# tum-vision/mono_dataset_code

Hardware: AMD Instinct MI355X
Metric: Mpix/s photometric+FOV undistort, 1280x1024 gray (higher is better)
Workload: dtype f32

## Files before the change

### include/mdc_hip.h

```cpp
#ifndef MDC_HIP_H
#define MDC_HIP_H

#include <stddef.h>
#include <stdint.h>

#ifndef MDC_API
#if defined(__GNUC__) || defined(__clang__)
#define MDC_API __attribute__((visibility("default")))
#else
#define MDC_API
#endif
#endif

#ifdef __cplusplus
extern "C" {
#endif

typedef struct mdc_ctx mdc_ctx;

typedef enum mdc_status {
  MDC_OK = 0,
  MDC_ERR_ARG = -1,
  MDC_ERR_STATE = -2,
  MDC_ERR_SIZE = -3,
  MDC_ERR_HIP = -4,
  MDC_ERR_NO_DEVICE = -5,
  MDC_ERR_NOMEM = -6
} mdc_status;

enum {
  MDC_GAMMA = 1u,
  MDC_VIGNETTE = 2u,
  MDC_KILL_OVEREXPOSED = 4u,
  MDC_RECTIFY = 8u
};

enum {
  MDC_KERNEL_AUTO = 0,
  MDC_KERNEL_GATHER = 1,
  MDC_KERNEL_TILED = 2
};
enum { MDC_OPT_KERNEL = 1, MDC_OPT_FRAMES_PER_BLOCK = 2 ,
       MDC_OPT_TILE_ROWS = 5 ,
       MDC_OPT_TILE_ORDER = 6 ,
       MDC_OPT_WINDOW_BUFFERS = 7 ,
       MDC_OPT_FRAME_INTERLEAVE = 8 ,
       MDC_OPT_TILE_COLS = 9 ,
       MDC_OPT_PIN_CALLER_BUFFERS = 10 ,
       MDC_OPT_TWO_STAGE = 11 ,
       MDC_OPT_PREFETCH_CHUNK = 12 ,
       MDC_OPT_PREFETCH_STREAMS = 13 ,
       MDC_OPT_ZERO_COPY = 14 ,
       MDC_OPT_DEVICE_PIPELINE_CHUNK = 16 ,
       MDC_OPT_DEVICE_PIPELINE_CHUNK_HINT = 17 ,
       MDC_OPT_TAIL_TAPER = 15 ,
       MDC_OPT_XCD_ROTATE = 18  };
enum { MDC_ORDER_BANDS = 0 , MDC_ORDER_ROWS = 1 ,
       MDC_ORDER_IDENTITY = 2 ,
       MDC_ORDER_BLOCKS2D = 3  };

typedef struct mdc_info {
  int device;
  int in_w, in_h;
  int out_w, out_h;
  int valid_gamma;
  int valid_vignette;
  int valid_remap;
  int tiled;
  int tile_w, tile_h;
  int n_tiles;
  int lds_bytes;
  int window_buffers;
  int f32_tiled;
  int f32_tile_w, f32_tile_h;
  int src_bbox[4];
  int64_t src_bbox_bytes;
  int64_t src_staged_bytes;
  int64_t n_black;
  int two_stage;
  int prefetch_chunk;
  int prefetch_streams;
} mdc_info;


MDC_API int mdc_create(int device, mdc_ctx** out);
MDC_API int mdc_device_count(void);
MDC_API int mdc_device_pci_bus_id(mdc_ctx* ctx, char* buf, size_t cap);
MDC_API void mdc_destroy(mdc_ctx* ctx);
MDC_API const char* mdc_last_error(const mdc_ctx* ctx);
MDC_API int mdc_get_info(mdc_ctx* ctx, mdc_info* info);
MDC_API int mdc_set_option(mdc_ctx* ctx, int option, int value);
MDC_API const char* mdc_build_flags(void);
MDC_API const char* mdc_code_id(void);


MDC_API int mdc_set_photometric(mdc_ctx* ctx, const float* ginv, const float* vignette_inv, int w, int h);

MDC_API int mdc_set_remap(mdc_ctx* ctx, const float* remap_x, const float* remap_y, int in_w, int in_h, int out_w, int out_h);


MDC_API int mdc_unmap_host(mdc_ctx* ctx, const uint8_t* image_in, float* image_out, int n, unsigned flags);

MDC_API int mdc_undistort_host_f32(mdc_ctx* ctx, const float* input, float* output, int n_in, int n_out);
MDC_API int mdc_undistort_host_u8(mdc_ctx* ctx, const uint8_t* input, float* output, int n_in, int n_out);

MDC_API int mdc_process_host(mdc_ctx* ctx, const uint8_t* raw, float* out, unsigned flags);


MDC_API void* mdc_host_alloc(size_t bytes);
MDC_API void mdc_host_free(void* p);

MDC_API int mdc_process_frames_host(mdc_ctx* ctx, const uint8_t* const* raw, float* const* out, int64_t nframes,
                            unsigned flags);

MDC_API int mdc_process_jpeg_frames_host(mdc_ctx* ctx, const void* const* records, int64_t record_bytes, int blocks_w, int blocks_rows,
                                 float* const* out, int64_t nframes, unsigned flags);
MDC_API int mdc_jpeg_idct_batch_device(mdc_ctx* ctx, const void* d_records, int64_t record_bytes, uint8_t* d_frames, int w, int h, int blocks_w,
                               int blocks_rows, int64_t nframes, void* stream);

#define MDC_JPEG_STREAM_MAGIC 0x33534a4du
#define MDC_JPEG_HUFF_SUBTABLES 32
typedef struct mdc_jpeg_huff {
  uint32_t t1[2048];
  uint32_t t2[MDC_JPEG_HUFF_SUBTABLES][32];
} mdc_jpeg_huff;
typedef struct mdc_jpeg_stream_header {
  uint32_t magic, w, h, ecs_bytes;
  uint32_t restart_interval;
  uint32_t n_intervals;
  uint32_t comp_info;
  uint32_t ecs_offset;
  uint16_t quant[64];
  mdc_jpeg_huff dc, ac;
} mdc_jpeg_stream_header;
MDC_API int mdc_process_jpeg_streams_host(mdc_ctx* ctx, const void* const* streams, const int64_t* stream_bytes, float* const* out, int64_t nframes,
                                  unsigned flags, int* status);
MDC_API int mdc_jpeg_huffman_batch_device(mdc_ctx* ctx, const void* d_streams, int64_t stream_stride, void* d_records, int64_t record_bytes, int w,
                                  int h, int blocks_w, int blocks_rows, int64_t nframes, int* d_status, void* stream);

typedef struct mdc_device_outputs {
  float* base;
  int levels;
  float* level[3];
  float* dI[4];
  float* abs_squared_grad[4];
} mdc_device_outputs;
MDC_API int mdc_process_frames_host_to_device(mdc_ctx* ctx, const uint8_t* const* raw, int64_t nframes, unsigned flags,
                                              const mdc_device_outputs* out, const int64_t* frame_index);
MDC_API int mdc_process_jpeg_frames_host_to_device(mdc_ctx* ctx, const void* const* records, int64_t record_bytes, int blocks_w, int blocks_rows,
                                                   int64_t nframes, unsigned flags, const mdc_device_outputs* out, const int64_t* frame_index);
MDC_API int mdc_process_jpeg_streams_host_to_device(mdc_ctx* ctx, const void* const* streams, const int64_t* stream_bytes, int64_t nframes,
                                                    unsigned flags, const mdc_device_outputs* out, const int64_t* frame_index, int* status);
MDC_API int mdc_device_alloc(mdc_ctx* ctx, size_t bytes, void** d_ptr);
MDC_API int mdc_tune_placement_device(mdc_ctx* ctx, const uint8_t* const* d_in, int n_in, float* const* d_out, int n_out, int64_t nframes,
                                      unsigned flags, void* stream, int* best_in, int* best_out, float* ms);
enum { MDC_PLACE_AUTO = 0, MDC_PLACE_FIRST = 1, MDC_PLACE_MALLOC = 2, MDC_PLACE_VMM = 3 };
typedef struct mdc_placed_buffers {
  uint8_t* d_in;
  float* d_out;
  size_t in_bytes, out_bytes;
  int64_t nframes, probe_frames;
  int strategy;
  int candidates_in, candidates_out, picked_in, picked_out;
  float pair_ms[64];
  int pieces, piece_mib;
  int class_count[3];
  float ms_first, ms_chosen;
  char note[384];
  void* handle;
} mdc_placed_buffers;
MDC_API int mdc_alloc_placed_device(mdc_ctx* ctx, size_t in_bytes, size_t out_bytes, int64_t nframes, unsigned flags, int strategy, void* stream,
                                    mdc_placed_buffers* out);
MDC_API int mdc_free_placed_device(mdc_ctx* ctx, mdc_placed_buffers* buffers);
#define MDC_STRIPED_SET_MAX 16
typedef struct mdc_striped_set {
  int n;
  void* d_ptr[MDC_STRIPED_SET_MAX];
  size_t bytes[MDC_STRIPED_SET_MAX];
  int strategy;
  int pieces, piece_mib;
  int class_count[3];
  char note[384];
  void* handle;
} mdc_striped_set;
MDC_API int mdc_alloc_striped_set_device(mdc_ctx* ctx, int n, const size_t* bytes, void* stream, mdc_striped_set* out);
MDC_API int mdc_free_striped_set_device(mdc_ctx* ctx, mdc_striped_set* set);
MDC_API void mdc_device_free(mdc_ctx* ctx, void* d_ptr);
MDC_API int mdc_copy_to_host(mdc_ctx* ctx, void* dst, const void* d_src, size_t bytes);


MDC_API int mdc_unmap_batch_device(mdc_ctx* ctx, const uint8_t* d_in, float* d_out, int64_t nframes, unsigned flags,
                           void* stream);

MDC_API int mdc_process_batch_device(mdc_ctx* ctx, const uint8_t* d_in, float* d_out, int64_t nframes, unsigned flags,
                             void* stream);

MDC_API int mdc_undistort_batch_device_f32(mdc_ctx* ctx, const float* d_in, float* d_out, int64_t nframes, void* stream);

MDC_API int mdc_pyramid_batch_device(mdc_ctx* ctx, const float* d_base, int w, int h, int levels, float* const* d_levels,
                             int64_t nframes, void* stream);

MDC_API int mdc_process_pyramid_batch_device(mdc_ctx* ctx, const uint8_t* d_in, float* d_base, int levels,
                                     float* const* d_levels, int64_t nframes, unsigned flags, void* stream);

MDC_API int mdc_gradients_batch_device(mdc_ctx* ctx, const float* d_level, int w, int h, float* d_dI, float* d_abs_squared_grad,
                               int64_t nframes, void* stream);

MDC_API int mdc_process_pyramid_gradients_batch_device(mdc_ctx* ctx, const uint8_t* d_in, float* d_base, int levels, float* const* d_levels,
                                               float* const* d_dI, float* const* d_abs_squared_grad, int64_t nframes, unsigned flags,
                                               int chunk_frames, void* stream);


typedef struct mdc_fov_model {
  float in_calib[5];
  int in_w, in_h;
  float out_calib[5];
  int out_w, out_h;
} mdc_fov_model;

MDC_API int mdc_distort_points_device(mdc_ctx* ctx, const mdc_fov_model* model, float* d_x, float* d_y, int64_t n, void* stream);
MDC_API int mdc_distort_points_host(mdc_ctx* ctx, const mdc_fov_model* model, float* x, float* y, int64_t n);



MDC_API int mdc_vcal_plane_step_device(mdc_ctx* ctx, const float* d_images, const float* d_p2x, const float* d_p2y, int n_images, int w, int h,
                               int n_plane, float* d_plane_color, const float* d_vignette_factor, int oth2, float* d_ff,
                               float* d_fc, double* d_er, void* stream);
MDC_API int mdc_vcal_vignette_step_device(mdc_ctx* ctx, const float* d_images, const float* d_p2x, const float* d_p2y, int n_images, int w,
                                  int h, int n_plane, const float* d_plane_color, float* d_vignette_factor, int oth2, float* d_tt,
                                  float* d_ct, double* d_er, void* stream);

typedef struct mdc_vcal_index mdc_vcal_index;
MDC_API int mdc_vcal_index_create(mdc_ctx* ctx, const float* d_images, const float* d_p2x, const float* d_p2y, int n_images, int w, int h,
                          int n_plane, void* stream, mdc_vcal_index** out);
MDC_API void mdc_vcal_index_destroy(mdc_vcal_index* index);
MDC_API int64_t mdc_vcal_index_bytes(const mdc_vcal_index* index);
MDC_API int64_t mdc_vcal_index_entries(const mdc_vcal_index* index);
MDC_API int mdc_vcal_vignette_step_indexed_device(mdc_ctx* ctx, const mdc_vcal_index* index, const float* d_plane_color,
                                          float* d_vignette_factor, int oth2, float* d_tt, float* d_ct, double* d_er, void* stream);

MDC_API int mdc_vcal_solve_device(mdc_ctx* ctx, const float* d_images, const float* d_p2x, const float* d_p2y, int n_images, int w, int h,
                          int n_plane, float* d_plane_color, float* d_vignette_factor, int max_iterations, int outlier_th,
                          double* er_out, void* stream);

MDC_API int mdc_vcal_scale_images_device(mdc_ctx* ctx, float* d_images, int n_images, int64_t npix, float mean_exposure,
                                 const float* d_exposure_times, void* stream);

MDC_API int mdc_vcal_gradient_mask_device(mdc_ctx* ctx, float* d_images, int n_images, int w, int h, int max_abs_grad, void* stream);

MDC_API int mdc_vcal_mask_coords_device(mdc_ctx* ctx, float* d_x, float* d_y, int64_t n, int w, int h, void* stream);

MDC_API int mdc_vcal_plane_coords_device(mdc_ctx* ctx, const mdc_fov_model* model, const float* d_corners, float* d_hk, int n, int gw,
                                 int gh, float facw, float fach, float* d_p2x, float* d_p2y, void* stream);

MDC_API int mdc_vcal_smooth_device(mdc_ctx* ctx, const float* d_vignette_factor, int w, int h, float* d_smoothed, float* d_scratch,
                           void* stream);

MDC_API int mdc_vcal_plot_plane_device(mdc_ctx* ctx, const float* d_plane, int gw, int gh, uint8_t* d_rgb, float* range_host, void* stream);
MDC_API int mdc_vcal_vignette_u16_device(mdc_ctx* ctx, const float* d_vignette, int64_t n, uint16_t* d_out, void* stream);



MDC_API int mdc_rcal_leak_pad_device(mdc_ctx* ctx, uint8_t* d_images, int n_images, int w, int h, int leak_padding, void* stream);
MDC_API int mdc_rcal_init_e_device(mdc_ctx* ctx, const uint8_t* d_images, int n_images, int w, int h, double* d_E, void* stream);
MDC_API int mdc_rcal_rmse_device(mdc_ctx* ctx, const uint8_t* d_images, const double* d_exposure, int n_images, int w, int h,
                         const double* d_G, const double* d_E, double* d_out, void* stream);
MDC_API int mdc_rcal_g_step_device(mdc_ctx* ctx, const uint8_t* d_images, const double* d_exposure, int n_images, int w, int h,
                           const double* d_E, double* d_G, void* stream);
typedef struct mdc_rcal_index mdc_rcal_index;
MDC_API int mdc_rcal_index_create(mdc_ctx* ctx, const uint8_t* d_images, int n_images, int w, int h, void* stream, mdc_rcal_index** out);
MDC_API void mdc_rcal_index_destroy(mdc_rcal_index* index);
MDC_API int64_t mdc_rcal_index_bytes(const mdc_rcal_index* index);
MDC_API int64_t mdc_rcal_index_entries(const mdc_rcal_index* index);
MDC_API int64_t mdc_rcal_index_longest_chain(const mdc_rcal_index* index);
MDC_API int mdc_rcal_g_step_indexed_device(mdc_ctx* ctx, const mdc_rcal_index* index, const double* d_exposure, const double* d_E,
                                   double* d_G, void* stream);
MDC_API int mdc_rcal_e_step_device(mdc_ctx* ctx, const uint8_t* d_images, const double* d_exposure, int n_images, int w, int h,
                           const double* d_G, double* d_E, double* d_rmse_g, void* stream);
MDC_API int mdc_rcal_rescale_device(mdc_ctx* ctx, const uint8_t* d_images, const double* d_exposure, int n_images, int w, int h,
                            double* d_G, double* d_E, double* d_rmse_e, double* d_rmse_resc, void* stream);

#define MDC_RCAL_EXACT_ORDER 0u
#define MDC_RCAL_DIRECT 1u
typedef struct mdc_rcal_iter {
  double rmse_G, num_G;
  double rmse_E, num_E;
  double rmse_resc, num_resc;
  double rescale;
} mdc_rcal_iter;
typedef struct mdc_rcal_log {
  double init_rmse, init_num;
  mdc_rcal_iter* iters;
} mdc_rcal_log;
MDC_API int mdc_rcal_solve_device(mdc_ctx* ctx, const uint8_t* d_images, const double* d_exposure, int n_images, int w, int h,
                          int iterations, unsigned mode, double* d_G, double* d_E, mdc_rcal_log* log, void* stream);
MDC_API int mdc_rcal_plot_e_device(mdc_ctx* ctx, const double* d_E, int w, int h, uint8_t* d_rgb, uint16_t* d_e16, double* range_host,
                           void* stream);
MDC_API int mdc_rcal_plot_g_device(mdc_ctx* ctx, const double* d_G, float* d_img, double* range_host, void* stream);
MDC_API int mdc_copy_to_device(mdc_ctx* ctx, void* d_dst, const void* src, size_t bytes);

typedef struct mdc_tune_result {
  int tile_w, tile_h, frames_per_block;
  float ms;
  int candidates;
} mdc_tune_result;
MDC_API int mdc_tune_device(mdc_ctx* ctx, const uint8_t* d_in, float* d_out, int64_t nframes, unsigned flags, void* stream,
                    mdc_tune_result* result);

MDC_API int mdc_describe_launch(mdc_ctx* ctx, unsigned flags, int pyramid_levels, char* buf, size_t cap);


MDC_API int mdc_export_tables(mdc_ctx* ctx, void* blob, size_t cap, size_t* size);
MDC_API int mdc_import_tables(mdc_ctx* ctx, const void* blob, size_t size);

MDC_API int mdc_synchronize(mdc_ctx* ctx);

#ifdef __cplusplus
}
#endif
#endif
```

### mono_dataset_code_amd/build.py

```python
import os
import shutil
import subprocess
import time
import sys

PKG = os.path.dirname(os.path.abspath(__file__))
ROOT = os.path.dirname(PKG)
CSRC = os.path.join(PKG, "csrc")
HOST = os.path.join(CSRC, "host")
INC = os.path.join(ROOT, "include")
EIGEN_STUB = os.path.join(INC, "mono_dataset_code", "compat")

LIB_HIP = os.path.join(PKG, "libmdc_hip.so")
LIB_HOST = os.path.join(PKG, "libmdc_host.so")

HIP_SOURCES = [os.path.join(CSRC, f) for f in ("mdc_kernels.hip", "mdc_vcal.hip", "mdc_jpeg.hip", "mdc_capi.hip", "mdc_plan.hip", "mdc_host_calls.hip",
                                                "mdc_pipeline.hip", "mdc_placement.hip", "mdc_rcal.hip")]
HIP_DEPS = HIP_SOURCES + [os.path.join(CSRC, "mdc_exports.map"), os.path.join(CSRC, "mdc_internal.h"), os.path.join(CSRC, "mdc_ctx.h"), os.path.join(CSRC, "mdc_build_config.h"), os.path.join(CSRC, "fov_point_model.h"), os.path.join(CSRC, "minmax_first.h"), os.path.join(CSRC, "placement_classes.h"), os.path.join(CSRC, "xcd_placement.h"), os.path.join(INC, "mdc_hip.h")]
HOST_SOURCES = [os.path.join(HOST, f) for f in (
    "fov_undistorter.cpp", "photometric_undistorter.cpp", "gray_png.cpp", "host_device.cpp", "mdc_host_capi.cpp",
    "image_codecs.cpp", "image_codecs_png.cpp", "image_codecs_jpeg.cpp", "image_codecs_jpeg_stream.cpp", "zip_reader.cpp", "image_pool.cpp", "frame_source.cpp", "decode_pool.cpp",
    "prefetch_cache.cpp", "device_lanes.cpp", "batch_run.cpp", "dataset_reader.cpp")]
HOST_DEPS = HOST_SOURCES + [os.path.join(HOST, "mdc_host_exports.map"), os.path.join(HOST, "gray_png.h"), os.path.join(HOST, "host_device.h"),
                            os.path.join(HOST, "image_codecs.h"), os.path.join(HOST, "image_codecs_internal.h"), os.path.join(HOST, "image_codecs_jpeg.h"), os.path.join(HOST, "zip_reader.h"),
                            os.path.join(HOST, "frame_source.h"), os.path.join(HOST, "decode_pool.h"), os.path.join(HOST, "prefetch_cache.h"),
                            os.path.join(HOST, "device_lanes.h"), os.path.join(HOST, "batch_run.h"), os.path.join(CSRC, "png_inflate_core.h"),
                            os.path.join(INC, "mono_dataset_code", "BenchmarkDatasetReader.h"),
                            os.path.join(INC, "mdc_hip.h"), os.path.join(INC, "mdc_host.h"),
                            os.path.join(INC, "mono_dataset_code", "FOVUndistorter.h"),
                            os.path.join(INC, "mono_dataset_code", "PhotometricUndistorter.h"),
                            os.path.join(INC, "mono_dataset_code", "ExposureImage.h"),
                            os.path.join(INC, "mono_dataset_code", "MdcBind.h")]

HIP_FLAGS = ["--offload-arch=gfx950", "-O3", "-std=c++17", "-ffp-contract=off", "-fPIC", "-shared",
             "-fno-fast-math", "-fvisibility=hidden", "-fvisibility-inlines-hidden", "-Wall", "-Wno-unused-function"]
HOST_FLAGS = ["-O2", "-std=c++11", "-ffp-contract=off", "-fPIC", "-shared", "-fvisibility=hidden", "-fvisibility-inlines-hidden", "-Wall"]
HOST_EXPORT_MAP = os.path.join(HOST, "mdc_host_exports.map")
EXPORT_MAP = os.path.join(CSRC, "mdc_exports.map")
RECIPE = os.path.abspath(__file__)


def _stale(target, deps):
    if not os.path.exists(target):
        return True
    t = os.path.getmtime(target)
    return any(os.path.getmtime(d) > t for d in deps)


def _run(cmd):
    r = subprocess.run(cmd, stdout=subprocess.PIPE, stderr=subprocess.STDOUT, text=True)
    if r.returncode != 0:
        sys.stderr.write(r.stdout)
        raise RuntimeError("build failed: " + " ".join(cmd))
    return r.stdout


def hipcc():
    for c in (os.environ.get("HIPCC"), shutil.which("hipcc"), "/opt/rocm/bin/hipcc"):
        if c and os.path.exists(c):
            return c
    raise RuntimeError("hipcc not found")


def eigen_include():
    for d in ("/usr/include/eigen3", "/usr/local/include/eigen3"):
        if os.path.exists(os.path.join(d, "Eigen", "Core")):
            return d
    return EIGEN_STUB


def code_text(src):
    out, i, n = [], 0, len(src)
    while i < n:
        c = src[i]
        if c == "/" and i + 1 < n and src[i + 1] == "/":
            while i < n and src[i] != "\n":
                if src[i] == "\\" and i + 1 < n and src[i + 1] == "\n":
                    i += 1
                i += 1
        elif c == "/" and i + 1 < n and src[i + 1] == "*":
            j = src.find("*/", i + 2)
            i = n if j < 0 else j + 2
            out.append(" ")
        elif c in "\"'":
            j = i + 1
            while j < n and src[j] != c:
                j += 2 if src[j] == "\\" else 1
            out.append(src[i:j + 1])
            i = j + 1
        elif c in " \t\r\f\v":
            if not out or out[-1] != " ":
                out.append(" ")
            i += 1
        else:
            out.append(c)
            i += 1
    lines = [l.strip() for l in "".join(out).split("\n")]
    return "\n".join(l for l in lines if l)


def code_id(defines=()):
    import hashlib

    h = hashlib.sha256()
    for path in sorted(HIP_DEPS):
        h.update(os.path.basename(path).encode() + b"\0")
        with open(path, "r", encoding="utf-8", errors="surrogateescape") as f:
            h.update(code_text(f.read()).encode("utf-8", "surrogateescape"))
    h.update(" ".join(HIP_FLAGS + sorted(defines)).encode())
    try:
        h.update(subprocess.run([hipcc(), "--version"], stdout=subprocess.PIPE).stdout)
    except OSError:
        pass
    return h.hexdigest()[:16]


def _linked_from(lib, defines=()):
    try:
        with open(lib, "rb") as f:
            return code_id(defines).encode() in f.read()
    except OSError:
        return False


def _compile_link_hip(out, defines=(), objdir_tag="product"):
    from concurrent.futures import ThreadPoolExecutor

    started = time.time()
    identity = code_id(defines)
    objdir = os.path.join(PKG, "build", objdir_tag)
    os.makedirs(objdir, exist_ok=True)
    flags = [f for f in HIP_FLAGS if f != "-shared"] + ["-I" + INC] + ["-D" + d for d in defines]
    stamp = os.path.join(objdir, "flags.txt")
    flags_changed = not os.path.exists(stamp) or open(stamp).read() != " ".join(flags)
    headers = [d for d in HIP_DEPS if d not in HIP_SOURCES]
    jobs = []
    for src in HIP_SOURCES:
        obj = os.path.join(objdir, os.path.basename(src) + ".o")
        if flags_changed or _stale(obj, [src] + headers) or not os.path.exists(out) or not _linked_from(out, defines):
            jobs.append([hipcc()] + flags + ["-c", src, "-o", obj])
    with ThreadPoolExecutor(max_workers=max(1, len(jobs))) as ex:
        list(ex.map(_run, jobs))
    with open(stamp, "w") as f:
        f.write(" ".join(flags))
    objs = [os.path.join(objdir, os.path.basename(src) + ".o") for src in HIP_SOURCES]
    idsrc = os.path.join(objdir, "mdc_code_id.cpp")
    with open(idsrc, "w") as f:
        f.write('#include "mdc_hip.h"\nextern "C" const char* mdc_code_id(void) { return "%s"; }\n' % identity)
    idobj = idsrc + ".o"
    _run(["g++", "-O1", "-fPIC", "-fvisibility=hidden", "-I" + INC, "-c", idsrc, "-o", idobj])
    _run([hipcc(), "--offload-arch=gfx950", "-shared", "-fPIC", "-Wl,--version-script=" + EXPORT_MAP] + objs + [idobj, "-o", out])
    if any(os.path.getmtime(d) > started for d in HIP_DEPS):
        sys.stderr.write("mono_dataset_code_amd.build: a source changed while %s was being built; it is stamped %s and the next build redoes it\n"
                         % (os.path.basename(out), identity))


def build_hip(force=False):
    if force or _stale(LIB_HIP, HIP_DEPS + [RECIPE]) or not _linked_from(LIB_HIP):
        if force:
            shutil.rmtree(os.path.join(PKG, "build", "product"), ignore_errors=True)
        _compile_link_hip(LIB_HIP)
    return LIB_HIP


def build_host(force=False):
    build_hip(force)
    if force or _stale(LIB_HOST, HOST_DEPS + [LIB_HIP]):
        _run(["g++"] + HOST_FLAGS + ["-I" + INC, "-I" + os.path.join(INC, "mono_dataset_code"), "-I" + HOST,
                                     "-I" + eigen_include()] + HOST_SOURCES +
             ["-L" + PKG, "-lmdc_hip", "-Wl,-rpath,$ORIGIN", "-Wl,--version-script=" + HOST_EXPORT_MAP, "-lz", "-lpthread", "-ldl", "-o", LIB_HOST])
    return LIB_HOST
# ... 211 lines not shown
```

### mono_dataset_code_amd/capi.py

```python
import ctypes as C
import os
import types

import numpy as np

_PKG = os.path.dirname(os.path.abspath(__file__))
LIB_HIP_PATH = os.environ.get("MDC_LIB_HIP") or os.path.join(_PKG, "libmdc_hip.so")
LIB_HOST_PATH = os.path.join(_PKG, "libmdc_host.so")

GAMMA, VIGNETTE, KILL_OVEREXPOSED, RECTIFY = 1, 2, 4, 8
KERNEL_AUTO, KERNEL_GATHER, KERNEL_TILED = 0, 1, 2
OPT_KERNEL, OPT_FRAMES_PER_BLOCK, OPT_TILE_ROWS, OPT_TILE_ORDER, OPT_WINDOW_BUFFERS, OPT_FRAME_INTERLEAVE, OPT_TILE_COLS, OPT_PIN_CALLER_BUFFERS = 1, 2, 5, 6, 7, 8, 9, 10
OPT_TWO_STAGE = 11
OPT_PREFETCH_CHUNK = 12
OPT_PREFETCH_STREAMS = 13
OPT_ZERO_COPY = 14
OPT_TAIL_TAPER = 15
OPT_XCD_ROTATE = 18
OPT_DEVICE_PIPELINE_CHUNK, OPT_DEVICE_PIPELINE_CHUNK_HINT = 16, 17
ORDER_BANDS, ORDER_ROWS, ORDER_IDENTITY, ORDER_BLOCKS2D = 0, 1, 2, 3
OK, ERR_ARG, ERR_STATE, ERR_SIZE, ERR_HIP, ERR_NO_DEVICE, ERR_NOMEM = 0, -1, -2, -3, -4, -5, -6

PLACE_AUTO, PLACE_FIRST, PLACE_MALLOC, PLACE_VMM = 0, 1, 2, 3
PLACE_NAMES = {PLACE_AUTO: "auto", PLACE_FIRST: "first", PLACE_MALLOC: "malloc", PLACE_VMM: "vmm"}


RCAL_EXACT_ORDER, RCAL_DIRECT = 0, 1


class RcalIter(C.Structure):
    _fields_ = [(n, C.c_double) for n in ("rmse_G", "num_G", "rmse_E", "num_E", "rmse_resc", "num_resc", "rescale")]


class RcalLog(C.Structure):
    _fields_ = [("init_rmse", C.c_double), ("init_num", C.c_double), ("iters", C.POINTER(RcalIter))]


class PlacedBuffers(C.Structure):
    _fields_ = [("d_in", C.c_void_p), ("d_out", C.c_void_p), ("in_bytes", C.c_size_t), ("out_bytes", C.c_size_t), ("nframes", C.c_int64),
                ("probe_frames", C.c_int64), ("strategy", C.c_int), ("candidates_in", C.c_int), ("candidates_out", C.c_int), ("picked_in", C.c_int),
                ("picked_out", C.c_int), ("pair_ms", C.c_float * 64), ("pieces", C.c_int), ("piece_mib", C.c_int), ("class_count", C.c_int * 3),
                ("ms_first", C.c_float), ("ms_chosen", C.c_float), ("note", C.c_char * 384), ("handle", C.c_void_p)]

    def describe(self):
        d = {"strategy": PLACE_NAMES.get(self.strategy, str(self.strategy)), "how": self.note.decode(errors="replace"),
             "probe_frames": int(self.probe_frames), "ms_on_first_allocations": round(float(self.ms_first), 4) or None,
             "ms_on_chosen_pair": round(float(self.ms_chosen), 4) or None}
        if self.strategy == PLACE_MALLOC and self.candidates_in > 1:
            ki, ko = self.candidates_in, self.candidates_out
            d["ms_frames_i_results_j"] = [[round(float(self.pair_ms[i * ko + j]), 4) for j in range(ko)] for i in range(ki)]
            d["picked_frames"], d["picked_results"] = int(self.picked_in), int(self.picked_out)
        if self.strategy == PLACE_VMM:
            d["pieces"], d["piece_mib"], d["class_count"] = int(self.pieces), int(self.piece_mib), [int(x) for x in self.class_count]
        return d


class StripedSet(C.Structure):
    _fields_ = [("n", C.c_int), ("d_ptr", C.c_void_p * 16), ("bytes", C.c_size_t * 16), ("strategy", C.c_int), ("pieces", C.c_int), ("piece_mib", C.c_int),
                ("class_count", C.c_int * 3), ("note", C.c_char * 384), ("handle", C.c_void_p)]


class FovModel(C.Structure):
    _fields_ = [("in_calib", C.c_float * 5), ("in_w", C.c_int), ("in_h", C.c_int), ("out_calib", C.c_float * 5),
                ("out_w", C.c_int), ("out_h", C.c_int)]


class MdcInfo(C.Structure):
    _fields_ = [("device", C.c_int), ("in_w", C.c_int), ("in_h", C.c_int), ("out_w", C.c_int), ("out_h", C.c_int),
                ("valid_gamma", C.c_int), ("valid_vignette", C.c_int), ("valid_remap", C.c_int), ("tiled", C.c_int),
                ("tile_w", C.c_int), ("tile_h", C.c_int), ("n_tiles", C.c_int), ("lds_bytes", C.c_int),
                ("window_buffers", C.c_int), ("f32_tiled", C.c_int), ("f32_tile_w", C.c_int), ("f32_tile_h", C.c_int),
                ("src_bbox", C.c_int * 4), ("src_bbox_bytes", C.c_int64), ("src_staged_bytes", C.c_int64),
                ("n_black", C.c_int64), ("two_stage", C.c_int), ("prefetch_chunk", C.c_int), ("prefetch_streams", C.c_int)]


class DeviceOutputs(C.Structure):
    _fields_ = [("base", C.c_void_p), ("levels", C.c_int), ("level", C.c_void_p * 3), ("dI", C.c_void_p * 4), ("abs_squared_grad", C.c_void_p * 4)]

    @classmethod
    def make(cls, base, levels=1, level=(), dI=(), abs2=()):
        o = cls()
        o.base, o.levels = base, levels
        for i, p in enumerate(level):
            o.level[i] = p
        for i, p in enumerate(dI):
            o.dI[i] = p
        for i, p in enumerate(abs2):
            o.abs_squared_grad[i] = p
        return o


class TuneResult(C.Structure):
    _fields_ = [("tile_w", C.c_int), ("tile_h", C.c_int), ("frames_per_block", C.c_int), ("ms", C.c_float), ("candidates", C.c_int)]


class MdcError(RuntimeError):
    def __init__(self, code, msg):
        super().__init__("mdc error %d: %s" % (code, msg))
        self.code = code


_vp, _i, _i64, _u32, _sz = C.c_void_p, C.c_int, C.c_int64, C.c_uint32, C.c_size_t
_u, _f, _cp, _P = C.c_uint, C.c_float, C.c_char_p, C.POINTER

HIP_API = {
    "mdc_create": (_i, [_i, _P(_vp)]),
    "mdc_device_count": (_i, []),
    "mdc_device_pci_bus_id": (_i, [_vp, _cp, _sz]),
    "mdc_destroy": (None, [_vp]),
    "mdc_last_error": (_cp, [_vp]),
    "mdc_get_info": (_i, [_vp, _P(MdcInfo)]),
    "mdc_set_option": (_i, [_vp, _i, _i]),
    "mdc_build_flags": (_cp, []),
    "mdc_code_id": (_cp, []),
    "mdc_set_photometric": (_i, [_vp, _vp, _vp, _i, _i]),
    "mdc_set_remap": (_i, [_vp, _vp, _vp, _i, _i, _i, _i]),
    "mdc_unmap_host": (_i, [_vp, _vp, _vp, _i, _u]),
    "mdc_undistort_host_f32": (_i, [_vp, _vp, _vp, _i, _i]),
    "mdc_undistort_host_u8": (_i, [_vp, _vp, _vp, _i, _i]),
    "mdc_process_host": (_i, [_vp, _vp, _vp, _u]),
    "mdc_host_alloc": (_vp, [_sz]),
    "mdc_host_free": (None, [_vp]),
    "mdc_process_frames_host": (_i, [_vp, _P(_vp), _P(_vp), _i64, _u]),
    "mdc_process_jpeg_frames_host": (_i, [_vp, _P(_vp), _i64, _i, _i, _P(_vp), _i64, _u]),
    "mdc_jpeg_idct_batch_device": (_i, [_vp, _vp, _i64, _vp, _i, _i, _i, _i, _i64, _vp]),
    "mdc_process_jpeg_streams_host": (_i, [_vp, _P(_vp), _P(_i64), _P(_vp), _i64, _u, _P(_i)]),
    "mdc_jpeg_huffman_batch_device": (_i, [_vp, _vp, _i64, _vp, _i64, _i, _i, _i, _i, _i64, _vp, _vp]),
    "mdc_process_frames_host_to_device": (_i, [_vp, _P(_vp), _i64, _u, _P(DeviceOutputs), _P(_i64)]),
    "mdc_process_jpeg_frames_host_to_device": (_i, [_vp, _P(_vp), _i64, _i, _i, _i64, _u, _P(DeviceOutputs), _P(_i64)]),
    "mdc_process_jpeg_streams_host_to_device": (_i, [_vp, _P(_vp), _P(_i64), _i64, _u, _P(DeviceOutputs), _P(_i64), _P(_i)]),
    "mdc_device_alloc": (_i, [_vp, _sz, _P(_vp)]),
    "mdc_tune_placement_device": (_i, [_vp, _P(_vp), _i, _P(_vp), _i, _i64, _u, _vp, _P(_i), _P(_i), _P(_f)]),
    "mdc_alloc_placed_device": (_i, [_vp, _sz, _sz, _i64, _u, _i, _vp, _P(PlacedBuffers)]),
    "mdc_free_placed_device": (_i, [_vp, _P(PlacedBuffers)]),
    "mdc_alloc_striped_set_device": (_i, [_vp, _i, _P(_sz), _vp, _P(StripedSet)]),
    "mdc_free_striped_set_device": (_i, [_vp, _P(StripedSet)]),
    "mdc_device_free": (None, [_vp, _vp]),
    "mdc_copy_to_host": (_i, [_vp, _vp, _vp, _sz]),
    "mdc_unmap_batch_device": (_i, [_vp, _vp, _vp, _i64, _u, _vp]),
    "mdc_process_batch_device": (_i, [_vp, _vp, _vp, _i64, _u, _vp]),
    "mdc_undistort_batch_device_f32": (_i, [_vp, _vp, _vp, _i64, _vp]),
    "mdc_pyramid_batch_device": (_i, [_vp, _vp, _i, _i, _i, _P(_vp), _i64, _vp]),
    "mdc_process_pyramid_batch_device": (_i, [_vp, _vp, _vp, _i, _P(_vp), _i64, _u, _vp]),
    "mdc_gradients_batch_device": (_i, [_vp, _vp, _i, _i, _vp, _vp, _i64, _vp]),
    "mdc_process_pyramid_gradients_batch_device": (_i, [_vp, _vp, _vp, _i, _P(_vp), _P(_vp), _P(_vp), _i64, _u, _i, _vp]),
    "mdc_distort_points_device": (_i, [_vp, _P(FovModel), _vp, _vp, _i64, _vp]),
    "mdc_distort_points_host": (_i, [_vp, _P(FovModel), _vp, _vp, _i64]),
    "mdc_vcal_plane_step_device": (_i, [_vp, _vp, _vp, _vp, _i, _i, _i, _i, _vp, _vp, _i, _vp, _vp, _vp, _vp]),
    "mdc_vcal_vignette_step_device": (_i, [_vp, _vp, _vp, _vp, _i, _i, _i, _i, _vp, _vp, _i, _vp, _vp, _vp, _vp]),
    "mdc_vcal_index_create": (_i, [_vp, _vp, _vp, _vp, _i, _i, _i, _i, _vp, _P(_vp)]),
    "mdc_vcal_index_destroy": (None, [_vp]),
    "mdc_vcal_index_bytes": (_i64, [_vp]),
    "mdc_vcal_index_entries": (_i64, [_vp]),
    "mdc_vcal_vignette_step_indexed_device": (_i, [_vp, _vp, _vp, _vp, _i, _vp, _vp, _vp, _vp]),
    "mdc_vcal_solve_device": (_i, [_vp, _vp, _vp, _vp, _i, _i, _i, _i, _vp, _vp, _i, _i, _vp, _vp]),
    "mdc_vcal_scale_images_device": (_i, [_vp, _vp, _i, _i64, _f, _vp, _vp]),
    "mdc_vcal_gradient_mask_device": (_i, [_vp, _vp, _i, _i, _i, _i, _vp]),
    "mdc_vcal_mask_coords_device": (_i, [_vp, _vp, _vp, _i64, _i, _i, _vp]),
    "mdc_vcal_plane_coords_device": (_i, [_vp, _P(FovModel), _vp, _vp, _i, _i, _i, _f, _f, _vp, _vp, _vp]),
    "mdc_vcal_smooth_device": (_i, [_vp, _vp, _i, _i, _vp, _vp, _vp]),
    "mdc_vcal_plot_plane_device": (_i, [_vp, _vp, _i, _i, _vp, _vp, _vp]),
    "mdc_vcal_vignette_u16_device": (_i, [_vp, _vp, _i64, _vp, _vp]),
    "mdc_rcal_leak_pad_device": (_i, [_vp, _vp, _i, _i, _i, _i, _vp]),
    "mdc_rcal_init_e_device": (_i, [_vp, _vp, _i, _i, _i, _vp, _vp]),
    "mdc_rcal_rmse_device": (_i, [_vp, _vp, _vp, _i, _i, _i, _vp, _vp, _vp, _vp]),
    "mdc_rcal_g_step_device": (_i, [_vp, _vp, _vp, _i, _i, _i, _vp, _vp, _vp]),
    "mdc_rcal_index_create": (_i, [_vp, _vp, _i, _i, _i, _vp, _P(_vp)]),
    "mdc_rcal_index_destroy": (None, [_vp]),
    "mdc_rcal_index_bytes": (_i64, [_vp]),
    "mdc_rcal_index_entries": (_i64, [_vp]),
    "mdc_rcal_index_longest_chain": (_i64, [_vp]),
    "mdc_rcal_g_step_indexed_device": (_i, [_vp, _vp, _vp, _vp, _vp, _vp]),
    "mdc_rcal_e_step_device": (_i, [_vp, _vp, _vp, _i, _i, _i, _vp, _vp, _vp, _vp]),
    "mdc_rcal_rescale_device": (_i, [_vp, _vp, _vp, _i, _i, _i, _vp, _vp, _vp, _vp, _vp]),
    "mdc_rcal_solve_device": (_i, [_vp, _vp, _vp, _i, _i, _i, _i, _u, _vp, _vp, _P(RcalLog), _vp]),
    "mdc_rcal_plot_e_device": (_i, [_vp, _vp, _i, _i, _vp, _vp, _vp, _vp]),
    "mdc_rcal_plot_g_device": (_i, [_vp, _vp, _vp, _vp, _vp]),
    "mdc_copy_to_device": (_i, [_vp, _vp, _vp, _sz]),
    "mdc_tune_device": (_i, [_vp, _vp, _vp, _i64, _u, _vp, _P(TuneResult)]),
    "mdc_describe_launch": (_i, [_vp, _u, _i, _cp, _sz]),
    "mdc_export_tables": (_i, [_vp, _vp, _sz, _P(_sz)]),
    "mdc_import_tables": (_i, [_vp, _vp, _sz]),
    "mdc_synchronize": (_i, [_vp]),
}
HOST_API = {
    "mdch_fov_create": (_vp, [_cp]),
    "mdch_fov_destroy": (None, [_vp]),
    "mdch_fov_valid": (_i, [_vp]),
    "mdch_fov_has_gpu": (_i, [_vp]),
    "mdch_fov_dims": (None, [_vp, _vp]),
    "mdch_fov_intrinsics": (None, [_vp, _vp]),
    "mdch_fov_remap": (_i, [_vp, _vp, _vp]),
    "mdch_fov_distort": (None, [_vp, _vp, _vp, _i]),
    "mdch_fov_undistort_f32": (None, [_vp, _vp, _vp, _i, _i]),
    "mdch_fov_undistort_u8": (None, [_vp, _vp, _vp, _i, _i]),
    "mdch_fov_model": (None, [_vp, _P(FovModel)]),
    "mdch_photo_create": (_vp, [_cp, _cp, _i, _i]),
    "mdch_photo_destroy": (None, [_vp]),
    "mdch_photo_valid": (_i, [_vp]),
    "mdch_photo_has_gpu": (_i, [_vp]),
    "mdch_photo_ginv": (_i, [_vp, _vp]),
    "mdch_photo_g": (_i, [_vp, _vp]),
    "mdch_photo_vignette": (_i, [_vp, _vp, _vp]),
    "mdch_photo_unmap": (None, [_vp, _vp, _vp, _i, _i, _i, _i]),
    "mdch_bind": (_i, [_vp, _vp, _vp]),
    "mdch_pack_tables": (_i, [_vp, _vp, _vp, _sz, _P(_sz)]),
    "mdch_reader_create": (_vp, [_cp]),
    "mdch_reader_destroy": (None, [_vp]),
    "mdch_reader_num_images": (_i, [_vp]),
    "mdch_reader_timestamp": (C.c_double, [_vp, _i]),
    "mdch_reader_exposure": (_f, [_vp, _i]),
    "mdch_reader_dims": (None, [_vp, _vp]),
    "mdch_reader_get_image": (_i, [_vp, _i, _i, _i, _i, _i, _vp, C.c_long, _vp, _P(C.c_double), _P(_f)]),
    "mdch_reader_get_images": (_i, [_vp, _i, _i, _i, _i, _i, _i, _vp, C.c_long, _vp]),
    "mdch_reader_get_images_device": (_i, [_vp, _i, _i, _i, _i, _i, _i, _P(DeviceOutputs), _vp]),
    "mdch_reader_context": (_vp, [_vp]),
    "mdch_reader_device": (_i, [_vp]),
    "mdch_reader_get_raw": (_i, [_vp, _i, _vp, C.c_long, _vp]),
    "mdch_reader_get_images_raw_device": (_i, [_vp, _i, _i, _i, _vp, _vp]),
    "mdch_reader_raw_dims": (None, [_vp, _vp]),
    "mdch_reader_set_threads": (None, [_vp, _i]),
    "mdch_reader_set_prefetch": (None, [_vp, _i]),
    "mdch_reader_set_lookahead": (None, [_vp, _i]),
    "mdch_reader_set_gpu_jpeg": (None, [_vp, _i]),
    "mdch_reader_set_gpu_png": (None, [_vp, _i]),
    "mdch_reader_png_device_frames": (C.c_long, [_vp]),
    "mdch_reader_last_error": (_cp, [_vp]),
    "mdch_reader_prefetch_stats": (None, [_vp, _vp]),
    "mdch_reader_device_stats": (_i, [_vp, _i, _vp, _vp]),
    "mdch_decode_gray8": (_i, [_vp, _sz, _vp, _sz, _vp, _cp, _sz]),
    "mdch_jpeg_record_bytes": (_sz, [_i, _i, _vp]),
    "mdch_decode_jpeg_record": (_i, [_vp, _sz, _vp, _sz, _i, _vp, _cp, _sz]),
    "mdch_jpeg_stream": (C.c_longlong, [_vp, _sz, _vp, _sz, _vp, _cp, _sz]),
    "mdch_png_stream": (_i, [_vp, _sz, _P(_i), _P(_i), _vp, _sz, _P(_sz)]),
    "mdch_image_alloc": (_vp, [C.c_ulong]),
    "mdch_image_free": (None, [_vp]),
    "mdch_image_pool_trim": (None, []),
    "mdch_image_pool_idle_bytes": (C.c_ulong, []),
}
BENCH_API = {
    "mdcb_synth_frames_device": (_i, [_i, _vp, _i64, _i64, _i, _u32, _vp]),
    "mdcb_ceiling_mix_device": (_i, [_i, _vp, _i64, _vp, _i64, _i, _i, _vp]),
    "mdcb_marker_device": (_i, [_i, _i, _vp]),
    "mdcb_alias_alloc": (_i, [_i, _i64, _i, _P(_vp), _P(_i64)]),
    "mdcb_alias_free": (_i, [_i, _vp, _i64, _i]),
    "mdcb_chunked_alloc": (_i, [_i, _i64, _i, _i, _P(_vp)]),
# ... 1225 lines not shown
```

### mono_dataset_code_amd/csrc/mdc_capi.hip

```cpp
#include "mdc_ctx.h"

using namespace mdc;


namespace mdc {

static thread_local std::string g_create_err;
static thread_local std::string t_err, t_err_other;
static thread_local const mdc_ctx* t_err_ctx = nullptr;

int fail(mdc_ctx* c, int code, const char* fmt, ...) {
  char buf[512];
  va_list ap;
  va_start(ap, fmt);
  vsnprintf(buf, sizeof buf, fmt, ap);
  va_end(ap);
  if (c) {
    {
      std::lock_guard<std::mutex> lk(c->err_mu);
      c->err = buf;
    }
    t_err = buf;
    t_err_ctx = c;
  } else {
    g_create_err = buf;
  }
  return code;
}



void normalise(const mdc_ctx* c, unsigned flags, bool& g, bool& v, bool& o) {
  g = (flags & MDC_GAMMA) != 0;
  v = (flags & MDC_VIGNETTE) != 0;
  o = (flags & MDC_KILL_OVEREXPOSED) != 0;
  if (!c->valid_gamma && g) g = false;
  if (!c->valid_vignette && v) v = false;
  if (!g && v) {
    v = false;
    g = false;
  }
}

const float* lut_for(const mdc_ctx* c, bool g, bool o) { return c->d_luts + 256 * ((g ? 1 : 0) | (o ? 2 : 0)); }

int upload_luts(mdc_ctx* c) {
  std::vector<float> l(4 * 256);
  for (int var = 0; var < 4; var++)
    for (int b = 0; b < 256; b++) {
      float x = (var & 1) ? (c->valid_gamma ? c->h_ginv[b] : (float)b) : (float)b;
      if ((var & 2) && b == 255) x = std::numeric_limits<float>::quiet_NaN();
      l[var * 256 + b] = x;
    }
  if (!c->d_luts) MDC_HIP(c, hipMalloc(&c->d_luts, l.size() * sizeof(float)));
  MDC_HIP(c, hipMemcpy(c->d_luts, l.data(), l.size() * sizeof(float), hipMemcpyHostToDevice));
  return MDC_OK;
}

int frames_per_block(const mdc_ctx* c, int64_t nframes, int blocks_per_group, int target_wgs) {
  if (c->opt_fpb > 0) return (int)std::min<int64_t>(c->opt_fpb, std::max<int64_t>(nframes, 1));
  int64_t groups = std::max<int64_t>(1, (target_wgs + blocks_per_group - 1) / std::max(1, blocks_per_group));
  groups = std::min<int64_t>(groups, std::max<int64_t>(1, nframes / 8));
  int64_t fpb = (nframes + groups - 1) / groups;
  if (fpb < 32 && (int64_t)blocks_per_group * ((nframes + 31) / 32) >= 2048) fpb = 32;
  if (target_wgs == 4800 && fpb > 64) fpb = 64;
  return (int)fpb;
}













TilePlan tile_plan(const mdc_ctx* c, int which) {
  const mdc_ctx::SrcPlan& pl = c->plan[which];
  return TilePlan{pl.d_chunks, pl.d_nch, pl.d_taps, pl.d_order, pl.n_blocks, pl.n_tiles, pl.tiles_x, pl.tile_w, pl.tile_h,
                  pl.chunk_cap, pl.win_bytes, pl.nbuf, c->n_black > 0, c->opt_interleave != 0, c->opt_taper != 2, c->opt_xcd_rotate != 0};
}

RemapArgs remap_args(const mdc_ctx* c, const float* lut, const float* vinv) {
  RemapArgs a;
  a.lut = lut;
  a.vinv = vinv;
  a.rx = c->d_rx;
  a.ry = c->d_ry;
  a.in_w = c->rm_in_w;
  a.in_h = c->rm_in_h;
  a.out_w = c->out_w;
  a.out_h = c->out_h;
  return a;
}

int64_t prefetch_box_bytes(const mdc_ctx* c) {
  const int x0 = c->bbox[0], x1 = c->bbox[2], y0 = c->bbox[1], y1 = c->bbox[3];
  return y1 >= y0 ? (int64_t)(y1 - y0 + 1) * std::min(c->rm_in_w, ((x1 + 128) & ~127) - (x0 & ~127)) : 0;
}
int prefetch_streams(const mdc_ctx* c) { return c->opt_prefetch_streams == 1 ? 1 : 2; }
int64_t strip_resident(bool pyr) { return 256 * (pyr ? 4 : 5); }
int64_t chunk_groups(const mdc_ctx* c, bool pyr) {
  const int64_t nb = std::max(1, c->strip.n_blocks);
  return std::max<int64_t>(1, (strip_resident(pyr) * 5 / 8 + nb / 2) / nb);
}
int64_t prefetch_chunk_frames(const mdc_ctx* c, bool pyr = true) {
  if (c->opt_prefetch_chunk > 0) return c->opt_prefetch_chunk;
  const int64_t box = std::max<int64_t>(1, prefetch_box_bytes(c));
  if (prefetch_streams(c) == 1) return std::max<int64_t>(16, (31ll << 20) / box);
  const int64_t g = chunk_groups(c, pyr);
  const int64_t per_group = std::max<int64_t>(8, ((26ll << 20) / box + g / 2) / g);
  return g * per_group;
}

int enqueue_undistort_f32(mdc_ctx* c, const float* d_in, float* d_out, int64_t nframes, hipStream_t s) {
  RemapArgs a = remap_args(c, nullptr, nullptr);
  const bool aligned = (reinterpret_cast<uintptr_t>(d_in) & 15) == 0;
  if (c->plan[1].tiled && aligned && c->opt_kernel != MDC_KERNEL_GATHER) {
    const int fpb = frames_per_block(c, nframes, c->plan[1].n_blocks);
    MDC_HIP(c, launch_remap_tiled_f32(d_in, d_out, a, tile_plan(c, 1), nframes, fpb, s));
  } else {
    const int fpb = frames_per_block(c, nframes, (c->out_w * c->out_h + 255) / 256);
    MDC_HIP(c, launch_remap_gather_f32(d_in, d_out, a, nframes, fpb, s));
  }
  return MDC_OK;
}

int enqueue_process(mdc_ctx* c, const uint8_t* d_in, float* d_out, int64_t nframes, unsigned flags, hipStream_t s,
                    float* const* pyr, bool* pyr_done) {
  if (pyr_done) *pyr_done = false;
  bool g, v, o;
  normalise(c, flags, g, v, o);
  const float* lut = lut_for(c, g, o);
  const float* vinv = v ? c->d_vinv : nullptr;
  if (!(flags & MDC_RECTIFY)) {
    const int fw = c->in_w > 0 ? c->in_w : c->rm_in_w, fh = c->in_h > 0 ? c->in_h : c->rm_in_h;
    if (fw <= 0 || fh <= 0) return fail(c, MDC_ERR_STATE, "frame size unknown: set the photometric tables or a remap first");
    const int64_t npix = (int64_t)fw * fh;
    int fpb = frames_per_block(c, nframes, (int)((npix + 4095) / 4096), 20000);
    if (!c->opt_fpb) fpb = std::min(fpb, 8);
    MDC_HIP(c, launch_unmap(d_in, d_out, lut, vinv, npix, nframes, fpb, s));
    return MDC_OK;
  }
  if (!c->valid_remap) return fail(c, MDC_ERR_STATE, "no remap set (UndistorterFOV invalid)");
  if (vinv && (c->in_w != c->rm_in_w || c->in_h != c->rm_in_h))
    return fail(c, MDC_ERR_SIZE, "vignette is %dx%d but the remap expects %dx%d input", c->in_w, c->in_h, c->rm_in_w,
                c->rm_in_h);
  RemapArgs a = remap_args(c, lut, vinv);
  const bool aligned = (reinterpret_cast<uintptr_t>(d_in) & 15) == 0;
  if (c->strip.planned && aligned && c->opt_kernel != MDC_KERNEL_GATHER) {
    const mdc_ctx::Strip& st = c->strip;
    const StripPlan sp{st.d_chunks, st.d_nch, st.d_taps, st.d_order, st.n_blocks, st.n_tiles, st.tiles_x, st.win_bytes, st.passes, st.nbuf,
                       c->opt_interleave != 0, c->opt_xcd_rotate == 2};
    const bool fuse_pyr = pyr && c->out_w % kStripTileW == 0;
    const int iw = c->rm_in_w;
    const int x0 = c->bbox[0], x1 = c->bbox[2], y0 = c->bbox[1], y1 = c->bbox[3];
    const int64_t frame_in = (int64_t)iw * c->rm_in_h;
    const int64_t box_bytes = prefetch_box_bytes(c);
    int64_t chunk = prefetch_chunk_frames(c, fuse_pyr);
    const bool prefetch = c->opt_prefetch_chunk >= 0 && (fuse_pyr || c->opt_prefetch_chunk > 0 || prefetch_streams(c) == 2) && box_bytes >= 4096 &&
                          nframes >= 2 * chunk;
    if (!prefetch) chunk = nframes;
    const size_t no = (size_t)c->out_w * c->out_h;
    const int64_t resident = strip_resident(fuse_pyr);
    auto strip = [&](int64_t f0, int64_t n, int fpb, hipStream_t t) {
      return launch_remap_strip_u8(d_in + (size_t)f0 * frame_in, d_out + (size_t)f0 * no, a, sp, n, fpb, t,
                                   fuse_pyr ? pyr[0] + (size_t)f0 * (no / 4) : nullptr, fuse_pyr ? pyr[1] + (size_t)f0 * (no / 16) : nullptr,
                                   fuse_pyr ? pyr[2] + (size_t)f0 * (no / 64) : nullptr);
    };
    hipStreamCaptureStatus capturing = hipStreamCaptureStatusNone;
    if (hipStreamIsCapturing(s, &capturing) != hipSuccess) {
      (void)hipGetLastError();
      capturing = hipStreamCaptureStatusNone;
    }
    if (prefetch && prefetch_streams(c) == 2 && capturing == hipStreamCaptureStatusNone) {
      SlotLease side(c, false);
      side.drained();
      mdc_ctx::HostSlot* h = side.s;
      if (h && !h->ev_fork) {
        if (hipEventCreateWithFlags(&h->ev_fork, hipEventDisableTiming) != hipSuccess) h->ev_fork = nullptr;
        if (h->ev_fork && hipEventCreateWithFlags(&h->ev_join, hipEventDisableTiming) != hipSuccess) {
          (void)hipEventDestroy(h->ev_fork);
          h->ev_fork = nullptr;
        }
      }
      if (h && h->ev_fork) {
        const int64_t groups = chunk_groups(c, fuse_pyr);
        MDC_HIP(c, hipEventRecord(h->ev_fork, s));
        MDC_HIP(c, hipStreamWaitEvent(h->stream, h->ev_fork, 0));
        hipError_t e = hipSuccess;
        int k = 0;
        for (int64_t f0 = 0; f0 < nframes && e == hipSuccess; f0 += chunk, k++) {
          const int64_t n = std::min<int64_t>(chunk, nframes - f0);
          hipStream_t t = (k & 1) ? h->stream : s;
          e = launch_prefetch_rows(d_in + (size_t)f0 * frame_in, frame_in, iw, x0, x1, y0, y1, n, c->d_vcal_max, t);
          const int fpb = c->opt_fpb > 0 ? (int)std::min<int64_t>(c->opt_fpb, n) : (int)((n + groups - 1) / groups);
          if (e == hipSuccess) e = strip(f0, n, fpb, t);
        }
        const hipError_t ej = hipEventRecord(h->ev_join, h->stream);
        const hipError_t ew = ej == hipSuccess ? hipStreamWaitEvent(s, h->ev_join, 0) : ej;
        MDC_HIP(c, e);
        MDC_HIP(c, ew);
        if (pyr_done) *pyr_done = fuse_pyr;
        return MDC_OK;
      }
    }
    if (prefetch) MDC_HIP(c, launch_prefetch_rows(d_in, frame_in, iw, x0, x1, y0, y1, std::min<int64_t>(chunk, nframes), c->d_vcal_max, s));
    for (int64_t f0 = 0; f0 < nframes; f0 += chunk) {
      const int64_t n = std::min<int64_t>(chunk, nframes - f0);
      if (prefetch && f0 + chunk < nframes)
        MDC_HIP(c, launch_prefetch_rows(d_in + (size_t)(f0 + chunk) * frame_in, frame_in, iw, x0, x1, y0, y1, std::min<int64_t>(chunk, nframes - f0 - chunk),
                                        c->d_vcal_max, s));
      int fpb = frames_per_block(c, n, st.n_blocks);
      if (prefetch && !c->opt_fpb) fpb = (int)std::max<int64_t>(8, (n * st.n_blocks + resident - 1) / resident);
      MDC_HIP(c, strip(f0, n, fpb, s));
    }
    if (pyr_done) *pyr_done = fuse_pyr;
    return MDC_OK;
  }
  bool use_tiled = c->plan[0].tiled && aligned;
  if (c->opt_kernel == MDC_KERNEL_GATHER) use_tiled = false;
  if (c->opt_kernel == MDC_KERNEL_TILED && !use_tiled)
    return fail(c, MDC_ERR_STATE, "tiled kernel requested but not plannable for this remap / alignment");
  if (use_tiled) {
    const TilePlan p = tile_plan(c, 0);
    int fpb = frames_per_block(c, nframes, p.n_blocks);
    if (!c->opt_fpb && c->tuned_fpb > 0 && nframes >= c->tuned_min_frames) fpb = (int)std::min<int64_t>(c->tuned_fpb, nframes);
    const bool fuse_pyr = pyr && p.tile_w * p.tile_h <= 2048 && p.tile_h % 8 == 0 && c->out_w % p.tile_w == 0 && c->out_h % p.tile_h == 0 &&
                          tiled_lds_bytes(p.win_bytes, p.nbuf, true) + tiled_pyramid_lds_bytes(p.tile_w, p.tile_h) <= kLdsPerCU;
    MDC_HIP(c, launch_remap_tiled_u8(d_in, d_out, a, p, nframes, fpb, s, fuse_pyr ? pyr[0] : nullptr,
                                     fuse_pyr ? pyr[1] : nullptr, fuse_pyr ? pyr[2] : nullptr));
    if (pyr_done) *pyr_done = fuse_pyr;
  } else {
    const int fpb = frames_per_block(c, nframes, (c->out_w * c->out_h + 255) / 256);
    MDC_HIP(c, launch_remap_gather_u8(d_in, d_out, a, nframes, fpb, s));
  }
  return MDC_OK;
}

int enqueue_pyramid_gradients(mdc_ctx* c, const uint8_t* d_in, float* d_base, int levels, float* const* d_levels, float* const* d_dI,
                              float* const* d_abs_squared_grad, int64_t nframes, unsigned flags, int chunk_frames, hipStream_t s) {
  const bool with_gradients = d_dI != nullptr && d_abs_squared_grad != nullptr;
  const bool rect = (flags & MDC_RECTIFY) != 0;
  if (rect && !c->valid_remap) return fail(c, MDC_ERR_STATE, "no remap set (UndistorterFOV invalid)");
  const int w0 = rect ? c->out_w : (c->in_w > 0 ? c->in_w : c->rm_in_w), h0 = rect ? c->out_h : (c->in_h > 0 ? c->in_h : c->rm_in_h);
  const int iw = (rect || c->in_w <= 0) ? c->rm_in_w : c->in_w, ih = (rect || c->in_h <= 0) ? c->rm_in_h : c->in_h;
  if (w0 <= 0 || h0 <= 0 || iw <= 0 || ih <= 0) return fail(c, MDC_ERR_STATE, "frame size unknown");
  int lw[8], lh[8];
  size_t level_bytes = 0;
  for (int l = 0; l < levels; l++) {
    lw[l] = w0 >> l;
    lh[l] = h0 >> l;
    if (lw[l] < 1 || lh[l] < 1) return fail(c, MDC_ERR_ARG, "level %d of a %dx%d image is empty", l, w0, h0);
    level_bytes += (size_t)lw[l] * lh[l] * sizeof(float);
  }
  int64_t chunk = chunk_frames;
  if (chunk <= 0) {
    chunk = (int64_t)((672ull << 20) / level_bytes);
    chunk = chunk >= 32 ? chunk / 32 * 32 : std::max<int64_t>(1, chunk);
  }
  {
    int64_t wgs = 0;
    for (int l = 0; l < std::min(levels, 4); l++) wgs += (int64_t)((lw[l] + 127) / 128) * ((lh[l] + 7) / 8);
    chunk = std::max<int64_t>(1, std::min<int64_t>(chunk, ((1ll << 31) - 1) / std::max<int64_t>(1, wgs)));
  }
  const size_t npi = (size_t)iw * ih;
  for (int64_t f0 = 0; f0 < nframes; f0 += chunk) {
    const int64_t n = std::min<int64_t>(chunk, nframes - f0);
    float* lv[8];
    for (int l = 1; l < levels; l++) lv[l - 1] = d_levels[l - 1] + (size_t)f0 * lw[l] * lh[l];
    float* base = d_base + (size_t)f0 * w0 * h0;
    float* pyr[3] = {levels > 1 ? lv[0] : nullptr, levels > 2 ? lv[1] : nullptr, levels > 3 ? lv[2] : nullptr};
    bool fused = false;
#if MDC_EXP_STRIP_FAKE_GRAD
    g_fake_grad_dI = with_gradients ? d_dI[0] + (size_t)f0 * w0 * h0 * 3 : nullptr;
    g_fake_grad_abs = with_gradients ? d_abs_squared_grad[0] + (size_t)f0 * w0 * h0 : nullptr;
#endif
    int rc = enqueue_process(c, d_in + (size_t)f0 * npi, base, n, flags, s, levels > 1 ? pyr : nullptr, &fused);
#if MDC_EXP_STRIP_FAKE_GRAD
    g_fake_grad_dI = g_fake_grad_abs = nullptr;
#endif
    if (rc != MDC_OK) return rc;
    const int first = fused ? std::min(levels, 4) : 1;
    const float* src = first == 1 ? base : lv[first - 2];
    for (int l = first; l < levels; l++) {
      MDC_HIP(c, launch_pyramid_level(src, lv[l - 1], lw[l - 1], lh[l - 1], n, s));
      src = lv[l - 1];
    }
#if MDC_EXP_STRIP_FAKE_GRAD
    constexpr int kGradFirst = 1;
#else
    constexpr int kGradFirst = 0;
#endif
    for (int l0 = kGradFirst; l0 < levels && with_gradients; l0 += 4) {
      const int nl = std::min(4, levels - l0);
      const float* gs[4];
      float *gd[4], *ga[4];
      for (int k = 0; k < nl; k++) {
        const int l = l0 + k;
        gs[k] = l == 0 ? base : lv[l - 1];
        gd[k] = d_dI[l] + (size_t)f0 * lw[l] * lh[l] * 3;
        ga[k] = d_abs_squared_grad[l] + (size_t)f0 * lw[l] * lh[l];
      }
      MDC_HIP(c, launch_gradients_levels(nl, gs, gd, ga, lw + l0, lh + l0, n, s));
    }
  }
  return MDC_OK;
}

struct BlobHeader {
  uint32_t magic, version;
  int32_t in_w, in_h, rm_in_w, rm_in_h, out_w, out_h;
  int32_t valid_gamma, valid_vignette, valid_remap, pad;
};
constexpr uint32_t kMagic = 0x4d444331u;

DistortModel distort_model(const mdc_fov_model* f) {
  return make_distort_model(f->in_calib, f->in_w, f->in_h, f->out_calib, f->out_w, f->out_h);
}

}

static int set_photometric_locked(mdc_ctx* c, const float* ginv, const float* vignette_inv, int w, int h);
static int set_remap_locked(mdc_ctx* c, const float* rx, const float* ry, int in_w, int in_h, int out_w, int out_h);


extern "C" {

int mdc_create(int device, mdc_ctx** out) try {
  if (!out) return fail(nullptr, MDC_ERR_ARG, "mdc_create: out is NULL");
  *out = nullptr;
  int n = 0;
  hipError_t e = hipGetDeviceCount(&n);
  if (e != hipSuccess || n <= 0)
    return fail(nullptr, MDC_ERR_NO_DEVICE, "no HIP device visible (%s); this library has no CPU fallback",
                e == hipSuccess ? "device count 0" : hipGetErrorString(e));
  if (device == -1 && hipGetDevice(&device) != hipSuccess) device = 0;
  if (device < 0 || device >= n) return fail(nullptr, MDC_ERR_ARG, "device %d out of range [0,%d)", device, n);
  mdc_ctx* c = new mdc_ctx();
  c->device = device;
  DeviceGuard dg(device);
  c->h_ginv.assign(256, 0.f);
  if (const char* e = getenv("MDC_PIN_CALLER_BUFFERS")) c->opt_pin_caller = atoi(e) != 0;
  if (const char* e = getenv("MDC_ZERO_COPY")) c->opt_zero_copy = std::max(0, std::min(2, atoi(e)));
  int rc = upload_luts(c);
  if (rc == MDC_OK && hipMalloc(&c->d_vcal_max, mdc_ctx::kVcalMaxWords * sizeof(unsigned)) != hipSuccess)
    rc = fail(c, MDC_ERR_HIP, "hipMalloc of the context's scratch words failed");
  if (rc != MDC_OK) {
    g_create_err = t_err;
    if (c->d_luts) (void)hipFree(c->d_luts);
    t_err_ctx = nullptr;
    delete c;
    return rc;
  }
  *out = c;
  return MDC_OK;
} MDC_CATCH(nullptr)

void mdc_destroy(mdc_ctx* c) {
  if (!c) return;
  {
    DeviceGuard dg(c->device);
    for (mdc_ctx::HostSlot* h : c->slots) {
      if (h->stream) (void)hipStreamSynchronize(h->stream);
      if (h->d_in) (void)hipFree(h->d_in);
      if (h->d_out) (void)hipFree(h->d_out);
      if (h->ev_fork) (void)hipEventDestroy(h->ev_fork);
      if (h->ev_join) (void)hipEventDestroy(h->ev_join);
      if (h->stream) (void)hipStreamDestroy(h->stream);
      delete h;
    }
    c->slots.clear();
    for (int k = 0; k < 2; k++)
      if (c->pipe_stream[k]) (void)hipStreamSynchronize(c->pipe_stream[k]);
    if (c->pipe_up_stream) (void)hipStreamSynchronize(c->pipe_up_stream);
    unpin_all(c);
    free_plan(c);
    {
      std::vector<void*> arenas;
      {
        std::lock_guard<std::mutex> lk(c->striped_mu);
        for (auto& kv : c->striped) arenas.push_back(kv.second);
        c->striped.clear();
      }
      for (void* a : arenas) {
        mdc_striped_set set;
        memset(&set, 0, sizeof set);
        set.handle = a;
        (void)mdc_free_striped_set_device(c, &set);
      }
    }
    void* ptrs[] = {c->d_luts, c->d_vinv, c->d_rx, c->d_ry, c->d_vcal_max, c->d_pipe_in[0], c->d_pipe_in[1], c->d_pipe_out[0], c->d_pipe_out[1],
                    c->d_pipe_rec[0], c->d_pipe_rec[1], c->d_pipe_strm[0], c->d_pipe_strm[1], c->d_pipe_status[0], c->d_pipe_status[1], c->d_pipe_seg[0], c->d_pipe_seg[1]};
    for (void* p : ptrs)
      if (p) (void)hipFree(p);
    if (c->h_pipe_status) (void)hipHostFree(c->h_pipe_status);
    for (int k = 0; k < 2; k++) {
      if (c->pipe_done[k]) (void)hipEventDestroy(c->pipe_done[k]);
      if (c->pipe_dec[k]) (void)hipEventDestroy(c->pipe_dec[k]);
      if (c->pipe_up[k]) (void)hipEventDestroy(c->pipe_up[k]);
      if (c->pipe_huff[k]) (void)hipEventDestroy(c->pipe_huff[k]);
      if (c->pipe_stream[k]) (void)hipStreamDestroy(c->pipe_stream[k]);
    }
    if (c->pipe_up_stream) (void)hipStreamDestroy(c->pipe_up_stream);
  }
  if (t_err_ctx == c) t_err_ctx = nullptr;
  delete c;
}

const char* mdc_build_flags(void) { return mdc::build_flags_string(); }

int mdc_device_count(void) {
  int n = 0;
  if (hipGetDeviceCount(&n) != hipSuccess) {
    (void)hipGetLastError();
    return 0;
  }
  return n;
}

const char* mdc_last_error(const mdc_ctx* c) {
  if (!c) return g_create_err.c_str();
  if (t_err_ctx == c) return t_err.c_str();
  std::lock_guard<std::mutex> lk(c->err_mu);
  t_err_other = c->err;
  return t_err_other.c_str();
}

int mdc_device_pci_bus_id(mdc_ctx* c, char* buf, size_t cap) try {
  if (!c) return MDC_ERR_ARG;
  if (!buf || cap < 13) return fail(c, MDC_ERR_ARG, "mdc_device_pci_bus_id: buffer of >= 13 bytes expected");
  char tmp[64] = {0};
  MDC_HIP(c, hipDeviceGetPCIBusId(tmp, (int)sizeof tmp, c->device));
  for (char* q = tmp; *q; q++) *q = (char)tolower((unsigned char)*q);
  snprintf(buf, cap, "%s", tmp);
  return MDC_OK;
} MDC_CATCH(c)

int mdc_set_option(mdc_ctx* c, int option, int value) try {
  if (!c) return MDC_ERR_ARG;
  WriteLock lk(c->mu);
  switch (option) {
    case MDC_OPT_KERNEL:
      if (value < MDC_KERNEL_AUTO || value > MDC_KERNEL_TILED) return fail(c, MDC_ERR_ARG, "bad kernel selector %d", value);
      c->opt_kernel = value;
      return MDC_OK;
    case MDC_OPT_FRAMES_PER_BLOCK:
      if (value < 0) return fail(c, MDC_ERR_ARG, "bad frames-per-block %d", value);
      c->opt_fpb = value;
      return MDC_OK;
    case MDC_OPT_TILE_ROWS: {
      if (value != 0 && value != 16 && value != 32 && value != 60 && value != 64)
        return fail(c, MDC_ERR_ARG, "tile rows must be 0 (automatic), 16, 32, 60 or 64");
      if (value == c->opt_tile_h) return MDC_OK;
      c->opt_tile_h = value;
      c->tuned_fpb = 0;
      if (!c->valid_remap) return MDC_OK;
      DeviceGuard dg(c->device);
      MDC_HIP(c, hipDeviceSynchronize());
      return plan_tiles(c);
    }
    case MDC_OPT_TILE_COLS: {
      if (value != 0 && value != 64 && value != 128) return fail(c, MDC_ERR_ARG, "tile columns must be 0 (automatic), 64 or 128");
      if (value == c->opt_tile_w) return MDC_OK;
      c->opt_tile_w = value;
      c->tuned_fpb = 0;
      if (!c->valid_remap) return MDC_OK;
      DeviceGuard dg(c->device);
      MDC_HIP(c, hipDeviceSynchronize());
      return plan_tiles(c);
    }
    case MDC_OPT_FRAME_INTERLEAVE:
      c->opt_interleave = value != 0;
      return MDC_OK;
    case MDC_OPT_PIN_CALLER_BUFFERS: {
      c->opt_pin_caller = value != 0;
      if (!c->opt_pin_caller) {
        DeviceGuard dg(c->device);
        MDC_HIP(c, hipDeviceSynchronize());
        unpin_all(c);
      }
      return MDC_OK;
    }
    case MDC_OPT_WINDOW_BUFFERS: {
      if (value < 0 || value > 4) return fail(c, MDC_ERR_ARG, "window buffers must be 0 (auto) or 1..4 (1: strip kernel only)");
      if (value == c->opt_nbuf) return MDC_OK;
      c->opt_nbuf = value;
      if (!c->valid_remap) return MDC_OK;
      DeviceGuard dg(c->device);
      MDC_HIP(c, hipDeviceSynchronize());
      return plan_tiles(c);
    }
    case MDC_OPT_DEVICE_PIPELINE_CHUNK:
      if (value != 0 && (value < 16 || value > 256)) return fail(c, MDC_ERR_ARG, "device pipeline chunk must be 0 (automatic) or 16..256 frames");
      c->opt_dev_chunk = value;
      return MDC_OK;
    case MDC_OPT_DEVICE_PIPELINE_CHUNK_HINT:
      if (value != 0 && (value < 16 || value > 256)) return fail(c, MDC_ERR_ARG, "device pipeline chunk hint must be 0 (none) or 16..256 frames");
      c->opt_dev_chunk_hint = value;
      return MDC_OK;
    case MDC_OPT_TAIL_TAPER:
      if (value < 0 || value > 2) return fail(c, MDC_ERR_ARG, "tail taper selector must be 0 (automatic), 1 (on) or 2 (off)");
      c->opt_taper = value;
      return MDC_OK;
    case MDC_OPT_ZERO_COPY:
      if (value < 0 || value > 2) return fail(c, MDC_ERR_ARG, "zero-copy selector must be 0 (automatic), 1 (on) or 2 (off)");
      c->opt_zero_copy = value;
      return MDC_OK;
    case MDC_OPT_PREFETCH_STREAMS:
      if (value < 0 || value > 2) return fail(c, MDC_ERR_ARG, "prefetch streams must be 0 (automatic), 1 or 2");
      c->opt_prefetch_streams = value;
      return MDC_OK;
    case MDC_OPT_PREFETCH_CHUNK:
      if (value < -1) return fail(c, MDC_ERR_ARG, "prefetch chunk must be -1 (off), 0 (automatic) or a frame count");
      c->opt_prefetch_chunk = value;
      return MDC_OK;
    case MDC_OPT_TWO_STAGE: {
      if (value < 0 || value > 2) return fail(c, MDC_ERR_ARG, "two-stage selector must be 0 (automatic), 1 (on) or 2 (off)");
      if (value == c->opt_two_stage) return MDC_OK;
      c->opt_two_stage = value;
      c->tuned_fpb = 0;
      if (!c->valid_remap) return MDC_OK;
      DeviceGuard dg(c->device);
      MDC_HIP(c, hipDeviceSynchronize());
      return plan_tiles(c);
    }
    case MDC_OPT_TILE_ORDER: {
      if (value < MDC_ORDER_BANDS || value > MDC_ORDER_BLOCKS2D) return fail(c, MDC_ERR_ARG, "bad tile order %d", value);
      if (value == c->opt_order) return MDC_OK;
      c->opt_order = value;
      if (!c->valid_remap) return MDC_OK;
      DeviceGuard dg(c->device);
      MDC_HIP(c, hipDeviceSynchronize());
      return plan_tiles(c);
    }
    case MDC_OPT_XCD_ROTATE: {
      if (value < 0 || value > 2) return fail(c, MDC_ERR_ARG, "XCD rotation must be 0 (off), 1 (on) or 2 (on, strip kernel included)");
      if (value == c->opt_xcd_rotate) return MDC_OK;
      c->opt_xcd_rotate = value;
      c->tuned_fpb = 0;
      if (!c->valid_remap) return MDC_OK;
      DeviceGuard dg(c->device);
      MDC_HIP(c, hipDeviceSynchronize());
      return plan_tiles(c);
    }
  }
  return fail(c, MDC_ERR_ARG, "unknown option %d", option);
} MDC_CATCH(c)

int mdc_get_info(mdc_ctx* c, mdc_info* i) try {
  if (!c || !i) return MDC_ERR_ARG;
  ReadLock lk(c->mu);
  memset(i, 0, sizeof *i);
  i->device = c->device;
  i->in_w = c->in_w ? c->in_w : c->rm_in_w;
  i->in_h = c->in_h ? c->in_h : c->rm_in_h;
  i->out_w = c->valid_remap ? c->out_w : 0;
  i->out_h = c->valid_remap ? c->out_h : 0;
  i->valid_gamma = c->valid_gamma;
  i->valid_vignette = c->valid_vignette;
  i->valid_remap = c->valid_remap;
  const mdc_ctx::SrcPlan& p0 = c->plan[0];
  i->tiled = c->valid_remap && p0.tiled;
  i->tile_w = p0.tiled ? p0.tile_w : c->opt_tile_w;
  i->tile_h = p0.tiled ? p0.tile_h : c->opt_tile_h;
  i->n_tiles = p0.n_tiles;
  i->lds_bytes = p0.tiled ? (int)tiled_lds_bytes(p0.win_bytes, p0.nbuf, true) : 0;
  i->two_stage = c->strip.planned ? 1 : 0;
  i->prefetch_chunk = (c->strip.planned && c->opt_prefetch_chunk >= 0 && prefetch_box_bytes(c) >= 4096) ? (int)prefetch_chunk_frames(c) : 0;
  i->prefetch_streams = i->prefetch_chunk ? prefetch_streams(c) : 0;
  if (c->strip.planned) {
    i->tiled = c->valid_remap;
    i->tile_w = kStripTileW;
    i->tile_h = kStripTileH;
    i->n_tiles = c->strip.n_tiles;
    i->lds_bytes = (int)strip_lds_bytes(c->strip.win_bytes, c->strip.nbuf, kStripWaves);
    i->window_buffers = c->strip.nbuf;
  }
  i->window_buffers = p0.tiled ? p0.nbuf : 0;
  i->f32_tiled = c->valid_remap && c->plan[1].tiled;
  i->f32_tile_w = c->plan[1].tiled ? c->plan[1].tile_w : 0;
  i->f32_tile_h = c->plan[1].tiled ? c->plan[1].tile_h : 0;
  for (int k = 0; k < 4; k++) i->src_bbox[k] = c->bbox[k];
  i->src_bbox_bytes = c->bbox[2] >= 0 ? (int64_t)(c->bbox[2] - c->bbox[0] + 1) * (c->bbox[3] - c->bbox[1] + 1) : 0;
  i->src_staged_bytes = c->strip.planned ? c->strip.staged_bytes : p0.staged_bytes;
  i->n_black = c->n_black;
  return MDC_OK;
} MDC_CATCH(c)

int mdc_set_photometric(mdc_ctx* c, const float* ginv, const float* vignette_inv, int w, int h) try {
  if (!c) return MDC_ERR_ARG;
  if (w <= 0 || h <= 0) return fail(c, MDC_ERR_ARG, "bad frame size %dx%d", w, h);
  WriteLock lk(c->mu);
  return set_photometric_locked(c, ginv, vignette_inv, w, h);
} MDC_CATCH(c)

static int set_photometric_locked(mdc_ctx* c, const float* ginv, const float* vignette_inv, int w, int h) {
  DeviceGuard dg(c->device);
  MDC_HIP(c, hipDeviceSynchronize());
  c->in_w = w;
  c->in_h = h;
  c->valid_gamma = ginv != nullptr;
  if (ginv) c->h_ginv.assign(ginv, ginv + 256);
  int rc = upload_luts(c);
  if (rc != MDC_OK) return rc;
  c->valid_vignette = vignette_inv != nullptr;
  if (c->d_vinv) {
    (void)hipFree(c->d_vinv);
    c->d_vinv = nullptr;
  }
  c->h_vinv.clear();
  if (vignette_inv) {
    const size_t n = (size_t)w * h;
    c->h_vinv.assign(vignette_inv, vignette_inv + n);
    MDC_HIP(c, hipMalloc(&c->d_vinv, n * sizeof(float)));
    MDC_HIP(c, hipMemcpy(c->d_vinv, vignette_inv, n * sizeof(float), hipMemcpyHostToDevice));
  }
  return MDC_OK;
}

int mdc_set_remap(mdc_ctx* c, const float* rx, const float* ry, int in_w, int in_h, int out_w, int out_h) try {
  if (!c) return MDC_ERR_ARG;
  WriteLock lk(c->mu);
  return set_remap_locked(c, rx, ry, in_w, in_h, out_w, out_h);
} MDC_CATCH(c)

static int set_remap_locked(mdc_ctx* c, const float* rx, const float* ry, int in_w, int in_h, int out_w, int out_h) {
  DeviceGuard dg(c->device);
  MDC_HIP(c, hipDeviceSynchronize());
  c->valid_remap = false;
  c->tuned_fpb = 0;
  free_plan(c);
  for (float** p : {&c->d_rx, &c->d_ry})
    if (*p) {
      (void)hipFree(*p);
      *p = nullptr;
    }
  c->h_rx.clear();
  c->h_ry.clear();
  if (!rx || !ry) return MDC_OK;
  if (in_w <= 1 || in_h <= 1 || out_w <= 0 || out_h <= 0)
    return fail(c, MDC_ERR_ARG, "bad remap geometry %dx%d -> %dx%d", in_w, in_h, out_w, out_h);
  const size_t n = (size_t)out_w * out_h;
  for (size_t i = 0; i < n; i++) {
    if (rx[i] < 0) continue;
    if (!(rx[i] > 0 && ry[i] > 0 && rx[i] < in_w - 1 && ry[i] < in_h - 1))
      return fail(c, MDC_ERR_ARG, "remap entry %zu = (%g,%g) is outside (0,%d)x(0,%d)", i, rx[i], ry[i], in_w - 1,
                  in_h - 1);
  }
  c->h_rx.assign(rx, rx + n);
  c->h_ry.assign(ry, ry + n);
  c->rm_in_w = in_w;
  c->rm_in_h = in_h;
  c->out_w = out_w;
  c->out_h = out_h;
  MDC_HIP(c, hipMalloc(&c->d_rx, n * sizeof(float)));
  MDC_HIP(c, hipMalloc(&c->d_ry, n * sizeof(float)));
  MDC_HIP(c, hipMemcpy(c->d_rx, rx, n * sizeof(float), hipMemcpyHostToDevice));
  MDC_HIP(c, hipMemcpy(c->d_ry, ry, n * sizeof(float), hipMemcpyHostToDevice));
  int rc = plan_tiles(c);
  if (rc != MDC_OK) return rc;
  c->valid_remap = true;
  return MDC_OK;
}

int mdc_unmap_batch_device(mdc_ctx* c, const uint8_t* d_in, float* d_out, int64_t nframes, unsigned flags, void* stream) try {
  if (!c) return MDC_ERR_ARG;
  if (!d_in || !d_out || nframes < 0) return fail(c, MDC_ERR_ARG, "mdc_unmap_batch_device: bad argument");
  ReadLock lk(c->mu);
  DeviceGuard dg(c->device);
  return enqueue_process(c, d_in, d_out, nframes, flags & ~MDC_RECTIFY, (hipStream_t)stream);
} MDC_CATCH(c)

int mdc_process_batch_device(mdc_ctx* c, const uint8_t* d_in, float* d_out, int64_t nframes, unsigned flags, void* stream) try {
  if (!c) return MDC_ERR_ARG;
  if (!d_in || !d_out || nframes < 0) return fail(c, MDC_ERR_ARG, "mdc_process_batch_device: bad argument");
  ReadLock lk(c->mu);
  DeviceGuard dg(c->device);
  return enqueue_process(c, d_in, d_out, nframes, flags, (hipStream_t)stream);
} MDC_CATCH(c)

int mdc_undistort_batch_device_f32(mdc_ctx* c, const float* d_in, float* d_out, int64_t nframes, void* stream) try {
  if (!c) return MDC_ERR_ARG;
  if (!d_in || !d_out || nframes < 0) return fail(c, MDC_ERR_ARG, "mdc_undistort_batch_device_f32: bad argument");
  ReadLock lk(c->mu);
  DeviceGuard dg(c->device);
  if (!c->valid_remap) return fail(c, MDC_ERR_STATE, "no remap set (UndistorterFOV invalid)");
  return enqueue_undistort_f32(c, d_in, d_out, nframes, (hipStream_t)stream);
} MDC_CATCH(c)

int mdc_pyramid_batch_device(mdc_ctx* c, const float* d_base, int w, int h, int levels, float* const* d_levels,
                             int64_t nframes, void* stream) try {
  if (!c) return MDC_ERR_ARG;
  if (!d_base || w <= 0 || h <= 0 || levels < 1 || nframes < 0 || (levels > 1 && !d_levels))
    return fail(c, MDC_ERR_ARG, "mdc_pyramid_batch_device: bad argument");
  ReadLock lk(c->mu);
  DeviceGuard dg(c->device);
  hipStream_t s = (hipStream_t)stream;
  const float* src = d_base;
  for (int l = 1; l < levels; l++) {
    if (!d_levels[l - 1]) return fail(c, MDC_ERR_ARG, "level %d buffer is NULL", l);
    MDC_HIP(c, launch_pyramid_level(src, d_levels[l - 1], w >> (l - 1), h >> (l - 1), nframes, s));
    src = d_levels[l - 1];
  }
  return MDC_OK;
} MDC_CATCH(c)

int mdc_process_pyramid_batch_device(mdc_ctx* c, const uint8_t* d_in, float* d_base, int levels, float* const* d_levels,
                                     int64_t nframes, unsigned flags, void* stream) try {
  if (!c) return MDC_ERR_ARG;
  if (!d_in || !d_base || nframes < 0 || levels < 1 || (levels > 1 && !d_levels))
    return fail(c, MDC_ERR_ARG, "mdc_process_pyramid_batch_device: bad argument");
  for (int l = 1; l < levels; l++)
    if (!d_levels[l - 1]) return fail(c, MDC_ERR_ARG, "level %d buffer is NULL", l);
  ReadLock lk(c->mu);
  DeviceGuard dg(c->device);
  hipStream_t s = (hipStream_t)stream;
  const bool rect = (flags & MDC_RECTIFY) != 0;
  const int w = rect ? c->out_w : (c->in_w > 0 ? c->in_w : c->rm_in_w), h = rect ? c->out_h : (c->in_h > 0 ? c->in_h : c->rm_in_h);
  float* pyr[3] = {levels > 1 ? d_levels[0] : nullptr, levels > 2 ? d_levels[1] : nullptr, levels > 3 ? d_levels[2] : nullptr};
  bool fused = false;
  int rc = enqueue_process(c, d_in, d_base, nframes, flags, s, levels > 1 ? pyr : nullptr, &fused);
  if (rc != MDC_OK) return rc;
  const int first = fused ? std::min(levels, 4) : 1;
  const float* src = first == 1 ? d_base : d_levels[first - 2];
  for (int l = first; l < levels; l++) {
    MDC_HIP(c, launch_pyramid_level(src, d_levels[l - 1], w >> (l - 1), h >> (l - 1), nframes, s));
    src = d_levels[l - 1];
  }
  return MDC_OK;
} MDC_CATCH(c)


int mdc_distort_points_device(mdc_ctx* c, const mdc_fov_model* model, float* d_x, float* d_y, int64_t n, void* stream) try {
  if (!c) return MDC_ERR_ARG;
  if (!model || n < 0 || (n > 0 && (!d_x || !d_y))) return fail(c, MDC_ERR_ARG, "mdc_distort_points_device: bad argument");
  ReadLock lk(c->mu);
  DeviceGuard dg(c->device);
  MDC_HIP(c, launch_distort_points(d_x, d_y, n, distort_model(model), (hipStream_t)stream));
  return MDC_OK;
} MDC_CATCH(c)


int mdc_gradients_batch_device(mdc_ctx* c, const float* d_level, int w, int h, float* d_dI, float* d_abs_squared_grad,
                               int64_t nframes, void* stream) try {
  if (!c) return MDC_ERR_ARG;
  if (!d_level || !d_dI || !d_abs_squared_grad || w < 1 || h < 1 || nframes < 0 || (int64_t)w * h >= (1ll << 31))
    return fail(c, MDC_ERR_ARG, "mdc_gradients_batch_device: bad argument");
  ReadLock lk(c->mu);
  DeviceGuard dg(c->device);
  MDC_HIP(c, launch_gradients(d_level, d_dI, d_abs_squared_grad, w, h, nframes, (hipStream_t)stream));
  return MDC_OK;
} MDC_CATCH(c)

int mdc_process_pyramid_gradients_batch_device(mdc_ctx* c, const uint8_t* d_in, float* d_base, int levels, float* const* d_levels,
                                               float* const* d_dI, float* const* d_abs_squared_grad, int64_t nframes, unsigned flags,
                                               int chunk_frames, void* stream) try {
  if (!c) return MDC_ERR_ARG;
  if (!d_in || !d_base || nframes < 0 || levels < 1 || levels > 8 || (levels > 1 && !d_levels) || !d_dI || !d_abs_squared_grad || chunk_frames < 0)
    return fail(c, MDC_ERR_ARG, "mdc_process_pyramid_gradients_batch_device: bad argument");
  for (int l = 0; l < levels; l++)
    if ((l && !d_levels[l - 1]) || !d_dI[l] || !d_abs_squared_grad[l]) return fail(c, MDC_ERR_ARG, "level %d has a NULL buffer", l);
  ReadLock lk(c->mu);
  DeviceGuard dg(c->device);
  return enqueue_pyramid_gradients(c, d_in, d_base, levels, d_levels, d_dI, d_abs_squared_grad, nframes, flags, chunk_frames, (hipStream_t)stream);
} MDC_CATCH(c)

int mdc_vcal_plane_step_device(mdc_ctx* c, const float* d_images, const float* d_p2x, const float* d_p2y, int n_images, int w, int h,
                               int n_plane, float* d_plane_color, const float* d_vignette_factor, int oth2, float* d_ff,
                               float* d_fc, double* d_er, void* stream) try {
  if (!c) return MDC_ERR_ARG;
  if (!d_images || !d_p2x || !d_p2y || !d_plane_color || !d_vignette_factor || !d_ff || !d_fc || !d_er || n_images < 0 || w < 2 ||
      h < 2 || n_plane < 0 || (long long)w * h >= (1ll << 31))
    return fail(c, MDC_ERR_ARG, "mdc_vcal_plane_step_device: bad argument");
  ReadLock lk(c->mu);
  DeviceGuard dg(c->device);
  MDC_HIP(c, launch_vcal_plane_step(d_images, d_p2x, d_p2y, n_images, w, h, n_plane, d_plane_color, d_vignette_factor, oth2, d_ff,
                                    d_fc, d_er, (hipStream_t)stream));
  return MDC_OK;
} MDC_CATCH(c)

int mdc_vcal_vignette_step_device(mdc_ctx* c, const float* d_images, const float* d_p2x, const float* d_p2y, int n_images, int w,
                                  int h, int n_plane, const float* d_plane_color, float* d_vignette_factor, int oth2, float* d_tt,
                                  float* d_ct, double* d_er, void* stream) try {
// ... 38 lines not shown

int64_t mdc_vcal_index_bytes(const mdc_vcal_index* index) { return index ? mdc::vcal_index_bytes(index->ix) : 0; }
int64_t mdc_vcal_index_entries(const mdc_vcal_index* index) { return index ? mdc::vcal_index_entries(index->ix) : 0; }

int mdc_vcal_vignette_step_indexed_device(mdc_ctx* c, const mdc_vcal_index* index, const float* d_plane_color,
                                          float* d_vignette_factor, int oth2, float* d_tt, float* d_ct, double* d_er, void* stream) try {
  if (!c) return MDC_ERR_ARG;
  if (!index || !d_plane_color || !d_vignette_factor || !d_tt || !d_ct || !d_er)
    return fail(c, MDC_ERR_ARG, "mdc_vcal_vignette_step_indexed_device: bad argument");
  if (index->device != c->device) return fail(c, MDC_ERR_ARG, "mdc_vcal_vignette_step_indexed_device: index built on another device");
  ReadLock lk(c->mu);
  DeviceGuard dg(c->device);
  MDC_HIP(c, mdc::launch_vcal_vignette_step_indexed(index->ix, d_plane_color, d_vignette_factor, oth2, d_tt, d_ct, d_er,
                                                    c->d_vcal_max + (c->vcal_max_next++ % mdc_ctx::kVcalMaxWords), (hipStream_t)stream));
  return MDC_OK;
} MDC_CATCH(c)

int mdc_vcal_scale_images_device(mdc_ctx* c, float* d_images, int n_images, int64_t npix, float mean_exposure,
                                 const float* d_exposure_times, void* stream) try {
  if (!c) return MDC_ERR_ARG;
  if (n_images < 0 || n_images > 65535 || npix < 0 || (n_images > 0 && npix > 0 && (!d_images || !d_exposure_times)))
    return fail(c, MDC_ERR_ARG, "mdc_vcal_scale_images_device: bad argument");
  ReadLock lk(c->mu);
  DeviceGuard dg(c->device);
  MDC_HIP(c, launch_vcal_scale_images(d_images, n_images, npix, mean_exposure, d_exposure_times, (hipStream_t)stream));
  return MDC_OK;
} MDC_CATCH(c)

int mdc_vcal_gradient_mask_device(mdc_ctx* c, float* d_images, int n_images, int w, int h, int max_abs_grad, void* stream) try {
  if (!c) return MDC_ERR_ARG;
  if (n_images < 0 || (n_images > 0 && !d_images) || w < 1 || h < 1 || (long long)w * h >= (1ll << 31) || max_abs_grad < 0)
    return fail(c, MDC_ERR_ARG, "mdc_vcal_gradient_mask_device: bad argument");
  ReadLock lk(c->mu);
  DeviceGuard dg(c->device);
  MDC_HIP(c, launch_vcal_gradient_mask(d_images, n_images, w, h, max_abs_grad, (hipStream_t)stream));
  return MDC_OK;
} MDC_CATCH(c)

int mdc_vcal_mask_coords_device(mdc_ctx* c, float* d_x, float* d_y, int64_t n, int w, int h, void* stream) try {
  if (!c) return MDC_ERR_ARG;
  if (n < 0 || (n > 0 && (!d_x || !d_y)) || w < 1 || h < 1) return fail(c, MDC_ERR_ARG, "mdc_vcal_mask_coords_device: bad argument");
  ReadLock lk(c->mu);
  DeviceGuard dg(c->device);
  MDC_HIP(c, launch_vcal_mask_coords(d_x, d_y, n, w, h, (hipStream_t)stream));
  return MDC_OK;
} MDC_CATCH(c)

int mdc_vcal_plane_coords_device(mdc_ctx* c, const mdc_fov_model* model, const float* d_corners, float* d_hk, int n, int gw, int gh,
                                 float facw, float fach, float* d_p2x, float* d_p2y, void* stream) try {
  if (!c) return MDC_ERR_ARG;
  if (n < 0 || n > 65535 || gw < 1 || gh < 1 || (long long)gw * gh >= (1ll << 31) ||
      (n > 0 && (!d_hk || !d_p2x || !d_p2y)) || (model && (model->in_w < 1 || model->in_h < 1)))
    return fail(c, MDC_ERR_ARG, "mdc_vcal_plane_coords_device: bad argument");
  ReadLock lk(c->mu);
  DeviceGuard dg(c->device);
  DistortModel m;
  if (model) m = distort_model(model);
  MDC_HIP(c, launch_vcal_plane_coords(d_corners, d_hk, n, gw, gh, facw, fach, model ? &m : nullptr, model ? model->in_w : 0,
                                      model ? model->in_h : 0, d_p2x, d_p2y, (hipStream_t)stream));
  return MDC_OK;
} MDC_CATCH(c)

int mdc_vcal_smooth_device(mdc_ctx* c, const float* d_vignette_factor, int w, int h, float* d_smoothed, float* d_scratch,
                           void* stream) try {
  if (!c) return MDC_ERR_ARG;
  if (!d_vignette_factor || !d_smoothed || !d_scratch || w < 1 || h < 1 || (long long)w * h >= (1ll << 31) ||
      d_smoothed == d_scratch || d_vignette_factor == d_scratch)
    return fail(c, MDC_ERR_ARG, "mdc_vcal_smooth_device: bad argument");
  ReadLock lk(c->mu);
  DeviceGuard dg(c->device);
  MDC_HIP(c, launch_vcal_smooth(d_vignette_factor, w, h, d_smoothed, d_scratch, (hipStream_t)stream));
  return MDC_OK;
} MDC_CATCH(c)

int mdc_vcal_plot_plane_device(mdc_ctx* c, const float* d_plane, int gw, int gh, uint8_t* d_rgb, float* range_host, void* stream) try {
  if (!c) return mdc_device_count() > 0 ? MDC_ERR_ARG : MDC_ERR_NO_DEVICE;
  if (!d_plane || !d_rgb || !range_host || gw < 1 || gh < 1 || (long long)gw * gh >= (1ll << 31))
    return fail(c, MDC_ERR_ARG, "mdc_vcal_plot_plane_device: bad argument");
  ReadLock lk(c->mu);
  DeviceGuard dg(c->device);
  MDC_HIP(c, launch_vcal_plot_plane(d_plane, (long long)gw * gh, d_rgb, range_host, (hipStream_t)stream));
  return MDC_OK;
} MDC_CATCH(c)

int mdc_vcal_vignette_u16_device(mdc_ctx* c, const float* d_vignette, int64_t n, uint16_t* d_out, void* stream) try {
  if (!c) return mdc_device_count() > 0 ? MDC_ERR_ARG : MDC_ERR_NO_DEVICE;
  if (n < 0 || (n > 0 && (!d_vignette || !d_out)) || ((uintptr_t)d_out & 1) || ((uintptr_t)d_vignette & 3))
    return fail(c, MDC_ERR_ARG, "mdc_vcal_vignette_u16_device: bad argument");
  ReadLock lk(c->mu);
  DeviceGuard dg(c->device);
  MDC_HIP(c, launch_vcal_vignette_u16(d_vignette, n, d_out, (hipStream_t)stream));
  return MDC_OK;
} MDC_CATCH(c)

int mdc_vcal_solve_device(mdc_ctx* c, const float* d_images, const float* d_p2x, const float* d_p2y, int n_images, int w, int h,
                          int n_plane, float* d_plane_color, float* d_vignette_factor, int max_iterations, int outlier_th,
                          double* er_out, void* stream) try {
  if (!c) return MDC_ERR_ARG;
  if (!d_plane_color || !d_vignette_factor || max_iterations < 0 || outlier_th < 0 || outlier_th > 46340)
    return fail(c, MDC_ERR_ARG, "mdc_vcal_solve_device: bad argument");
  if (max_iterations == 0) return MDC_OK;
  mdc_vcal_index* index = nullptr;
  int rc = mdc_vcal_index_create(c, d_images, d_p2x, d_p2y, n_images, w, h, n_plane, stream, &index);
  if (rc != MDC_OK) return rc;
  ReadLock lk(c->mu);
  DeviceGuard dg(c->device);
  hipStream_t s = (hipStream_t)stream;
  float *d_ff = nullptr, *d_fc = nullptr, *d_tt = nullptr, *d_ct = nullptr;
  double* d_er = nullptr;
  const size_t plane_bytes = (size_t)std::max(n_plane, 1) * sizeof(float), img_bytes = (size_t)w * h * sizeof(float);
  const size_t er_bytes = (size_t)max_iterations * 4 * sizeof(double);
  auto done = [&](int code) {
    (void)hipStreamSynchronize(s);
    for (void* p : {(void*)d_ff, (void*)d_fc, (void*)d_tt, (void*)d_ct, (void*)d_er}) (void)hipFree(p);
    mdc_vcal_index_destroy(index);
    return code;
  };
#define MDC_SOLVE(call_)                                                  \
  do {                                                                    \
    hipError_t e_ = (call_);                                              \
    if (e_ != hipSuccess) return done(fail(c, MDC_ERR_HIP, "%s: %s", #call_, hipGetErrorString(e_))); \
  } while (0)
  MDC_SOLVE(hipMalloc(&d_ff, plane_bytes));
  MDC_SOLVE(hipMalloc(&d_fc, plane_bytes));
  MDC_SOLVE(hipMalloc(&d_tt, img_bytes));
  MDC_SOLVE(hipMalloc(&d_ct, img_bytes));
  MDC_SOLVE(hipMalloc(&d_er, er_bytes));
  for (int it = 0; it < max_iterations; it++) {
    const int oth2 = it < max_iterations / 2 ? 10000 * 10000 : outlier_th * outlier_th;
    MDC_SOLVE(launch_vcal_plane_step(d_images, d_p2x, d_p2y, n_images, w, h, n_plane, d_plane_color, d_vignette_factor, oth2, d_ff,
                                     d_fc, d_er + 4 * it, s));
    MDC_SOLVE(mdc::launch_vcal_vignette_step_indexed(index->ix, d_plane_color, d_vignette_factor, oth2, d_tt, d_ct, d_er + 4 * it + 2,
                                                     c->d_vcal_max + (c->vcal_max_next++ % mdc_ctx::kVcalMaxWords), s));
  }
  if (er_out) MDC_SOLVE(hipMemcpyAsync(er_out, d_er, er_bytes, hipMemcpyDeviceToHost, s));
#undef MDC_SOLVE
  return done(MDC_OK);
} MDC_CATCH(c)

int mdc_tune_device(mdc_ctx* c, const uint8_t* d_in, float* d_out, int64_t nframes, unsigned flags, void* stream,
                    mdc_tune_result* result) try {
  if (!c) return MDC_ERR_ARG;
  if (!d_in || !d_out || nframes <= 0) return fail(c, MDC_ERR_ARG, "mdc_tune_device: bad argument");
  WriteLock lk(c->mu);
  DeviceGuard dg(c->device);
  if (!(flags & MDC_RECTIFY) || !c->valid_remap) return fail(c, MDC_ERR_STATE, "mdc_tune_device: needs a remap and MDC_RECTIFY");
  hipStream_t s = (hipStream_t)stream;
  static const TileShape shapes[] = {{128, 16}, {64, 32}, {128, 32}};
  static const int fpbs[] = {32, 64, 96, 128};
  hipEvent_t e0, e1;
  MDC_HIP(c, hipEventCreate(&e0));
  MDC_HIP(c, hipEventCreate(&e1));
  float best = 1e30f;
  int bw = 0, bh = 0, bf = 0, tried = 0;
  int rc = MDC_OK;
  const int caller_fpb = c->opt_fpb;
  for (const TileShape& sh : shapes) {
    c->opt_tile_w = sh.w;
    c->opt_tile_h = sh.h;
    if (hipDeviceSynchronize() != hipSuccess) {
      rc = fail(c, MDC_ERR_HIP, "mdc_tune_device: hipDeviceSynchronize failed");
      break;
    }
    if ((rc = plan_tiles(c)) != MDC_OK) break;
    if (!c->plan[0].tiled) continue;
    for (int fpb : fpbs) {
      c->opt_fpb = fpb;
      float ms[5];
      bool ok = true;
      for (int k = 0; k < 7 && ok; k++) {
        if (k >= 2) ok = hipEventRecord(e0, s) == hipSuccess;
        ok = ok && enqueue_process(c, d_in, d_out, nframes, flags, s) == MDC_OK;
        if (k >= 2) ok = ok && hipEventRecord(e1, s) == hipSuccess && hipEventSynchronize(e1) == hipSuccess &&
                         hipEventElapsedTime(&ms[k - 2], e0, e1) == hipSuccess;
      }
      if (!ok) continue;
      std::sort(ms, ms + 5);
      tried++;
      if (ms[2] < best) {
        best = ms[2];
        bw = sh.w;
        bh = sh.h;
        bf = fpb;
      }
    }
  }
  (void)hipEventDestroy(e0);
  (void)hipEventDestroy(e1);
  (void)hipDeviceSynchronize();
  c->opt_tile_w = bw;
  c->opt_tile_h = bh;
  c->opt_fpb = caller_fpb;
  c->tuned_fpb = bf;
  c->tuned_min_frames = bf ? std::max<int64_t>(nframes / 4, (int64_t)bf * 8) : 0;
  const int rc2 = plan_tiles(c);
  if (rc == MDC_OK) rc = rc2;
  if (result) {
    result->tile_w = bw;
    result->tile_h = bh;
    result->frames_per_block = bf;
    result->ms = tried ? best : 0.f;
    result->candidates = tried;
  }
  return rc;
} MDC_CATCH(c)

int mdc_tune_placement_device(mdc_ctx* c, const uint8_t* const* d_in, int n_in, float* const* d_out, int n_out, int64_t nframes, unsigned flags,
                              void* stream, int* best_in, int* best_out, float* ms_out) try {
  if (!c) return MDC_ERR_ARG;
  if (!d_in || !d_out || n_in < 1 || n_out < 1 || (int64_t)n_in * n_out > 256 || nframes <= 0 || !best_in || !best_out)
    return fail(c, MDC_ERR_ARG, "mdc_tune_placement_device: bad argument");
  for (int k = 0; k < n_in; k++)
    if (!d_in[k]) return fail(c, MDC_ERR_ARG, "mdc_tune_placement_device: input candidate %d is NULL", k);
  for (int k = 0; k < n_out; k++)
    if (!d_out[k]) return fail(c, MDC_ERR_ARG, "mdc_tune_placement_device: output candidate %d is NULL", k);
  ReadLock lk(c->mu);
  DeviceGuard dg(c->device);
  hipStream_t s = (hipStream_t)stream;
  hipEvent_t e0, e1;
  MDC_HIP(c, hipEventCreate(&e0));
  if (hipEventCreate(&e1) != hipSuccess) {
    (void)hipEventDestroy(e0);
    return fail(c, MDC_ERR_HIP, "hipEventCreate failed");
  }
  int rc = MDC_OK, bi = 0, bo = 0;
  float best = 1e30f;
  for (int i = 0; i < n_in && rc == MDC_OK; i++)
    for (int j = 0; j < n_out && rc == MDC_OK; j++) {
      float ms[5] = {0, 0, 0, 0, 0};
      for (int k = 0; k < 7 && rc == MDC_OK; k++) {
        bool ok = k < 2 || hipEventRecord(e0, s) == hipSuccess;
        if (ok) rc = enqueue_process(c, d_in[i], d_out[j], nframes, flags, s);
        if (rc != MDC_OK) break;
        if (k >= 2) ok = ok && hipEventRecord(e1, s) == hipSuccess && hipEventSynchronize(e1) == hipSuccess && hipEventElapsedTime(&ms[k - 2], e0, e1) == hipSuccess;
        if (!ok) rc = fail(c, MDC_ERR_HIP, "mdc_tune_placement_device: timing a launch failed");
      }
      if (rc != MDC_OK) break;
      std::sort(ms, ms + 5);
      if (ms_out) ms_out[(size_t)i * n_out + j] = ms[2];
      if (ms[2] < best) {
        best = ms[2];
        bi = i;
        bo = j;
      }
    }
  (void)hipStreamSynchronize(s);
  (void)hipEventDestroy(e0);
  (void)hipEventDestroy(e1);
  *best_in = bi;
  *best_out = bo;
  return rc;
} MDC_CATCH(c)

int mdc_describe_launch(mdc_ctx* c, unsigned flags, int pyramid_levels, char* buf, size_t cap) try {
  if (!c || !buf || cap == 0) return MDC_ERR_ARG;
  ReadLock lk(c->mu);
  bool g, v, o;
  normalise(c, flags, g, v, o);
  char tmp[160];
  if (pyramid_levels == -1) {
    if (!c->valid_remap) return fail(c, MDC_ERR_STATE, "no remap set (UndistorterFOV invalid)");
    const mdc_ctx::SrcPlan& p = c->plan[1];
    if (p.tiled && c->opt_kernel != MDC_KERNEL_GATHER)
      snprintf(tmp, sizeof tmp, "remap_tiled_kernel<false, %s, false, true, %d, %d, %d>", c->n_black > 0 ? "true" : "false", p.tile_w,
               tile_threads(p.tile_w, p.tile_h), p.nbuf);
    else snprintf(tmp, sizeof tmp, "remap_gather_f32_kernel");
  } else if (!(flags & MDC_RECTIFY)) {
    const int fw = c->in_w > 0 ? c->in_w : c->rm_in_w, fh = c->in_h > 0 ? c->in_h : c->rm_in_h;
    snprintf(tmp, sizeof tmp, "%s<%s>", ((int64_t)fw * fh) % 4 == 0 ? "unmap_xpose_kernel" : "unmap_scalar_kernel", v ? "true" : "false");
  } else if (!c->valid_remap) {
    return fail(c, MDC_ERR_STATE, "no remap set (UndistorterFOV invalid)");
  } else if (c->strip.planned && c->opt_kernel != MDC_KERNEL_GATHER) {
    const bool pyr = pyramid_levels > 1 && c->out_w % kStripTileW == 0;
    snprintf(tmp, sizeof tmp, "remap_strip_kernel<%s, %s, %d, %d, %d>", v ? "true" : "false", pyr ? "true" : "false", c->strip.nbuf,
             c->strip.passes, kStripWaves);
  } else if (c->plan[0].tiled && c->opt_kernel != MDC_KERNEL_GATHER) {
    const mdc_ctx::SrcPlan& p = c->plan[0];
    const bool pyr = pyramid_levels > 1 && p.tile_w * p.tile_h <= 2048 && p.tile_h % 8 == 0 && c->out_w % p.tile_w == 0 && c->out_h % p.tile_h == 0 &&
                     tiled_lds_bytes(p.win_bytes, p.nbuf, true) + tiled_pyramid_lds_bytes(p.tile_w, p.tile_h) <= kLdsPerCU;
    snprintf(tmp, sizeof tmp, "remap_tiled_kernel<%s, %s, %s, false, %d, %d, %d>", v ? "true" : "false",
             c->n_black > 0 ? "true" : "false", pyr ? "true" : "false", p.tile_w, tile_threads(p.tile_w, p.tile_h), p.nbuf);
  } else {
    snprintf(tmp, sizeof tmp, "remap_gather_u8_kernel<%s>", v ? "true" : "false");
  }
  if (strlen(tmp) + 1 > cap) return fail(c, MDC_ERR_ARG, "mdc_describe_launch: buffer too small");
  memcpy(buf, tmp, strlen(tmp) + 1);
  return MDC_OK;
} MDC_CATCH(c)

int mdc_synchronize(mdc_ctx* c) try {
  if (!c) return MDC_ERR_ARG;
  ReadLock lk(c->mu);
  DeviceGuard dg(c->device);
  std::vector<hipStream_t> streams;
  {
    std::lock_guard<std::mutex> sl(c->slot_mu);
    for (mdc_ctx::HostSlot* h : c->slots) streams.push_back(h->stream);
  }
  for (int k = 0; k < 2; k++)
    if (c->pipe_stream[k]) streams.push_back(c->pipe_stream[k]);
  if (c->pipe_up_stream) streams.push_back(c->pipe_up_stream);
  for (hipStream_t st : streams) MDC_HIP(c, hipStreamSynchronize(st));
  return MDC_OK;
} MDC_CATCH(c)












int mdc_jpeg_huffman_batch_device(mdc_ctx* c, const void* d_streams, int64_t stream_stride, void* d_records, int64_t record_bytes, int w, int h,
                                  int blocks_w, int blocks_rows, int64_t nframes, int* d_status, void* stream) try {
  if (!c) return MDC_ERR_ARG;
  if (!d_streams || !d_records || !d_status || nframes < 0 || w <= 0 || h <= 0) return fail(c, MDC_ERR_ARG, "mdc_jpeg_huffman_batch_device: bad argument");
  ReadLock lk(c->mu);
  DeviceGuard dg(c->device);
  void* scratch = nullptr;
  hipStream_t s = (hipStream_t)stream;
  if (jpeg_huffman_segments(nframes) > 1 && hipMallocAsync(&scratch, jpeg_huffman_scratch_bytes(nframes), s) != hipSuccess) {
    (void)hipGetLastError();
    scratch = nullptr;
  }
  const hipError_t e = launch_jpeg_huffman(d_streams, stream_stride, d_records, record_bytes, w, h, blocks_w, blocks_rows, nframes, d_status, s, 7u, scratch);
  if (scratch) (void)hipFreeAsync(scratch, s);
  MDC_HIP(c, e);
  return MDC_OK;
} MDC_CATCH(c)

int mdc_jpeg_idct_batch_device(mdc_ctx* c, const void* d_records, int64_t record_bytes, uint8_t* d_frames, int w, int h, int blocks_w,
                               int blocks_rows, int64_t nframes, void* stream) try {
  if (!c) return MDC_ERR_ARG;
  if (!d_records || !d_frames || nframes < 0 || w <= 0 || h <= 0) return fail(c, MDC_ERR_ARG, "mdc_jpeg_idct_batch_device: bad argument");
  ReadLock lk(c->mu);
  DeviceGuard dg(c->device);
  MDC_HIP(c, launch_jpeg_idct(d_records, record_bytes, d_frames, w, h, blocks_w, blocks_rows, nframes, (hipStream_t)stream));
  return MDC_OK;
} MDC_CATCH(c)


int mdc_export_tables(mdc_ctx* c, void* blob, size_t cap, size_t* size) try {
  if (!c || !size) return MDC_ERR_ARG;
  ReadLock lk(c->mu);
  const size_t nv = c->valid_vignette ? c->h_vinv.size() : 0;
  const size_t nr = c->valid_remap ? c->h_rx.size() : 0;
  const size_t need = sizeof(BlobHeader) + 256 * 4 + nv * 4 + 2 * nr * 4;
  *size = need;
  if (!blob) return MDC_OK;
  if (cap < need) return fail(c, MDC_ERR_ARG, "export buffer too small (%zu < %zu)", cap, need);
  BlobHeader h{kMagic, 1, c->in_w, c->in_h, c->rm_in_w, c->rm_in_h, c->out_w, c->out_h,
// ... 57 lines not shown
```

### mono_dataset_code_amd/csrc/mdc_ctx.h

```cpp
#pragma once
#include "../../include/mdc_hip.h"
#include "mdc_internal.h"

#include <algorithm>
#include <atomic>
#include <chrono>
#include <cmath>
#include <condition_variable>
#include <cstdarg>
#include <cstdio>
#include <cstdlib>
#include <cstring>
#include <limits>
#include <map>
#include <mutex>
#include <new>
#include <shared_mutex>
#include <string>
#include <vector>

struct mdc_ctx {
  int device = 0;
  std::shared_timed_mutex mu;
  mutable std::mutex err_mu;
  std::string err;
  std::mutex pin_mu, pipe_mu;

  struct HostSlot {
    hipStream_t stream = nullptr;
    void* d_in = nullptr;
    size_t in_cap = 0;
    float* d_out = nullptr;
    size_t out_cap = 0;
    hipEvent_t ev_fork = nullptr, ev_join = nullptr;
    bool busy = false;
  };
  static constexpr int kMaxSlots = 8;
  std::mutex slot_mu;
  std::condition_variable slot_cv;
  std::vector<HostSlot*> slots;

  int in_w = 0, in_h = 0;
  bool valid_gamma = false, valid_vignette = false;
  std::vector<float> h_ginv;
  std::vector<float> h_vinv;
  float* d_luts = nullptr;
  float* d_vinv = nullptr;

  bool valid_remap = false;
  int rm_in_w = 0, rm_in_h = 0, out_w = 0, out_h = 0;
  std::vector<float> h_rx, h_ry;
  float *d_rx = nullptr, *d_ry = nullptr;

  struct SrcPlan {
    uint32_t* d_chunks = nullptr;
    int* d_nch = nullptr;
    uint32_t* d_taps = nullptr;
    int* d_order = nullptr;
    int chunk_cap = 0, win_bytes = 0, nbuf = 2;
    int tile_w = 0, tile_h = 0, n_tiles = 0, tiles_x = 0, n_blocks = 0;
    bool tiled = false;
    int64_t staged_bytes = 0;
  } plan[2];
  struct Strip {
    uint32_t* d_chunks = nullptr;
    int* d_nch = nullptr;
    uint32_t* d_taps = nullptr;
    int* d_order = nullptr;
    int n_blocks = 0, n_tiles = 0, tiles_x = 0, win_bytes = 0, passes = 0, nbuf = 2;
    bool planned = false;
    int64_t staged_bytes = 0;
  } strip;
  int bbox[4] = {0, 0, -1, -1};
  int64_t n_black = 0;

  int opt_kernel = MDC_KERNEL_AUTO;
  int opt_fpb = 0;
  int tuned_fpb = 0;
  int64_t tuned_min_frames = 0;
  int opt_tile_h = 0;
  int opt_tile_w = 0;
  int opt_order = MDC_ORDER_BANDS;
  int opt_xcd_rotate = 1;
  int opt_nbuf = 0;
  int opt_interleave = 0;
  int opt_pin_caller = 0;
  int opt_taper = 0;
  int opt_zero_copy = 0;
  int opt_prefetch_streams = 0;
  int opt_prefetch_chunk = 0;
  int opt_dev_chunk = 0;
  int opt_dev_chunk_hint = 0;
  int opt_two_stage = 0;

  struct Pinned {
    const void* p = nullptr;
    size_t bytes = 0;
    bool ok = false;
    uint64_t used = 0;
  };
  std::vector<Pinned> pinned;
  const void* pin_candidate[2] = {nullptr, nullptr};
  size_t pin_candidate_bytes[2] = {0, 0};
  uint64_t pin_clock = 0;

  hipStream_t pipe_stream[2] = {nullptr, nullptr};
  hipEvent_t pipe_done[2] = {nullptr, nullptr};
  hipEvent_t pipe_dec[2] = {nullptr, nullptr};
  hipStream_t pipe_up_stream = nullptr;
  hipEvent_t pipe_up[2] = {nullptr, nullptr};
  hipEvent_t pipe_huff[2] = {nullptr, nullptr};
  uint8_t* d_pipe_in[2] = {nullptr, nullptr};
  float* d_pipe_out[2] = {nullptr, nullptr};
  void* d_pipe_rec[2] = {nullptr, nullptr};
  void* d_pipe_strm[2] = {nullptr, nullptr};
  int* d_pipe_status[2] = {nullptr, nullptr};
  void* d_pipe_seg[2] = {nullptr, nullptr};
  int* h_pipe_status = nullptr;
  size_t pipe_status_cap = 0;
  int pipe_chunk_cap = 0;
  size_t pipe_in_cap = 0, pipe_out_cap = 0, pipe_rec_cap = 0, pipe_strm_cap = 0;

  std::mutex striped_mu;
  std::map<void*, void*> striped;

  static constexpr int kVcalMaxWords = 256;
  unsigned* d_vcal_max = nullptr;
  std::atomic<unsigned> vcal_max_next{0};

};
using ReadLock = std::shared_lock<std::shared_timed_mutex>;
using WriteLock = std::unique_lock<std::shared_timed_mutex>;

namespace mdc {

int fail(mdc_ctx* c, int code, const char* fmt, ...);

#define MDC_HIP(c, call)                                                                      \
  do {                                                                                        \
    hipError_t e_ = (call);                                                                   \
    if (e_ != hipSuccess) return fail((c), MDC_ERR_HIP, "%s: %s", #call, hipGetErrorString(e_)); \
  } while (0)

struct DeviceGuard {
  int prev = -1;
  explicit DeviceGuard(int dev) {
    if (hipGetDevice(&prev) != hipSuccess) prev = -1;
    if (prev != dev) (void)hipSetDevice(dev);
    else prev = -1;
  }
  ~DeviceGuard() {
    if (prev >= 0) (void)hipSetDevice(prev);
  }
};

#define MDC_CATCH(c_)                                                                    \
  catch (const std::bad_alloc&) {                                                        \
    return fail((c_), MDC_ERR_NOMEM, "out of host memory");                              \
  }                                                                                      \
  catch (const std::exception& e_) {                                                     \
    return fail((c_), MDC_ERR_HIP, "unexpected exception: %s", e_.what());               \
  }                                                                                      \
  catch (...) {                                                                          \
    return fail((c_), MDC_ERR_HIP, "unexpected exception");                              \
  }

void normalise(const mdc_ctx* c, unsigned flags, bool& g, bool& v, bool& o);
const float* lut_for(const mdc_ctx* c, bool g, bool o);
int frames_per_block(const mdc_ctx* c, int64_t nframes, int blocks_per_group, int target_wgs = 4800);
TilePlan tile_plan(const mdc_ctx* c, int which);
RemapArgs remap_args(const mdc_ctx* c, const float* lut, const float* vinv);
int enqueue_process(mdc_ctx* c, const uint8_t* d_in, float* d_out, int64_t nframes, unsigned flags, hipStream_t s, float* const* pyr = nullptr,
                    bool* pyr_done = nullptr);
int enqueue_pyramid_gradients(mdc_ctx* c, const uint8_t* d_in, float* d_base, int levels, float* const* d_levels, float* const* d_dI,
                              float* const* d_abs_squared_grad, int64_t nframes, unsigned flags, int chunk_frames, hipStream_t s);
int enqueue_undistort_f32(mdc_ctx* c, const float* d_in, float* d_out, int64_t nframes, hipStream_t s);
DistortModel distort_model(const mdc_fov_model* f);

int plan_tiles(mdc_ctx* c);
void free_plan(mdc_ctx* c);

void maybe_pin(mdc_ctx* c, int role, const void* p, size_t bytes);
void unpin_all(mdc_ctx* c);
const void* device_view_raw(const mdc_ctx* c, const void* p, size_t bytes);
template <class T>
T* device_view(const mdc_ctx* c, T* p, size_t bytes) {
  return (T*)device_view_raw(c, (const void*)p, bytes);
}
bool one_host_allocation(const void* p, size_t bytes);
int ensure_stage(mdc_ctx* c, mdc_ctx::HostSlot* h, size_t in_bytes, size_t out_bytes);

struct SlotLease {
  mdc_ctx* c;
  mdc_ctx::HostSlot* s = nullptr;
  explicit SlotLease(mdc_ctx* ctx, bool wait = true);
  bool in_flight = true;
  void drained() { in_flight = false; }
  ~SlotLease();
  SlotLease(const SlotLease&) = delete;
  SlotLease& operator=(const SlotLease&) = delete;
};

}
```

### mono_dataset_code_amd/csrc/mdc_internal.h

```cpp
#pragma once
#include <hip/hip_runtime.h>
#include <stdint.h>

#include "fov_point_model.h"
#include "mdc_build_config.h"
#include "xcd_placement.h"

namespace mdc {

struct TileShape {
  int w, h;
};
constexpr TileShape kTileShapes[] = {{64, 16}, {64, 32}, {64, 60}, {64, 64}, {128, 16}, {128, 32}};
constexpr bool tile_shape_ok(int w, int h) {
  for (const TileShape& t : kTileShapes)
    if (t.w == w && t.h == h) return true;
  return false;
}
constexpr int tile_rpt(int w, int h) { return w >= 320 ? 8 : 4; }
constexpr int tile_threads(int w, int h) { return w * h / tile_rpt(w, h); }
constexpr int kTileMaxChunks = 3;
constexpr int kTileMaxChunksF32 = 4;
constexpr int kLutRep = MDC_EXP_LUT_REP;
constexpr uint32_t kOutside = 0xfffffff0u;

struct RemapArgs {
  const float* lut;
  const float* vinv;
  const float* rx;
  const float* ry;
  int in_w, in_h, out_w, out_h;
};

struct TilePlan {
  const uint32_t* d_chunks;
  const int* d_nch;
  const uint32_t* d_taps;
  const int* d_order;
  int n_blocks;
  int n_tiles, tiles_x;
  int tile_w;
  int tile_h;
  int chunk_cap;
  int win_bytes;
  int nbuf;
  bool has_black;
  bool interleave;
  bool taper = true;
  bool rotate = false;
};

constexpr int kStripTileW = 128, kStripTileH = 8;
constexpr int kStripChunkCap = 128;
constexpr int kStripWaves = MDC_EXP_STRIP_WAVES;
struct StripPlan {
  const uint32_t* d_chunks;
  const int* d_nch;
  const uint32_t* d_taps;
  const int* d_order;
  int n_blocks, n_tiles, tiles_x;
  int win_bytes;
  int passes;
  int nbuf;
  bool interleave;
  bool rotate = false;
};
#if MDC_EXP_STRIP_FAKE_GRAD
extern float* g_fake_grad_dI;
extern float* g_fake_grad_abs;
#endif
hipError_t launch_remap_strip_u8(const uint8_t* d_in, float* d_out, const RemapArgs& a, const StripPlan& p, int64_t nframes, int fpb,
                                 hipStream_t s, float* d_l1 = nullptr, float* d_l2 = nullptr, float* d_l3 = nullptr);
size_t strip_lds_bytes(int win_bytes, int nbuf, int waves);

hipError_t launch_unmap(const uint8_t* d_in, float* d_out, const float* d_lut, const float* d_vinv, int64_t npix,
                        int64_t nframes, int fpb, hipStream_t s);

hipError_t launch_remap_gather_u8(const uint8_t* d_in, float* d_out, const RemapArgs& a, int64_t nframes, int fpb,
                                  hipStream_t s);
hipError_t launch_remap_gather_f32(const float* d_in, float* d_out, const RemapArgs& a, int64_t nframes, int fpb,
                                   hipStream_t s);
hipError_t launch_remap_tiled_u8(const uint8_t* d_in, float* d_out, const RemapArgs& a, const TilePlan& p,
                                 int64_t nframes, int fpb, hipStream_t s, float* d_l1 = nullptr, float* d_l2 = nullptr,
                                 float* d_l3 = nullptr);
hipError_t launch_remap_tiled_f32(const float* d_in, float* d_out, const RemapArgs& a, const TilePlan& p,
                                  int64_t nframes, int fpb, hipStream_t s);
size_t tiled_lds_bytes(int win_bytes, int nbuf, bool lut = true);
size_t tiled_pyramid_lds_bytes(int tile_w, int tile_h);
constexpr size_t kLdsPerCU = 160 * 1024;

hipError_t launch_prefetch_rows(const uint8_t* d_frames, int64_t frame_bytes, int row_pitch, int x0, int x1, int y0, int y1, int64_t nframes,
                                uint32_t* d_sink, hipStream_t s);

hipError_t launch_pyramid_level(const float* d_src, float* d_dst, int w, int h, int64_t nframes, hipStream_t s);

hipError_t launch_distort_points(float* d_x, float* d_y, int64_t n, const DistortModel& m, hipStream_t s);

hipError_t launch_vcal_plane_step(const float* d_images, const float* d_p2x, const float* d_p2y, int n, int wI, int hI, int np,
                                  float* d_plane_color, const float* d_vig, int oth2, float* d_ff, float* d_fc, double* d_er,
                                  hipStream_t s);
hipError_t launch_vcal_vignette_step(const float* d_images, const float* d_p2x, const float* d_p2y, int n, int wI, int hI, int np,
                                     const float* d_plane_color, float* d_vig, int oth2, float* d_tt, float* d_ct, double* d_er,
                                     unsigned* d_max_bits, hipStream_t s);

struct VcalIndex;
hipError_t vcal_index_build(const float* d_images, const float* d_p2x, const float* d_p2y, int n, int wI, int hI, int np,
                            hipStream_t s, VcalIndex** out);
void vcal_index_free(VcalIndex* ix);
long long vcal_index_bytes(const VcalIndex* ix);
long long vcal_index_entries(const VcalIndex* ix);
hipError_t launch_vcal_vignette_step_indexed(const VcalIndex* ix, const float* d_plane_color, float* d_vig, int oth2, float* d_tt,
                                             float* d_ct, double* d_er, unsigned* d_max_bits, hipStream_t s);

hipError_t launch_vcal_scale_images(float* d_images, int n, int64_t npix, float mean_exposure, const float* d_exposure, hipStream_t s);
hipError_t launch_vcal_gradient_mask(float* d_images, int n, int wI, int hI, int max_abs_grad, hipStream_t s);
hipError_t launch_vcal_mask_coords(float* d_x, float* d_y, int64_t n, int wI, int hI, hipStream_t s);
hipError_t launch_vcal_plane_coords(const float* d_corners, float* d_hk, int n, int gw, int gh, float facw, float fach,
                                    const DistortModel* m, int wI, int hI, float* d_p2x, float* d_p2y, hipStream_t s);
hipError_t launch_vcal_smooth(const float* d_vig, int wI, int hI, float* d_tt, float* d_ct, hipStream_t s);
hipError_t launch_vcal_plot_plane(const float* d_plane, long long n, uint8_t* d_rgb, float* range_host, hipStream_t s);
hipError_t launch_vcal_vignette_u16(const float* d_vignette, int64_t n, uint16_t* d_out, hipStream_t s);

hipError_t launch_jpeg_huffman(const void* d_streams, int64_t stream_stride, void* d_records, int64_t record_bytes, int w, int h, int blocks_w,
                               int blocks_rows, int64_t nframes, int* d_status, hipStream_t s, unsigned kinds = 7u, void* d_scratch = nullptr);
size_t jpeg_huffman_scratch_bytes(int64_t nframes);
int jpeg_huffman_segments(int64_t nframes);
hipError_t launch_jpeg_idct(const void* d_records, int64_t record_bytes, uint8_t* d_frames, int w, int h, int blocks_w, int blocks_rows,
                            int64_t nframes, hipStream_t s);

hipError_t launch_gradients(const float* d_level, float* d_dI, float* d_abs2, int w, int h, int64_t nframes, hipStream_t s);
hipError_t launch_gradients_levels(int n_levels, const float* const* d_src, float* const* d_dI, float* const* d_abs2, const int* w,
                                   const int* h, int64_t nframes, hipStream_t s);

}
```

### mono_dataset_code_amd/csrc/mdc_kernels.hip

```cpp
#include "mdc_internal.h"

namespace mdc {

namespace {

constexpr int kLutBytes = 256 * kLutRep * 4;
#if MDC_DEBUG_BOUNDS
#define MDC_CHECK(cond)               \
  do {                                \
    if (!(cond)) __builtin_trap();    \
  } while (0)
#else
#define MDC_CHECK(cond) \
  do {                  \
  } while (0)
#endif

typedef float f32x4 __attribute__((ext_vector_type(4)));

template <int NT>
__device__ __forceinline__ void fill_lut(float* s_lut, const float* __restrict__ lut, int tid) {
  constexpr int N = 256 * (kLutRep / 4);
  constexpr int IT = (N + NT - 1) / NT;
  float v[IT];
// ... 350 lines not shown
    }
  __builtin_amdgcn_sched_barrier(0);
#endif
}

template <int N>
__device__ __forceinline__ void wait_vm_barrier() {
  static_assert(N >= 0 && N < 64, "vmcnt is 6 bits");
  asm volatile("s_waitcnt vmcnt(%0) lgkmcnt(0)\n\ts_barrier" ::"n"(N) : "memory");
}
#if MDC_EXP_TIMING
__device__ __forceinline__ unsigned long long exp_now() {
  unsigned long long t;
  asm volatile("s_memtime %0\n\ts_waitcnt lgkmcnt(0)" : "=s"(t)::"memory");
  return t;
}
#endif
#if MDC_EXP_TIMING
template <int N>
__device__ __forceinline__ void wait_vm_only() {
  asm volatile("s_waitcnt vmcnt(%0) lgkmcnt(0)" ::"n"(N) : "memory");
}
template <int D, int R, int S = 4>
__device__ __forceinline__ void frame_wait_only(int rw) {
  if (R >= 4 && rw >= 4) wait_vm_only<(D - 1) * (4 + S) + S>();
  else if (R >= 3 && rw == 3) wait_vm_only<(D - 1) * (3 + S) + S>();
  else if (R >= 2 && rw == 2) wait_vm_only<(D - 1) * (2 + S) + S>();
  else if (rw == 1) wait_vm_only<(D - 1) * (1 + S) + S>();
  else wait_vm_only<S>();
}
#endif
template <int D, int R, int S = 4>
__device__ __forceinline__ void frame_barrier(int rw) {
  if constexpr (D == 1) {
    (void)rw;
    wait_vm_barrier<S>();
    return;
  }
  if (R >= 4 && rw >= 4) wait_vm_barrier<(D - 1) * (4 + S) + S>();
  else if (R >= 3 && rw == 3) wait_vm_barrier<(D - 1) * (3 + S) + S>();
  else if (R >= 2 && rw == 2) wait_vm_barrier<(D - 1) * (2 + S) + S>();
  else if (rw == 1) wait_vm_barrier<(D - 1) * (1 + S) + S>();
  else wait_vm_barrier<S>();
}

template <bool VIG, bool BLACK, bool PYR, bool F32, int R, int TW, int NT, int NBUF, int RPT>
__device__ __forceinline__ void tile_frames(const TileThread<RPT>& t, const uint8_t* __restrict__ src,
                                            float* __restrict__ dst, uint32_t in_bytes, uint32_t out_bytes,
                                            int nframes, int nch, const uint32_t (&goff_all)[F32 ? kTileMaxChunksF32 : kTileMaxChunks],
                                            lds_u8_ptr s_win, int win_bytes, lds_f32_ptr my_lut, int tid,
                                            const PyramidOut& py, long long f_first, int fstep, uint32_t p3byte,
                                            uint32_t row_bytes) {
  constexpr int D = NBUF - 1;
  const long long in_step = (long long)fstep * in_bytes;
  const long long out_step = (long long)fstep * (out_bytes / 4);
  uint32_t goff[R];
#pragma unroll
  for (int k = 0; k < R; k++) goff[k] = goff_all[k];
  const int wave = __builtin_amdgcn_readfirstlane(tid >> 6);
  int rw = 0;
#pragma unroll
  for (int k = 0; k < R; k++) rw += (wave * 64 + k * NT < nch) ? 1 : 0;
  lds_u8_ptr w[NBUF];
#pragma unroll
  for (int i = 0; i < NBUF; i++) w[i] = s_win + i * win_bytes;
  const int last = nframes - 1;
#pragma unroll
  for (int d = 0; d < D; d++) {
#if MDC_EXP_SKIP_LOAD
    stage_window<R, NT>(src, in_bytes, w[d], goff, wave, rw);
#else
    stage_window<R, NT>(src + min(d, last) * in_step, in_bytes, w[d], goff, wave, rw);
#endif
  }
  if (R >= 4 && rw >= 4) wait_vm_barrier<(D - 1) * 4>();
  else if (R >= 3 && rw == 3) wait_vm_barrier<(D - 1) * 3>();
  else if (R >= 2 && rw == 2) wait_vm_barrier<(D - 1) * 2>();
  else if (rw == 1) wait_vm_barrier<(D - 1) * 1>();
  else wait_vm_barrier<0>();
  constexpr int G = NT / TW;
  constexpr bool LEAN = (NT >= 960 && (NBUF != 2 || BLACK || PYR || F32)) || RPT > 4;
  static_assert(!PYR || RPT == 4, "the fused pyramid pairs the 4 rows of a thread");
  constexpr int L2W = TW / 4;
  float* s_pyr = (float*)(s_win + NBUF * win_bytes);
  const int pyr_slot = (wave / (TW / 64)) * L2W + (wave % (TW / 64)) * 16;
  const uint32_t l1_bytes = out_bytes / 4, l2_bytes = out_bytes / 16, l3_bytes = out_bytes / 64;
  const bool pyr_all_levels = PYR && py.l1 && py.l2;
#if MDC_EXP_TIMING
  unsigned long long tp[4] = {0, 0, 0, 0};
  const unsigned long long t_begin = exp_now();
#endif
  const uint8_t* stg = src + (long long)min(D, last) * in_step;
  for (int f = 0; f <= last; f++) {
#if MDC_EXP_TIMING
    const unsigned long long t0 = exp_now();
#endif
    if (PYR && f > 0)
      pyramid_level3<G, TW>(py, f_first + (long long)(f - 1) * fstep, l3_bytes, s_pyr + ((f - 1) & 1) * G * L2W, p3byte, tid - (NT - 64));
#if MDC_EXP_SKIP_LOAD
    stage_window<R, NT>(src, in_bytes, w[D], goff, wave, rw);
#else
    stage_window<R, NT>(stg, in_bytes, w[D], goff, wave, rw);
    if (f + D < last) stg += in_step;
#endif
#if MDC_EXP_TIMING
    const unsigned long long t1 = exp_now();
#endif
    float res[RPT];
#if MDC_EXP_PAD_VALU
    {
      int pad_v = tid;
#pragma unroll
      for (int q = 0; q < MDC_EXP_PAD_VALU; q++) asm volatile("v_add_u32 %0, %0, %0" : "+v"(pad_v));
    }
#endif
    tile_compute<VIG, BLACK, F32, LEAN, ((LEAN || PYR) ? 2 : 4), RPT>(t, w[0], my_lut, dst, out_bytes, row_bytes, res, win_bytes);
    if constexpr (PYR)
      pyramid_levels12(t, res, py, f_first + (long long)f * fstep, l1_bytes, l2_bytes, s_pyr + (f & 1) * G * L2W + pyr_slot,
                       tid & 63);
    dst += out_step;
#if MDC_EXP_TIMING
    const unsigned long long t2 = exp_now();
    if (PYR && pyr_all_levels) frame_wait_only<D, R, 6>(rw);
    else frame_wait_only<D, R, RPT>(rw);
    const unsigned long long t3 = exp_now();
    asm volatile("s_barrier" ::: "memory");
    const unsigned long long t4 = exp_now();
    tp[0] += t1 - t0;
    tp[1] += t2 - t1;
    tp[2] += t3 - t2;
    tp[3] += t4 - t3;
#else
    if (D > 1 && f < D - 1) wait_vm_barrier<RPT>();
    else if (PYR && pyr_all_levels) frame_barrier<D, R, 6>(rw);
    else frame_barrier<D, R, RPT>(rw);
#endif
    lds_u8_ptr x = w[0];
#pragma unroll
    for (int i = 0; i < D; i++) w[i] = w[i + 1];
    w[D] = x;
  }
  if (PYR) pyramid_level3<G, TW>(py, f_first + (long long)last * fstep, l3_bytes, s_pyr + (last & 1) * G * L2W, p3byte, tid - (NT - 64));
#if MDC_EXP_TIMING
  if ((tid & 63) == 0 && (wave == 0 || wave == 5) && blockIdx.x % 41 == 3 && blockIdx.y % 7 == 2)
    printf("TIMING block %d,%d wave %d frames %d cycles/frame: issue %.0f compute+stores %.0f vmwait %.0f barrier %.0f total %.0f\n",
           (int)blockIdx.x, (int)blockIdx.y, wave, nframes, (double)tp[0] / nframes, (double)tp[1] / nframes, (double)tp[2] / nframes,
           (double)tp[3] / nframes, (double)(exp_now() - t_begin) / nframes);
#endif
}

template <bool VIG, bool BLACK, bool PYR, bool F32, int TW, int NT, int NBUF>
__global__ __launch_bounds__(NT, (NT >= 960 ? 8 : NT == 640 ? 5 : NT == 512 ? (kLutRep < 32 ? 8 : 6) : 4)) void remap_tiled_kernel(
    const uint8_t* __restrict__ in, float* __restrict__ out, RemapArgs a, TilePlan p, PyramidOut py, int nframes, int fpb,
    int interleave, int taper_full, int taper_r) {
  constexpr int RPT = tile_rpt(TW, 0);
  extern __shared__ __attribute__((aligned(1024))) unsigned char smem[];
  float* s_lut = reinterpret_cast<float*>(smem);
  lds_u8_ptr s_win = (lds_u8_ptr)smem + (F32 ? 0 : kLutBytes);

  const int tile = p.d_order[xcd_table_entry((int)blockIdx.x, (int)blockIdx.y, p.rotate)];
  if (tile < 0) return;
  const int fstep = interleave ? (int)gridDim.y : 1;
  int f0 = interleave ? (int)blockIdx.y : (int)blockIdx.y * fpb;
  int nf = interleave ? (nframes - f0 + fstep - 1) / fstep : min(nframes, f0 + fpb) - f0;
  if (!interleave && taper_r > 0 && (int)blockIdx.y >= taper_full) {
    const int k = (int)blockIdx.y - taper_full;
    const int lvl = min(k / taper_r, 2);
    const int size = fpb >> (lvl + 1);
    f0 = taper_full * fpb + taper_r * (fpb - (fpb >> lvl)) + (k - lvl * taper_r) * size;
    nf = min(nframes, f0 + size) - f0;
  }
  if (nf <= 0) return;

  const int tid = threadIdx.x;
  const int lane_x = tid % TW;
  const int row0 = (tid / TW) * RPT;
  const int ox = (tile % p.tiles_x) * TW + lane_x;
  constexpr int kTileRows = NT * RPT / TW;
  constexpr bool LEAN = (NT >= 960 && (NBUF != 2 || BLACK || PYR || F32)) || RPT > 4;
  const int oy0 = (tile / p.tiles_x) * kTileRows + row0;

  const int nch = p.d_nch[tile];
  constexpr int RMAX = F32 ? kTileMaxChunksF32 : kTileMaxChunks;
  const uint32_t* chunks = p.d_chunks + (size_t)tile * (RMAX * NT);
  uint32_t goff[RMAX];
#pragma unroll
  for (int k = 0; k < RMAX; k++) goff[k] = chunks[tid + k * NT];

  float xx[RPT], yy[RPT];
  uint32_t tp[RPT];
#pragma unroll
  for (int j = 0; j < RPT; j++) {
    const bool inside = (ox < a.out_w) && (oy0 + j < a.out_h);
    const int oidx = inside ? (oy0 + j) * a.out_w + ox : 0;
    xx[j] = a.rx[oidx];
    yy[j] = a.ry[oidx];
    tp[j] = p.d_taps[oidx];
  }
  if (!F32) fill_lut<NT>(s_lut, a.lut, tid);
  lds_f32_ptr my_lut = (lds_f32_ptr)s_lut + (tid & (kLutRep - 1));

  TileThread<RPT> t;
#pragma unroll
  for (int j = 0; j < RPT; j++) {
    const int oy = oy0 + j;
    const bool inside = (ox < a.out_w) && (oy < a.out_h);
    const int oidx = oy * a.out_w + ox;
    if (LEAN) {
      if (j == 0) t.obyte[0] = ox < a.out_w ? (uint32_t)oidx * 4u : kOutsideLean;
    } else {
      t.obyte[j] = inside ? (uint32_t)oidx * 4u : kOutside;
    }
    if (!inside) {
      xx[j] = yy[j] = -1.f;
      tp[j] = 0;
    }
    if (PYR && j == 0)
      t.p1byte = (uint32_t)(((oy >> 1) + (lane_x & 1)) * (a.out_w >> 1) + (ox >> 1)) * 4u;
    if (PYR && j == 0) t.p2byte = (lane_x & 3) ? kOutside : (uint32_t)((oy >> 2) * (a.out_w >> 2) + (ox >> 2)) * 4u;
    t.black[j] = xx[j] < 0;
    t.bl[j] = bilin_of(t.black[j] ? 0.f : xx[j], t.black[j] ? 0.f : yy[j]);
    t.fx[j] = (t.black[j] ? 0.f : xx[j]) - (float)t.bl[j].xi;
    t.fy[j] = (t.black[j] ? 0.f : yy[j]) - (float)t.bl[j].yi;
    t.tap[j] = tp[j];
    t.off0[j] = (int)(tp[j] & 0xffffu);
    t.off1[j] = (int)(tp[j] >> 16);
  }
#pragma unroll
  for (int j = 0; j < RPT; j++) {
    t.v00[j] = t.v10[j] = t.v01[j] = t.v11[j] = 1.f;
    if (VIG) {
      const int s = t.black[j] ? 0 : t.bl[j].xi + t.bl[j].yi * a.in_w;
      t.v00[j] = a.vinv[s];
      t.v10[j] = a.vinv[s + 1];
      t.v01[j] = a.vinv[s + a.in_w];
      t.v11[j] = a.vinv[s + a.in_w + 1];
    }
  }

  const uint32_t in_bytes = (uint32_t)a.in_w * (uint32_t)a.in_h * (F32 ? 4u : 1u);
  const uint32_t out_bytes = (uint32_t)a.out_w * (uint32_t)a.out_h * 4u;
  const uint8_t* src = in + (long long)f0 * in_bytes;
  float* dst = out + (long long)f0 * (out_bytes / 4);
  static_assert(!PYR || (TW / 8) * (kTileRows / 8) <= 64, "level 3 of a tile is one wave's work");
  const int u3 = tid - (NT - 64);
  uint32_t p3byte = kOutside;
  if (PYR && u3 >= 0 && u3 < (TW / 8) * (kTileRows / 8))
    p3byte = (uint32_t)(((tile / p.tiles_x) * (kTileRows / 8) + u3 / (TW / 8)) * (a.out_w >> 3) + (tile % p.tiles_x) * (TW / 8) +
                        u3 % (TW / 8)) * 4u;
  if (nch == 0) {
#if __HIP_DEVICE_COMPILE__
    for (int f = 0; f < nf; f++, dst += (long long)fstep * (out_bytes / 4)) {
      const auto ro = MDC_FRAME_RSRC(dst, out_bytes);
#pragma unroll
      for (int j = 0; j < RPT; j++)
        __builtin_amdgcn_raw_buffer_store_b32(0u, ro, LEAN ? t.obyte[0] + (uint32_t)j * (uint32_t)a.out_w * 4u : t.obyte[j], 0, 0);
      if (PYR) {
        const long long fa = (long long)f0 + (long long)f * fstep;
        if (py.l1) {
          const auto r1 = MDC_FRAME_RSRC(py.l1 + fa * (out_bytes / 16), out_bytes / 4);
          __builtin_amdgcn_raw_buffer_store_b32(0u, r1, t.p1byte, 0, 0);
        }
        if (py.l2) __builtin_amdgcn_raw_buffer_store_b32(0u, MDC_FRAME_RSRC(py.l2 + fa * (out_bytes / 64), out_bytes / 16), t.p2byte, 0, 0);
        if (py.l3) __builtin_amdgcn_raw_buffer_store_b32(0u, MDC_FRAME_RSRC(py.l3 + fa * (out_bytes / 256), out_bytes / 64), p3byte, 0, 0);
      }
    }
#endif
    return;
  }
  const int rounds = (nch + NT - 1) / NT;
  MDC_CHECK(nch * 16 <= p.win_bytes && rounds <= RMAX && (goff[0] == kOutside) == (tid >= nch));
#define MDC_TILE_RUN(R_)                                                                                              \
  tile_frames<VIG, BLACK, PYR, F32, R_, TW, NT, NBUF, RPT>(t, src, dst, in_bytes, out_bytes, nf, nch, goff, s_win, p.win_bytes, \
                                             my_lut, tid, py, (long long)f0, fstep, p3byte, (uint32_t)a.out_w * 4u)
  if (rounds == 1) MDC_TILE_RUN(1);
  else if (rounds == 2) MDC_TILE_RUN(2);
  else if (rounds == 3 || !F32) MDC_TILE_RUN(3);
  else if constexpr (F32) MDC_TILE_RUN(4);
#undef MDC_TILE_RUN
}

template <int N>
__device__ __forceinline__ void wait_vm() {
  static_assert(N >= 0 && N < 64, "vmcnt is 6 bits");
  asm volatile("s_waitcnt vmcnt(%0)" ::"n"(N) : "memory");
}
template <typename T>
__device__ __forceinline__ T* uniform_ptr(T* p) {
  const unsigned long long v = reinterpret_cast<unsigned long long>(p);
  const unsigned lo = __builtin_amdgcn_readfirstlane((unsigned)v), hi = __builtin_amdgcn_readfirstlane((unsigned)(v >> 32));
  return reinterpret_cast<T*>(((unsigned long long)hi << 32) | lo);
}

constexpr int kStripLutRep = MDC_EXP_STRIP_LUT_REP;
constexpr int kStripLutBytes = 256 * kStripLutRep * 4;
constexpr int kStripCap = kStripChunkCap;
constexpr int kStripPad = 64;

template <int NT, int REP>
__device__ __forceinline__ void fill_lut_rep(float* s_lut, const float* __restrict__ lut, int tid) {
  constexpr int N = 256 * (REP / 4);
  constexpr int IT = (N + NT - 1) / NT;
  float v[IT];
#pragma unroll
  for (int k = 0; k < IT; k++) v[k] = lut[min(tid + k * NT, N - 1) / (REP / 4)];
#pragma unroll
  for (int k = 0; k < IT; k++)
    if (IT * NT == N || tid + k * NT < N) reinterpret_cast<f32x4*>(s_lut)[tid + k * NT] = f32x4{v[k], v[k], v[k], v[k]};
}

template <int CTRL>
__device__ __forceinline__ float dpp_row(float v) {
  return __int_as_float(__builtin_amdgcn_update_dpp(0, __float_as_int(v), CTRL, 0xf, 0xf, false));
}

template <bool VIG, bool PYR, int NBUF, int P, int W>
__global__ __launch_bounds__(64 * W, ((PYR || P > 5 || NBUF > 2) ? MDC_EXP_STRIP_WAVES_PER_EU - 1 : MDC_EXP_STRIP_WAVES_PER_EU)) void remap_strip_kernel(const uint8_t* __restrict__ in, float* __restrict__ out, RemapArgs a,
                                                            StripPlan p, PyramidOut py, int nframes, int fpb, int interleave) {
#if __HIP_DEVICE_COMPILE__
  extern __shared__ __attribute__((aligned(1024))) unsigned char smem[];
  const int win = p.win_bytes;
  const int per_wave = (4 + NBUF) * win + kStripPad;
  float* s_lut = reinterpret_cast<float*>(smem + W * per_wave);
  const int tid = threadIdx.x, lane = tid & 63;
// ... 237 lines not shown
              tt[3 * lane + 0] = res[u0 + u];
              tt[3 * lane + 1] = res[u0 + u] * 0.5f;
              tt[3 * lane + 2] = res[u0 + u] * 0.25f;
              __builtin_amdgcn_wave_barrier();
              const auto rg = MDC_FRAME_RSRC(uniform_ptr(py.gI + fa * (long long)(out_bytes / 4) * 3), out_bytes * 3u);
              const uint32_t rowoff = (uint32_t)(((ty * 8 + (int)R) * a.out_w + tx * 128 + 64 * h) * 12);
#pragma unroll
              for (int k3 = 0; k3 < 3; k3++)
                __builtin_amdgcn_raw_buffer_store_b32(__float_as_uint(tt[k3 * 64 + lane]), rg, rowoff + (uint32_t)(k3 * 64 + lane) * 4u, 0, kStoreAux);
              __builtin_amdgcn_wave_barrier();
              const auto ra = MDC_FRAME_RSRC(uniform_ptr(py.gA + fa * (long long)(out_bytes / 4)), out_bytes);
              __builtin_amdgcn_raw_buffer_store_b32(__float_as_uint(res[u0 + u] * res[u0 + u]), ra, vo[h], R * row_bytes, kStoreAux);
            }
#endif
          }
        }
#if MDC_EXP_STRIP_FAKE_GRAD
        if (py.gI && q == 0) {
          float dummy = 0.f;
#pragma unroll
          for (int e = 0; e < (h == 0 ? 3 : 2); e++) {
            uint32_t b0, b1;
            asm volatile("v_add_u32_sdwa %0, %1, %2 dst_sel:DWORD dst_unused:UNUSED_PAD src0_sel:DWORD src1_sel:WORD_0" : "=v"(b0) : "v"(f_base), "v"(tap[8 * h + e]));
            asm volatile("v_add_u32_sdwa %0, %1, %2 dst_sel:DWORD dst_unused:UNUSED_PAD src0_sel:DWORD src1_sel:WORD_1" : "=v"(b1) : "v"(f_base), "v"(tap[8 * h + e]));
            lds_f32_ptr t0 = reinterpret_cast<lds_f32_ptr>((lds_u8_ptr)0 + b0);
            lds_f32_ptr t1 = reinterpret_cast<lds_f32_ptr>((lds_u8_ptr)0 + b1);
            Bilin bw;
            float xxyy, omx;
            asm volatile("v_mul_f32 %0, %1, %2" : "=v"(xxyy) : "v"(fx[8 * h + e]), "v"(fy[8 * h + e]));
            asm volatile("v_sub_f32 %0, 1.0, %1" : "=v"(omx) : "v"(fx[8 * h + e]));
            bw.w11 = xxyy;
            bw.w01 = fy[8 * h + e] - xxyy;
            bw.w10 = fx[8 * h + e] - xxyy;
            bw.w00 = (omx - fy[8 * h + e]) + xxyy;
            dummy += bilin_sum(bw, t0[0], t0[1], t1[0], t1[1]);
          }
          if (dummy == -1.2345e30f) __builtin_amdgcn_raw_buffer_store_b32(__float_as_uint(dummy), ro, vo[h], 0, kStoreAux);
        }
#endif
        if (PYR) {
          float v1[2];
#pragma unroll
          for (int pp = 0; pp < 2; pp++) {
            const float b = dpp_quad<0xF5>(res[2 * pp]);
            const float d = dpp_quad<0xF5>(res[2 * pp + 1]);
            v1[pp] = box4(res[2 * pp], b, res[2 * pp + 1], d);
          }
          if (py.l1) {
            const auto r1 = MDC_FRAME_RSRC(uniform_ptr(py.l1 + fa * (l1_bytes / 4)), l1_bytes);
            const float left2 = dpp_quad<0xA0>(v1[1]);
            const float mm = (lane & 1) ? left2 : v1[0];
            __builtin_amdgcn_raw_buffer_store_b32(__float_as_uint(mm), r1, p1o[h], (uint32_t)q * row_bytes, kStoreAux);
          }
          const float b2 = dpp_quad<0xAA>(v1[0]);
          const float d2 = dpp_quad<0xAA>(v1[1]);
          v2[h][q] = box4(v1[0], b2, v1[1], d2);
        }
      }
    if (PYR) {
      if (py.l2) {
        const float a00 = dpp_quad<0x00>(v2[0][0]), a01 = dpp_quad<0x00>(v2[0][1]), a10 = dpp_quad<0x00>(v2[1][0]), a11 = dpp_quad<0x00>(v2[1][1]);
        const int j = lane & 3;
        const float mm = j == 0 ? a00 : j == 1 ? a01 : j == 2 ? a10 : a11;
        __builtin_amdgcn_raw_buffer_store_b32(__float_as_uint(mm), MDC_FRAME_RSRC(uniform_ptr(py.l2 + fa * (l2_bytes / 4)), l2_bytes), p2o, 0, kStoreAux);
      }
      if (py.l3) {
        float v3[2];
#pragma unroll
        for (int h = 0; h < 2; h++) v3[h] = box4(v2[h][0], dpp_row<0x104>(v2[h][0]), v2[h][1], dpp_row<0x104>(v2[h][1]));
        const float up = dpp_row<0x114>(v3[1]);
        const float mm = (lane & 4) ? up : v3[0];
        __builtin_amdgcn_raw_buffer_store_b32(__float_as_uint(mm), MDC_FRAME_RSRC(uniform_ptr(py.l3 + fa * (l3_bytes / 4)), l3_bytes), p3o, 0, kStoreAux);
      }
    }
    dst += out_step;
    ub = ub + 1 == NBUF ? 0 : ub + 1;
  }
#endif
}

__global__ __launch_bounds__(256) void pyramid_level_kernel(const float* __restrict__ src, float* __restrict__ dst,
                                                            int w, int h, long long nframes) {
  const int w2 = w >> 1, h2 = h >> 1;
  const long long n2 = (long long)w2 * h2;
  const long long i = (long long)blockIdx.x * 256 + threadIdx.x;
  if (i >= n2 * nframes) return;
  const long long f = i / n2;
  const int r = (int)(i - f * n2);
  const int y = r / w2, x = r - y * w2;
  const float* p = src + f * (long long)w * h + (long long)(2 * y) * w + 2 * x;
  dst[i] = 0.25f * (((p[0] + p[1]) + p[w]) + p[w + 1]);
}

__global__ __launch_bounds__(256) void distort_points_kernel(float* __restrict__ xs, float* __restrict__ ys, long long n,
                                                             DistortModel m) {
  const long long i = (long long)blockIdx.x * 256 + threadIdx.x;
  if (i >= n) return;
  float x = xs[i], y = ys[i];
  fov_distort_point(m, x, y);
  xs[i] = x;
  ys[i] = y;
}

inline int ceil_div(long long a, long long b) { return (int)((a + b - 1) / b); }

}

size_t tiled_lds_bytes(int win_bytes, int nbuf, bool lut) { return (lut ? (size_t)kLutBytes : 0) + (size_t)nbuf * win_bytes; }
size_t tiled_pyramid_lds_bytes(int tile_w, int tile_h) { return (size_t)2 * (tile_h / 4) * (tile_w / 4) * sizeof(float); }

hipError_t launch_unmap(const uint8_t* d_in, float* d_out, const float* d_lut, const float* d_vinv, int64_t npix,
                        int64_t nframes, int fpb, hipStream_t s) {
  if (nframes <= 0 || npix <= 0) return hipSuccess;
  const int groups = ceil_div(nframes, fpb);
  const bool vec = (npix % 4 == 0) && ((reinterpret_cast<uintptr_t>(d_in) & 3) == 0);
  if (vec) {
    dim3 grid(ceil_div(npix, 4096), groups);
    if (d_vinv) unmap_xpose_kernel<true><<<grid, 256, 0, s>>>(d_in, d_out, d_lut, d_vinv, npix, (int)nframes, fpb);
    else unmap_xpose_kernel<false><<<grid, 256, 0, s>>>(d_in, d_out, d_lut, d_vinv, npix, (int)nframes, fpb);
  } else {
    dim3 grid(ceil_div(npix, 256), groups);
    if (d_vinv) unmap_scalar_kernel<true><<<grid, 256, 0, s>>>(d_in, d_out, d_lut, d_vinv, npix, (int)nframes, fpb);
    else unmap_scalar_kernel<false><<<grid, 256, 0, s>>>(d_in, d_out, d_lut, d_vinv, npix, (int)nframes, fpb);
  }
  return hipGetLastError();
}

hipError_t launch_remap_gather_u8(const uint8_t* d_in, float* d_out, const RemapArgs& a, int64_t nframes, int fpb,
                                  hipStream_t s) {
  if (nframes <= 0) return hipSuccess;
  dim3 grid(ceil_div((long long)a.out_w * a.out_h, 256), ceil_div(nframes, fpb));
  if (a.vinv) remap_gather_u8_kernel<true><<<grid, 256, 0, s>>>(d_in, d_out, a, (int)nframes, fpb);
  else remap_gather_u8_kernel<false><<<grid, 256, 0, s>>>(d_in, d_out, a, (int)nframes, fpb);
  return hipGetLastError();
}

hipError_t launch_remap_gather_f32(const float* d_in, float* d_out, const RemapArgs& a, int64_t nframes, int fpb,
                                   hipStream_t s) {
  if (nframes <= 0) return hipSuccess;
  dim3 grid(ceil_div((long long)a.out_w * a.out_h, 256), ceil_div(nframes, fpb));
  remap_gather_f32_kernel<<<grid, 256, 0, s>>>(d_in, d_out, a, (int)nframes, fpb);
  return hipGetLastError();
}

struct TiledLaunch {
  const uint8_t* d_in;
  float* d_out;
  RemapArgs a;
  TilePlan p;
  PyramidOut py;
  int64_t nframes;
  int fpb;
  hipStream_t s;
};

static int taper_groups(int64_t nframes, int fpb, int taper_r, int* full) {
  *full = 0;
  if (taper_r <= 0) return (int)ceil_div(nframes, fpb);
  const int64_t tail = (int64_t)taper_r * (fpb / 2 + fpb / 4);
  *full = (int)((nframes - tail) / fpb);
  const int64_t rest = nframes - (int64_t)*full * fpb - tail;
  return *full + 2 * taper_r + (int)ceil_div(rest, fpb / 8);
}

template <bool VIG, bool BLACK, bool PYR, bool F32, int TW, int NT, int NBUF>
static hipError_t launch_tiled_variant(const TiledLaunch& l) {
  const size_t lds = tiled_lds_bytes(l.p.win_bytes, NBUF, !F32) + (PYR ? tiled_pyramid_lds_bytes(l.p.tile_w, l.p.tile_h) : 0);
  const int resident = 256 * (int)std::max<size_t>(1, std::min<size_t>(2048 / NT, kLdsPerCU / std::max<size_t>(lds, 1)));
  int taper_r = std::max(2, (resident + l.p.n_blocks / 2) / std::max(1, l.p.n_blocks));
  if (!l.p.taper || l.p.interleave || l.fpb % 8 != 0 || l.fpb < 16 || l.nframes < (int64_t)l.fpb * (4 * taper_r)) taper_r = 0;
  int taper_full = 0;
  dim3 grid(l.p.n_blocks, taper_groups(l.nframes, l.fpb, taper_r, &taper_full));
  if (lds > 64 * 1024) {
    hipError_t e = hipFuncSetAttribute(reinterpret_cast<const void*>(&remap_tiled_kernel<VIG, BLACK, PYR, F32, TW, NT, NBUF>),
                                       hipFuncAttributeMaxDynamicSharedMemorySize, (int)lds);
    if (e != hipSuccess) return e;
  }
  remap_tiled_kernel<VIG, BLACK, PYR, F32, TW, NT, NBUF><<<grid, NT, lds, l.s>>>(l.d_in, l.d_out, l.a, l.p, l.py, (int)l.nframes, l.fpb,
                                                                                 l.p.interleave ? 1 : 0, taper_full, taper_r);
  return hipGetLastError();
}

template <bool VIG, bool BLACK, bool PYR, bool F32, int TW, int NT>
static hipError_t launch_tiled_buf(const TiledLaunch& l) {
  constexpr int RPT = tile_rpt(TW, 0);
  switch (l.p.nbuf) {
    case 2:
      if constexpr (RPT == 4) return launch_tiled_variant<VIG, BLACK, PYR, F32, TW, NT, 2>(l);
      break;
    case 3: return launch_tiled_variant<VIG, BLACK, PYR, F32, TW, NT, 3>(l);
    case 4:
      if constexpr (NT <= 512) return launch_tiled_variant<VIG, BLACK, PYR, F32, TW, NT, 4>(l);
      break;
  }
  return hipErrorInvalidValue;
}

template <bool VIG, bool BLACK, bool PYR, bool F32>
static hipError_t launch_tiled_shape(const TiledLaunch& l) {
  switch (l.p.tile_w * 1000 + l.p.tile_h) {
    case 64016: return launch_tiled_buf<VIG, BLACK, PYR, F32, 64, 256>(l);
    case 64032: return launch_tiled_buf<VIG, BLACK, PYR, F32, 64, 512>(l);
    case 64060:
      if constexpr (!PYR) return launch_tiled_buf<VIG, BLACK, false, F32, 64, 960>(l);
      break;
    case 64064:
      if constexpr (!PYR) return launch_tiled_buf<VIG, BLACK, false, F32, 64, 1024>(l);
      break;
    case 128016: return launch_tiled_buf<VIG, BLACK, PYR, F32, 128, 512>(l);
    case 128032:
      if constexpr (!PYR) return launch_tiled_buf<VIG, BLACK, false, F32, 128, 1024>(l);
      break;
  }
  return hipErrorInvalidValue;
}

template <bool VIG, bool BLACK>
static hipError_t launch_tiled_nt(const TiledLaunch& l) {
  const bool pyr = l.py.l1 || l.py.l2 || l.py.l3;
  return pyr ? launch_tiled_shape<VIG, BLACK, true, false>(l) : launch_tiled_shape<VIG, BLACK, false, false>(l);
}

size_t strip_lds_bytes(int win_bytes, int nbuf, int waves) {
  return (size_t)waves * ((4 + nbuf) * win_bytes + kStripPad) + kStripLutBytes
#if MDC_EXP_STRIP_FAKE_GRAD
         + (size_t)waves * 1536
#endif
      ;
}
template <bool VIG, bool PYR, int NBUF, int P>
static hipError_t launch_strip_variant(const uint8_t* d_in, float* d_out, const RemapArgs& a, const StripPlan& p, const PyramidOut& py,
                                       int64_t nframes, int fpb, hipStream_t s) {
  constexpr int W = kStripWaves;
  dim3 grid(p.n_blocks, ceil_div(nframes, fpb));
  const size_t lds = strip_lds_bytes(p.win_bytes, NBUF, W);
  if (lds > 64 * 1024) {
    hipError_t e = hipFuncSetAttribute(reinterpret_cast<const void*>(&remap_strip_kernel<VIG, PYR, NBUF, P, W>),
                                       hipFuncAttributeMaxDynamicSharedMemorySize, (int)lds);
    if (e != hipSuccess) return e;
  }
  remap_strip_kernel<VIG, PYR, NBUF, P, W><<<grid, 64 * W, lds, s>>>(d_in, d_out, a, p, py, (int)nframes, fpb, p.interleave ? 1 : 0);
  return hipGetLastError();
}
template <bool VIG, bool PYR, int NBUF>
static hipError_t launch_strip_passes(const uint8_t* d_in, float* d_out, const RemapArgs& a, const StripPlan& p, const PyramidOut& py,
                                      int64_t nframes, int fpb, hipStream_t s) {
  switch (p.passes) {
    case 2: return launch_strip_variant<VIG, PYR, NBUF, 2>(d_in, d_out, a, p, py, nframes, fpb, s);
    case 3: return launch_strip_variant<VIG, PYR, NBUF, 3>(d_in, d_out, a, p, py, nframes, fpb, s);
    case 4: return launch_strip_variant<VIG, PYR, NBUF, 4>(d_in, d_out, a, p, py, nframes, fpb, s);
    case 5: return launch_strip_variant<VIG, PYR, NBUF, 5>(d_in, d_out, a, p, py, nframes, fpb, s);
    case 8: return launch_strip_variant<VIG, PYR, NBUF, 8>(d_in, d_out, a, p, py, nframes, fpb, s);
  }
  return hipErrorInvalidValue;
}
#if MDC_EXP_STRIP_FAKE_GRAD
float* g_fake_grad_dI = nullptr;
float* g_fake_grad_abs = nullptr;
#endif
hipError_t launch_remap_strip_u8(const uint8_t* d_in, float* d_out, const RemapArgs& a, const StripPlan& p, int64_t nframes, int fpb,
                                 hipStream_t s, float* d_l1, float* d_l2, float* d_l3) {
  if (nframes <= 0) return hipSuccess;
  if ((int64_t)a.in_w * a.in_h >= (int64_t)kOutside || (int64_t)a.out_w * (a.out_h + 8) * 4 >= 0xc0000000ll) return hipErrorInvalidValue;
#if MDC_EXP_STRIP_FAKE_GRAD
  const PyramidOut py{d_l1, d_l2, d_l3, g_fake_grad_dI, g_fake_grad_abs};
#else
  const PyramidOut py{d_l1, d_l2, d_l3};
#endif
  const bool pyr = d_l1 || d_l2 || d_l3;
#define MDC_STRIP(V_, P_)                                                                                        \
  (p.nbuf == 1   ? launch_strip_passes<V_, P_, 1>(d_in, d_out, a, p, py, nframes, fpb, s)                          \
   : p.nbuf == 2 ? launch_strip_passes<V_, P_, 2>(d_in, d_out, a, p, py, nframes, fpb, s)                          \
   : p.nbuf == 3 ? launch_strip_passes<V_, P_, 3>(d_in, d_out, a, p, py, nframes, fpb, s)                          \
                 : launch_strip_passes<V_, P_, 4>(d_in, d_out, a, p, py, nframes, fpb, s))
  if (a.vinv) return pyr ? MDC_STRIP(true, true) : MDC_STRIP(true, false);
  return pyr ? MDC_STRIP(false, true) : MDC_STRIP(false, false);
#undef MDC_STRIP
}

hipError_t launch_remap_tiled_u8(const uint8_t* d_in, float* d_out, const RemapArgs& a, const TilePlan& p,
                                 int64_t nframes, int fpb, hipStream_t s, float* d_l1, float* d_l2, float* d_l3) {
  if (nframes <= 0) return hipSuccess;
  if ((int64_t)a.in_w * a.in_h >= (int64_t)kOutside || (int64_t)a.out_w * a.out_h * 4 >= (int64_t)kOutside)
    return hipErrorInvalidValue;
  PyramidOut tiled_py{};
  tiled_py.l1 = d_l1, tiled_py.l2 = d_l2, tiled_py.l3 = d_l3;
  const TiledLaunch l{d_in, d_out, a, p, tiled_py, nframes, fpb, s};
  if (a.vinv) return p.has_black ? launch_tiled_nt<true, true>(l) : launch_tiled_nt<true, false>(l);
  return p.has_black ? launch_tiled_nt<false, true>(l) : launch_tiled_nt<false, false>(l);
}

hipError_t launch_remap_tiled_f32(const float* d_in, float* d_out, const RemapArgs& a, const TilePlan& p,
                                  int64_t nframes, int fpb, hipStream_t s) {
  if (nframes <= 0) return hipSuccess;
  if ((int64_t)a.in_w * a.in_h * 4 >= (int64_t)kOutside || (int64_t)a.out_w * a.out_h * 4 >= (int64_t)kOutside)
    return hipErrorInvalidValue;
  const TiledLaunch l{reinterpret_cast<const uint8_t*>(d_in), d_out, a, p, PyramidOut{}, nframes, fpb, s};
  return p.has_black ? launch_tiled_shape<false, true, false, true>(l) : launch_tiled_shape<false, false, false, true>(l);
}

__global__ __launch_bounds__(256) void prefetch_rows_kernel(const uint8_t* __restrict__ frames, long long frame_bytes, long long first_byte,
                                                            int row_pitch, int row16, long long rows, long long nframes,
                                                            uint32_t* __restrict__ sink) {
  typedef uint32_t u32x4_t __attribute__((ext_vector_type(4)));
  const long long per_frame = rows * row16, total = per_frame * nframes;
  uint32_t acc = 0;
  for (long long i = (long long)blockIdx.x * 256 + threadIdx.x; i < total; i += (long long)gridDim.x * 256) {
    const long long f = i / per_frame, r = i - f * per_frame;
    const long long row = r / row16, k = r - row * row16;
    const u32x4_t v = *reinterpret_cast<const u32x4_t*>(frames + f * frame_bytes + first_byte + row * row_pitch + k * 16);
    acc ^= v.x ^ v.y ^ v.z ^ v.w;
  }
  if (acc == 0x9e3779b9u && sink) *sink = acc;
}

hipError_t launch_prefetch_rows(const uint8_t* d_frames, int64_t frame_bytes, int row_pitch, int x0, int x1, int y0, int y1, int64_t nframes,
                                uint32_t* d_sink, hipStream_t s) {
  if (nframes <= 0 || y1 < y0 || x1 < x0) return hipSuccess;
  const int xa = x0 & ~127, xb = std::min(row_pitch, (x1 + 128) & ~127);
  if (xb - xa < 16 || (row_pitch & 15) != 0 || (reinterpret_cast<uintptr_t>(d_frames) & 15) != 0 || (frame_bytes & 15) != 0) return hipSuccess;
  prefetch_rows_kernel<<<4096, 256, 0, s>>>(d_frames, frame_bytes, (long long)y0 * row_pitch + xa, row_pitch, (xb - xa) / 16, (long long)(y1 - y0 + 1),
                                            nframes, d_sink);
  return hipGetLastError();
}

hipError_t launch_pyramid_level(const float* d_src, float* d_dst, int w, int h, int64_t nframes, hipStream_t s) {
  const long long n = (long long)(w >> 1) * (h >> 1) * nframes;
  if (n <= 0) return hipSuccess;
  pyramid_level_kernel<<<ceil_div(n, 256), 256, 0, s>>>(d_src, d_dst, w, h, nframes);
  return hipGetLastError();
}

hipError_t launch_distort_points(float* d_x, float* d_y, int64_t n, const DistortModel& m, hipStream_t s) {
  if (n <= 0) return hipSuccess;
  distort_points_kernel<<<ceil_div(n, 256), 256, 0, s>>>(d_x, d_y, n, m);
  return hipGetLastError();
}

}
```

### mono_dataset_code_amd/csrc/mdc_plan.hip

```cpp
#include "mdc_ctx.h"

namespace mdc {

void free_src_plan(mdc_ctx::SrcPlan& pl) {
  for (void** p : {(void**)&pl.d_chunks, (void**)&pl.d_nch, (void**)&pl.d_taps, (void**)&pl.d_order})
    if (*p) {
      (void)hipFree(*p);
      *p = nullptr;
    }
  pl.tiled = false;
  pl.staged_bytes = 0;
  pl.n_tiles = pl.tiles_x = pl.n_blocks = 0;
}

void free_strip_plan(mdc_ctx::Strip& st) {
  for (void** p : {(void**)&st.d_chunks, (void**)&st.d_nch, (void**)&st.d_taps, (void**)&st.d_order})
    if (*p) {
      (void)hipFree(*p);
      *p = nullptr;
    }
  st.planned = false;
  st.staged_bytes = 0;
  st.n_blocks = st.n_tiles = st.tiles_x = 0;
}

void free_plan(mdc_ctx* c) {
  for (auto& pl : c->plan) {
    free_src_plan(pl);
  }
  free_strip_plan(c->strip);
}

template <typename T>
int upload(mdc_ctx* c, T** dst, const std::vector<T>& v) {
  MDC_HIP(c, hipMalloc(dst, std::max<size_t>(v.size(), 1) * sizeof(T)));
  if (!v.empty()) MDC_HIP(c, hipMemcpy(*dst, v.data(), v.size() * sizeof(T), hipMemcpyHostToDevice));
  return MDC_OK;
}

int plan_source(mdc_ctx* c, int es, int kTileW, int kTileH, mdc_ctx::SrcPlan& pl) {
  const int ow = c->out_w, oh = c->out_h, iw = c->rm_in_w;
  const int kTileThreads = tile_threads(kTileW, kTileH);
  pl.staged_bytes = 0;
  const int tx = (ow + kTileW - 1) / kTileW, ty = (oh + kTileH - 1) / kTileH;
  const int n_tiles = tx * ty;
  const int ppc = 16 / es;
  const bool lut = es == 1;
  const char* why = "frame rows are not whole chunks / frame too large";
  bool ok = (iw % ppc == 0) && (int64_t)iw * c->rm_in_h * es < (int64_t)kOutside && (int64_t)ow * oh * 4 < (int64_t)kOutside;
  if (tile_rpt(kTileW, kTileH) != 4 && es != 1) ok = false;
  if ((kTileThreads >= 960 || tile_rpt(kTileW, kTileH) > 4) && (int64_t)ow * (oh + kTileH) * 4 >= 0xc0000000ll) ok = false;
  std::vector<std::vector<uint32_t>> chunks(n_tiles);
  std::vector<int> nch(n_tiles, 0);
  std::vector<uint32_t> taps((size_t)ow * oh, 0u);
  for (int t = 0; t < n_tiles && ok; t++) {
    const int bx = (t % tx) * kTileW, by = (t / tx) * kTileH;
    const int x1 = std::min(bx + kTileW, ow), y1 = std::min(by + kTileH, oh);
    int y_lo = std::numeric_limits<int>::max(), y_hi = -1;
    for (int y = by; y < y1; y++)
      for (int x = bx; x < x1; x++) {
        const float xx = c->h_rx[(size_t)y * ow + x], yy = c->h_ry[(size_t)y * ow + x];
        if (xx < 0) continue;
        y_lo = std::min(y_lo, (int)yy);
        y_hi = std::max(y_hi, (int)yy + 1);
      }
    if (y_hi < 0) continue;
    const int cpr = iw / ppc;
    const int nrows = y_hi - y_lo + 1;
    std::vector<int> pos((size_t)nrows * cpr, -1);
    for (int y = by; y < y1; y++)
      for (int x = bx; x < x1; x++) {
        const float xx = c->h_rx[(size_t)y * ow + x], yy = c->h_ry[(size_t)y * ow + x];
        if (xx < 0) continue;
        const int xi = (int)xx, yi = (int)yy;
        for (int dy = 0; dy < 2; dy++) {
          int* pr = &pos[(size_t)(yi + dy - y_lo) * cpr];
          pr[xi / ppc] = 0;
          pr[(xi + 1) / ppc] = 0;
        }
      }
    for (int k = 0; k < nrows; k++)
      for (int ch = 0; ch < cpr; ch++) {
        int& q = pos[(size_t)k * cpr + ch];
        if (q < 0) continue;
        q = (int)chunks[t].size();
        chunks[t].push_back((uint32_t)(((y_lo + k) * iw + ch * ppc) * es));
      }
    nch[t] = (int)chunks[t].size();
    if (nch[t] > (lut ? kTileMaxChunks : kTileMaxChunksF32) * kTileThreads || nch[t] * 16 > 65535) {
      ok = false;
      why = "a window has too many chunks";
    }
    pl.staged_bytes += (int64_t)nch[t] * 16;
    for (int y = by; y < y1 && ok; y++)
      for (int x = bx; x < x1; x++) {
        const float xx = c->h_rx[(size_t)y * ow + x], yy = c->h_ry[(size_t)y * ow + x];
        if (xx < 0) continue;
        const int xi = (int)xx, yi = (int)yy;
        const int p0 = pos[(size_t)(yi - y_lo) * cpr + xi / ppc], p1 = pos[(size_t)(yi + 1 - y_lo) * cpr + xi / ppc];
        taps[(size_t)y * ow + x] = (uint32_t)(p0 * 16 + (xi % ppc) * es) | ((uint32_t)(p1 * 16 + (xi % ppc) * es) << 16);
      }
  }
  const int cap = (lut ? kTileMaxChunks : kTileMaxChunksF32) * kTileThreads;
  int nch_max = 1;
  for (int t = 0; t < n_tiles; t++) nch_max = std::max(nch_max, nch[t]);
  const int win_bytes = (nch_max * 16 + 1023) & ~1023;
  const int wg_per_cu =
      std::max<int>(1, std::min<size_t>(kLdsPerCU / tiled_lds_bytes(win_bytes, 2, lut), 2048 / kTileThreads));
  const int nbuf_max = kTileThreads > 512 ? 3 : 4;
  int nbuf = 2;
  while (kTileThreads <= 512 && nbuf < nbuf_max && tiled_lds_bytes(win_bytes, nbuf + 1, lut) * wg_per_cu <= kLdsPerCU) nbuf++;
  if (c->opt_nbuf >= 2) nbuf = std::min(c->opt_nbuf, nbuf_max);
  if (tile_rpt(kTileW, kTileH) > 4) nbuf = 3;
  if (tiled_lds_bytes(win_bytes, nbuf, lut) > kLdsPerCU) {
    ok = false;
    why = "windows do not fit LDS";
  }
  if (!ok) {
    if (getenv("MDC_DEBUG_PLAN")) fprintf(stderr, "mdc plan %dx%d (element size %d): not plannable: %s\n", kTileW, kTileH, es, why);
    return MDC_OK;
  }
  std::vector<uint32_t> flat((size_t)n_tiles * cap, kOutside);
  for (int t = 0; t < n_tiles; t++) std::copy(chunks[t].begin(), chunks[t].end(), flat.begin() + (size_t)t * cap);
  int rc;
  if ((rc = upload(c, &pl.d_chunks, flat)) != MDC_OK || (rc = upload(c, &pl.d_nch, nch)) != MDC_OK ||
      (rc = upload(c, &pl.d_taps, taps)) != MDC_OK)
    return rc;
  const std::vector<int> order = tile_order(tx, ty, c->opt_order, c->opt_xcd_rotate != 0);
  if ((rc = upload(c, &pl.d_order, order)) != MDC_OK) return rc;
  pl.n_blocks = (int)order.size();
  pl.n_tiles = n_tiles;
  pl.tiles_x = tx;
  pl.tile_w = kTileW;
  pl.tile_h = kTileH;
  pl.chunk_cap = cap;
  pl.win_bytes = win_bytes;
  pl.nbuf = nbuf;
  pl.tiled = true;
  return MDC_OK;
}

int plan_strip(mdc_ctx* c) {
  mdc_ctx::Strip& st = c->strip;
  free_strip_plan(st);
  if (c->opt_two_stage == 2) return MDC_OK;
  const int ow = c->out_w, oh = c->out_h, iw = c->rm_in_w;
  constexpr int TW = kStripTileW, TH = kStripTileH;
  if (iw % 16 != 0 || oh % TH != 0 || (int64_t)iw * c->rm_in_h >= (int64_t)kOutside || (int64_t)ow * (oh + TH) * 4 >= 0xc0000000ll) return MDC_OK;
  const int tx = (ow + TW - 1) / TW, ty = oh / TH, n_tiles = tx * ty;
  std::vector<uint32_t> flat((size_t)n_tiles * kStripChunkCap, kOutside);
  std::vector<int> nch(n_tiles, 0);
  std::vector<uint32_t> taps((size_t)ow * oh, 0u);
  struct Row {
    int lo = std::numeric_limits<int>::max(), hi = -1, x0 = 0, lds = 0;
  };
  int nch_max = 1;
  int64_t staged = 0;
  for (int t = 0; t < n_tiles; t++) {
    const int bx = (t % tx) * TW, by = (t / tx) * TH;
    const int x1 = std::min(bx + TW, ow), y1 = by + TH;
    int y_lo = std::numeric_limits<int>::max(), y_hi = -1;
    for (int y = by; y < y1; y++)
      for (int x = bx; x < x1; x++) {
        const float xx = c->h_rx[(size_t)y * ow + x], yy = c->h_ry[(size_t)y * ow + x];
        if (xx < 0) continue;
        y_lo = std::min(y_lo, (int)yy);
        y_hi = std::max(y_hi, (int)yy + 1);
      }
    if (y_hi < 0) continue;
    std::vector<Row> rows(y_hi - y_lo + 1);
    for (int y = by; y < y1; y++)
      for (int x = bx; x < x1; x++) {
        const float xx = c->h_rx[(size_t)y * ow + x], yy = c->h_ry[(size_t)y * ow + x];
        if (xx < 0) continue;
        const int xi = (int)xx, yi = (int)yy;
        for (int dy = 0; dy < 2; dy++) {
          Row& r = rows[yi + dy - y_lo];
          r.lo = std::min(r.lo, xi);
          r.hi = std::max(r.hi, xi + 1);
        }
      }
    int n = 0;
    for (size_t k = 0; k < rows.size(); k++) {
      Row& r = rows[k];
      if (r.hi < 0) continue;
      r.x0 = r.lo - r.lo % 16;
      r.lds = n * 16;
      const int cnt = (r.hi - r.x0) / 16 + 1;
      if (r.x0 + cnt * 16 > iw || n + cnt > kStripChunkCap) return MDC_OK;
      for (int j = 0; j < cnt; j++) flat[(size_t)t * kStripChunkCap + n + j] = (uint32_t)((y_lo + (int)k) * iw + r.x0 + j * 16);
      n += cnt;
    }
    nch[t] = n;
    nch_max = std::max(nch_max, n);
    staged += (int64_t)n * 16;
    for (int y = by; y < y1; y++)
      for (int x = bx; x < x1; x++) {
        const float xx = c->h_rx[(size_t)y * ow + x], yy = c->h_ry[(size_t)y * ow + x];
        if (xx < 0) continue;
        const int xi = (int)xx, yi = (int)yy;
        const Row &r0 = rows[yi - y_lo], &r1 = rows[yi + 1 - y_lo];
        taps[(size_t)y * ow + x] = (uint32_t)(4 * (r0.lds + xi - r0.x0)) | ((uint32_t)(4 * (r1.lds + xi - r1.x0)) << 16);
      }
  }
  const double src_per_out = (double)staged / std::max<double>(1.0, (double)ow * oh);
  if (c->opt_two_stage != 1 && src_per_out >= 1.0) return MDC_OK;
  const int win = (nch_max * 16 + 63) & ~63;
  const int need = (4 * nch_max + 63) / 64;
  const int passes = need <= 2 ? 2 : need <= 3 ? 3 : need <= 4 ? 4 : need <= 5 ? 5 : 8;
  const int nbuf = c->opt_nbuf >= 1 && c->opt_nbuf <= 4 ? c->opt_nbuf : 2;
  if (strip_lds_bytes(win, nbuf, kStripWaves) > kLdsPerCU) return MDC_OK;
  int rc;
  if ((rc = upload(c, &st.d_chunks, flat)) != MDC_OK || (rc = upload(c, &st.d_nch, nch)) != MDC_OK || (rc = upload(c, &st.d_taps, taps)) != MDC_OK)
    return rc;
  const int n_groups = (n_tiles + kStripWaves - 1) / kStripWaves;
  const int gx = std::max(1, tx / kStripWaves);
  const bool rot = c->opt_xcd_rotate == 2;
  const std::vector<int> order = (tx % kStripWaves == 0) ? tile_order(gx, n_groups / gx, c->opt_order, rot) : tile_order(n_groups, 1, MDC_ORDER_BANDS, rot);
  if ((rc = upload(c, &st.d_order, order)) != MDC_OK) return rc;
  st.n_blocks = (int)order.size();
  st.n_tiles = n_tiles;
  st.tiles_x = tx;
  st.win_bytes = win;
  st.passes = passes;
  st.nbuf = nbuf;
  st.staged_bytes = staged;
  st.planned = true;
  return MDC_OK;
}

int plan_tiles(mdc_ctx* c) {
  c->n_black = 0;
  c->bbox[0] = c->bbox[1] = std::numeric_limits<int>::max();
  c->bbox[2] = c->bbox[3] = -1;
  free_plan(c);
  const int ow = c->out_w, oh = c->out_h;
  for (size_t i = 0; i < (size_t)ow * oh; i++) {
    const float xx = c->h_rx[i], yy = c->h_ry[i];
    if (xx < 0) {
      c->n_black++;
      continue;
    }
    c->bbox[0] = std::min(c->bbox[0], (int)xx);
    c->bbox[2] = std::max(c->bbox[2], (int)xx + 1);
    c->bbox[1] = std::min(c->bbox[1], (int)yy);
    c->bbox[3] = std::max(c->bbox[3], (int)yy + 1);
  }
  if (c->bbox[2] < 0) c->bbox[0] = c->bbox[1] = 0;
  static const TileShape cand_u8[] = {{128, 16}, {64, 32}, {128, 32}, {64, 64}, {64, 60}, {64, 16}};
  static const TileShape cand_f32[] = {{128, 16}, {64, 32}, {64, 16}, {128, 32}, {64, 64}, {64, 60}};
  for (int which = 0; which < 2; which++) {
    const TileShape* cand = which == 0 ? cand_u8 : cand_f32;
    const bool forced = c->opt_tile_h != 0 || c->opt_tile_w != 0;
    for (int k = 0; k < 6; k++) {
      const int tw = c->opt_tile_w ? c->opt_tile_w : cand[k].w, th = c->opt_tile_h ? c->opt_tile_h : cand[k].h;
      if (forced && (tw != cand[k].w || th != cand[k].h)) continue;
      free_src_plan(c->plan[which]);
      const int rc = plan_source(c, which == 0 ? 1 : 4, tw, th, c->plan[which]);
      if (rc != MDC_OK) return rc;
      if (c->plan[which].tiled) break;
    }
  }
  return plan_strip(c);
}

}
```

### mono_dataset_code_amd/csrc/xcd_placement.h

```cpp
#pragma once
#include <algorithm>
#include <cstddef>
#include <vector>

#include "mdc_hip.h"

#if defined(__HIPCC__)
#define MDC_XCD_HD __host__ __device__ __forceinline__
#else
#define MDC_XCD_HD inline
#endif

namespace mdc {

constexpr int kXcds = 8;

MDC_XCD_HD int xcd_table_entry(int x, int y, bool rotate) { return rotate ? ((x & ~(kXcds - 1)) | ((x + y) & (kXcds - 1))) : x; }

inline void xcd_bisect(int x0, int y0, int x1, int y1, int parts, int tx, std::vector<std::vector<int>>& out) {
  if (parts == 1) {
    std::vector<int> v;
    for (int y = y0; y < y1; y++)
      for (int x = x0; x < x1; x++) v.push_back(y * tx + x);
    out.push_back(v);
    return;
  }
  if (x1 - x0 > y1 - y0) {
    const int xm = x0 + (x1 - x0 + 1) / 2;
    xcd_bisect(x0, y0, xm, y1, parts / 2, tx, out);
    xcd_bisect(xm, y0, x1, y1, parts / 2, tx, out);
  } else {
    const int ym = y0 + (y1 - y0 + 1) / 2;
    xcd_bisect(x0, y0, x1, ym, parts / 2, tx, out);
    xcd_bisect(x0, ym, x1, y1, parts / 2, tx, out);
  }
}

inline std::vector<int> tile_order(int tx, int ty, int mode, bool rotate = false) {
  const int n = tx * ty;
  std::vector<std::vector<int>> per_xcd(kXcds);
  if (mode == MDC_ORDER_BLOCKS2D && n >= kXcds) {
    per_xcd.clear();
    xcd_bisect(0, 0, tx, ty, kXcds, tx, per_xcd);
  } else if (mode == MDC_ORDER_IDENTITY) {
    for (int t = 0; t < n; t++) per_xcd[t % kXcds].push_back(t);
  } else if (mode == MDC_ORDER_ROWS && ty >= kXcds) {
    int r = 0;
    for (int k = 0; k < kXcds; k++) {
      const int rows = ty / kXcds + (k < ty % kXcds ? 1 : 0);
      for (int y = r; y < r + rows; y++)
        for (int x = 0; x < tx; x++) per_xcd[k].push_back(y * tx + x);
      r += rows;
    }
  } else if (rotate) {
    for (int k = 0; k < kXcds; k++)
      for (int t = (int)((long long)k * n / kXcds); t < (int)((long long)(k + 1) * n / kXcds); t++) per_xcd[k].push_back(t);
  } else {
    const int per = (n + kXcds - 1) / kXcds;
    for (int t = 0; t < n; t++) per_xcd[t / per].push_back(t);
  }
  size_t slots = 0;
  for (const auto& v : per_xcd) slots = std::max(slots, v.size());
  std::vector<int> order(slots * kXcds, -1);
  for (int k = 0; k < kXcds; k++)
    for (size_t j = 0; j < per_xcd[k].size(); j++) order[j * kXcds + k] = per_xcd[k][j];
  return order;
}

}
```

Measured before the change: 3.864 million.

## Add balanced XCD deal schedule and tune tile order in autotuner

Adds an opt-in XCD rotation mode 3 that computes a per-frame-group rotation shift on the host. The shifts are chosen greedily so that work dealt to the eight XCDs stays balanced across tapered frame groups, cached per key, and passed to the tiled kernel. The autotuner also tries row tile ordering as extra trials and remembers the best order, which plan_tiles then applies. The frame-group computation is moved into a shared header. Default rotation stays 1, so the deal path is off unless selected, but the kernel gains an extra argument and a little per-block index work.

```diff
diff --git a/include/mdc_hip.h b/include/mdc_hip.h
--- a/include/mdc_hip.h
+++ b/include/mdc_hip.h
@@ -80,6 +80,7 @@
   int two_stage;
   int prefetch_chunk;
   int prefetch_streams;
+  int tile_order;
 } mdc_info;
 
 
@@ -303,6 +304,8 @@
   int tile_w, tile_h, frames_per_block;
   float ms;
   int candidates;
+  int order;
+  int timed;
 } mdc_tune_result;
 MDC_API int mdc_tune_device(mdc_ctx* ctx, const uint8_t* d_in, float* d_out, int64_t nframes, unsigned flags, void* stream,
                     mdc_tune_result* result);
diff --git a/mono_dataset_code_amd/build.py b/mono_dataset_code_amd/build.py
--- a/mono_dataset_code_amd/build.py
+++ b/mono_dataset_code_amd/build.py
@@ -16,7 +16,7 @@
 
 HIP_SOURCES = [os.path.join(CSRC, f) for f in ("mdc_kernels.hip", "mdc_vcal.hip", "mdc_jpeg.hip", "mdc_capi.hip", "mdc_plan.hip", "mdc_host_calls.hip",
                                                 "mdc_pipeline.hip", "mdc_placement.hip", "mdc_rcal.hip")]
-HIP_DEPS = HIP_SOURCES + [os.path.join(CSRC, "mdc_exports.map"), os.path.join(CSRC, "mdc_internal.h"), os.path.join(CSRC, "mdc_ctx.h"), os.path.join(CSRC, "mdc_build_config.h"), os.path.join(CSRC, "fov_point_model.h"), os.path.join(CSRC, "minmax_first.h"), os.path.join(CSRC, "placement_classes.h"), os.path.join(CSRC, "xcd_placement.h"), os.path.join(INC, "mdc_hip.h")]
+HIP_DEPS = HIP_SOURCES + [os.path.join(CSRC, "mdc_exports.map"), os.path.join(CSRC, "mdc_internal.h"), os.path.join(CSRC, "mdc_ctx.h"), os.path.join(CSRC, "mdc_build_config.h"), os.path.join(CSRC, "fov_point_model.h"), os.path.join(CSRC, "minmax_first.h"), os.path.join(CSRC, "placement_classes.h"), os.path.join(CSRC, "xcd_placement.h"), os.path.join(CSRC, "frame_groups.h"), os.path.join(INC, "mdc_hip.h")]
 HOST_SOURCES = [os.path.join(HOST, f) for f in (
     "fov_undistorter.cpp", "photometric_undistorter.cpp", "gray_png.cpp", "host_device.cpp", "mdc_host_capi.cpp",
     "image_codecs.cpp", "image_codecs_png.cpp", "image_codecs_jpeg.cpp", "image_codecs_jpeg_stream.cpp", "zip_reader.cpp", "image_pool.cpp", "frame_source.cpp", "decode_pool.cpp",
diff --git a/mono_dataset_code_amd/capi.py b/mono_dataset_code_amd/capi.py
--- a/mono_dataset_code_amd/capi.py
+++ b/mono_dataset_code_amd/capi.py
@@ -17,6 +17,7 @@
 OPT_ZERO_COPY = 14
 OPT_TAIL_TAPER = 15
 OPT_XCD_ROTATE = 18
+XCD_ROTATE_OFF, XCD_ROTATE_ON, XCD_ROTATE_STRIPS, XCD_ROTATE_BALANCED = 0, 1, 2, 3
 OPT_DEVICE_PIPELINE_CHUNK, OPT_DEVICE_PIPELINE_CHUNK_HINT = 16, 17
 ORDER_BANDS, ORDER_ROWS, ORDER_IDENTITY, ORDER_BLOCKS2D = 0, 1, 2, 3
 OK, ERR_ARG, ERR_STATE, ERR_SIZE, ERR_HIP, ERR_NO_DEVICE, ERR_NOMEM = 0, -1, -2, -3, -4, -5, -6
@@ -71,7 +72,8 @@
                 ("tile_w", C.c_int), ("tile_h", C.c_int), ("n_tiles", C.c_int), ("lds_bytes", C.c_int),
                 ("window_buffers", C.c_int), ("f32_tiled", C.c_int), ("f32_tile_w", C.c_int), ("f32_tile_h", C.c_int),
                 ("src_bbox", C.c_int * 4), ("src_bbox_bytes", C.c_int64), ("src_staged_bytes", C.c_int64),
-                ("n_black", C.c_int64), ("two_stage", C.c_int), ("prefetch_chunk", C.c_int), ("prefetch_streams", C.c_int)]
+                ("n_black", C.c_int64), ("two_stage", C.c_int), ("prefetch_chunk", C.c_int), ("prefetch_streams", C.c_int),
+                ("tile_order", C.c_int)]
 
 
 class DeviceOutputs(C.Structure):
@@ -91,7 +93,8 @@
 
 
 class TuneResult(C.Structure):
-    _fields_ = [("tile_w", C.c_int), ("tile_h", C.c_int), ("frames_per_block", C.c_int), ("ms", C.c_float), ("candidates", C.c_int)]
+    _fields_ = [("tile_w", C.c_int), ("tile_h", C.c_int), ("frames_per_block", C.c_int), ("ms", C.c_float), ("candidates", C.c_int),
+                ("order", C.c_int), ("timed", C.c_int)]
 
 
 class MdcError(RuntimeError):
diff --git a/mono_dataset_code_amd/csrc/frame_groups.h b/mono_dataset_code_amd/csrc/frame_groups.h
--- /dev/null
+++ b/mono_dataset_code_amd/csrc/frame_groups.h
@@ -0,0 +1,46 @@
+#pragma once
+#include <stdint.h>
+
+#if defined(__HIPCC__)
+#define MDC_FG_HD __host__ __device__ __forceinline__
+#else
+#define MDC_FG_HD inline
+#endif
+
+namespace mdc {
+
+struct FrameGroups {
+  int groups;
+  int full;
+  int r;
+};
+
+MDC_FG_HD FrameGroups frame_groups(int64_t nframes, int fpb, int taper_r) {
+  FrameGroups g{0, 0, taper_r > 0 ? taper_r : 0};
+  if (taper_r <= 0) {
+    g.groups = (int)((nframes + fpb - 1) / fpb);
+    return g;
+  }
+  const int64_t tail = (int64_t)taper_r * (fpb / 2 + fpb / 4);
+  g.full = (int)((nframes - tail) / fpb);
+  const int64_t rest = nframes - (int64_t)g.full * fpb - tail;
+  g.groups = g.full + 2 * taper_r + (int)((rest + fpb / 8 - 1) / (fpb / 8));
+  return g;
+}
+
+MDC_FG_HD void frame_group_range(int y, int groups, int nframes, int fpb, bool interleave, int taper_full, int taper_r, int* first, int* count) {
+  const int fstep = interleave ? groups : 1;
+  int f0 = interleave ? y : y * fpb;
+  int nf = interleave ? (nframes - f0 + fstep - 1) / fstep : (nframes < f0 + fpb ? nframes : f0 + fpb) - f0;
+  if (!interleave && taper_r > 0 && y >= taper_full) {
+    const int k = y - taper_full;
+    const int lvl = k / taper_r < 2 ? k / taper_r : 2;
+    const int size = fpb >> (lvl + 1);
+    f0 = taper_full * fpb + taper_r * (fpb - (fpb >> lvl)) + (k - lvl * taper_r) * size;
+    nf = (nframes < f0 + size ? nframes : f0 + size) - f0;
+  }
+  *first = f0;
+  *count = nf;
+}
+
+}
diff --git a/mono_dataset_code_amd/csrc/mdc_capi.hip b/mono_dataset_code_amd/csrc/mdc_capi.hip
--- a/mono_dataset_code_amd/csrc/mdc_capi.hip
+++ b/mono_dataset_code_amd/csrc/mdc_capi.hip
@@ -83,6 +83,25 @@
   const mdc_ctx::SrcPlan& pl = c->plan[which];
   return TilePlan{pl.d_chunks, pl.d_nch, pl.d_taps, pl.d_order, pl.n_blocks, pl.n_tiles, pl.tiles_x, pl.tile_w, pl.tile_h,
                   pl.chunk_cap, pl.win_bytes, pl.nbuf, c->n_black > 0, c->opt_interleave != 0, c->opt_taper != 2, c->opt_xcd_rotate != 0};
+}
+
+static bool deal_schedule_for(mdc_ctx* c, int which, const TilePlan& p, int64_t nframes, int fpb, bool pyr, DealSchedule* out) {
+  if (c->opt_xcd_rotate != 3 || p.interleave) return false;
+  const mdc_ctx::DealKey key{which, fpb, (pyr ? 1 : 0) | (p.taper ? 2 : 0), nframes};
+  std::lock_guard<std::mutex> g(c->deal_mu);
+  auto it = c->deal_cache.find(key);
+  if (it == c->deal_cache.end()) {
+    const FrameGroups fg = tiled_frame_groups(p, nframes, fpb, pyr, which == 1);
+    std::vector<int> frames((size_t)fg.groups);
+    for (int y = 0; y < fg.groups; y++) {
+      int f0;
+      frame_group_range(y, fg.groups, (int)nframes, fpb, false, fg.full, fg.r, &f0, &frames[y]);
+    }
+    if (c->deal_cache.size() >= 256) c->deal_cache.clear();
+    it = c->deal_cache.emplace(key, deal_schedule(c->plan[which].share, frames)).first;
+  }
+  *out = it->second;
+  return out->first < 0x7fffffff;
 }
 
 RemapArgs remap_args(const mdc_ctx* c, const float* lut, const float* vinv) {
@@ -122,7 +141,10 @@
   const bool aligned = (reinterpret_cast<uintptr_t>(d_in) & 15) == 0;
   if (c->plan[1].tiled && aligned && c->opt_kernel != MDC_KERNEL_GATHER) {
     const int fpb = frames_per_block(c, nframes, c->plan[1].n_blocks);
-    MDC_HIP(c, launch_remap_tiled_f32(d_in, d_out, a, tile_plan(c, 1), nframes, fpb, s));
+    const TilePlan p = tile_plan(c, 1);
+    DealSchedule deal;
+    const bool dealt = deal_schedule_for(c, 1, p, nframes, fpb, false, &deal);
+    MDC_HIP(c, launch_remap_tiled_f32(d_in, d_out, a, p, nframes, fpb, s, dealt ? &deal : nullptr));
   } else {
     const int fpb = frames_per_block(c, nframes, (c->out_w * c->out_h + 255) / 256);
     MDC_HIP(c, launch_remap_gather_f32(d_in, d_out, a, nframes, fpb, s));
@@ -232,8 +254,10 @@
     if (!c->opt_fpb && c->tuned_fpb > 0 && nframes >= c->tuned_min_frames) fpb = (int)std::min<int64_t>(c->tuned_fpb, nframes);
     const bool fuse_pyr = pyr && p.tile_w * p.tile_h <= 2048 && p.tile_h % 8 == 0 && c->out_w % p.tile_w == 0 && c->out_h % p.tile_h == 0 &&
                           tiled_lds_bytes(p.win_bytes, p.nbuf, true) + tiled_pyramid_lds_bytes(p.tile_w, p.tile_h) <= kLdsPerCU;
+    DealSchedule deal;
+    const bool dealt = deal_schedule_for(c, 0, p, nframes, fpb, fuse_pyr, &deal);
     MDC_HIP(c, launch_remap_tiled_u8(d_in, d_out, a, p, nframes, fpb, s, fuse_pyr ? pyr[0] : nullptr,
-                                     fuse_pyr ? pyr[1] : nullptr, fuse_pyr ? pyr[2] : nullptr));
+                                     fuse_pyr ? pyr[1] : nullptr, fuse_pyr ? pyr[2] : nullptr, dealt ? &deal : nullptr));
     if (pyr_done) *pyr_done = fuse_pyr;
   } else {
     const int fpb = frames_per_block(c, nframes, (c->out_w * c->out_h + 255) / 256);
@@ -459,6 +483,7 @@
       if (value == c->opt_tile_h) return MDC_OK;
       c->opt_tile_h = value;
       c->tuned_fpb = 0;
+      c->tuned_order = -1;
       if (!c->valid_remap) return MDC_OK;
       DeviceGuard dg(c->device);
       MDC_HIP(c, hipDeviceSynchronize());
@@ -469,6 +494,7 @@
       if (value == c->opt_tile_w) return MDC_OK;
       c->opt_tile_w = value;
       c->tuned_fpb = 0;
+      c->tuned_order = -1;
       if (!c->valid_remap) return MDC_OK;
       DeviceGuard dg(c->device);
       MDC_HIP(c, hipDeviceSynchronize());
@@ -524,6 +550,7 @@
       if (value == c->opt_two_stage) return MDC_OK;
       c->opt_two_stage = value;
       c->tuned_fpb = 0;
+      c->tuned_order = -1;
       if (!c->valid_remap) return MDC_OK;
       DeviceGuard dg(c->device);
       MDC_HIP(c, hipDeviceSynchronize());
@@ -531,18 +558,22 @@
     }
     case MDC_OPT_TILE_ORDER: {
       if (value < MDC_ORDER_BANDS || value > MDC_ORDER_BLOCKS2D) return fail(c, MDC_ERR_ARG, "bad tile order %d", value);
-      if (value == c->opt_order) return MDC_OK;
+      const bool same = value == c->opt_order && (c->tuned_order < 0 || c->opt_order_set || c->tuned_order == value);
       c->opt_order = value;
+      c->opt_order_set = true;
+      if (same) return MDC_OK;
       if (!c->valid_remap) return MDC_OK;
       DeviceGuard dg(c->device);
       MDC_HIP(c, hipDeviceSynchronize());
       return plan_tiles(c);
     }
     case MDC_OPT_XCD_ROTATE: {
-      if (value < 0 || value > 2) return fail(c, MDC_ERR_ARG, "XCD rotation must be 0 (off), 1 (on) or 2 (on, strip kernel included)");
+      if (value < 0 || value > 3)
+        return fail(c, MDC_ERR_ARG, "XCD rotation must be 0 (off), 1 (on), 2 (on, strip kernel included) or 3 (on, with the balanced deal schedule)");
       if (value == c->opt_xcd_rotate) return MDC_OK;
       c->opt_xcd_rotate = value;
       c->tuned_fpb = 0;
+      c->tuned_order = -1;
       if (!c->valid_remap) return MDC_OK;
       DeviceGuard dg(c->device);
       MDC_HIP(c, hipDeviceSynchronize());
@@ -589,6 +620,7 @@
   i->src_bbox_bytes = c->bbox[2] >= 0 ? (int64_t)(c->bbox[2] - c->bbox[0] + 1) * (c->bbox[3] - c->bbox[1] + 1) : 0;
   i->src_staged_bytes = c->strip.planned ? c->strip.staged_bytes : p0.staged_bytes;
   i->n_black = c->n_black;
+  i->tile_order = p0.tiled ? p0.order : c->opt_order;
   return MDC_OK;
 } MDC_CATCH(c)
 
@@ -634,6 +666,7 @@
   MDC_HIP(c, hipDeviceSynchronize());
   c->valid_remap = false;
   c->tuned_fpb = 0;
+  c->tuned_order = -1;
   free_plan(c);
   for (float** p : {&c->d_rx, &c->d_ry})
     if (*p) {
@@ -978,10 +1011,16 @@
   MDC_HIP(c, hipEventCreate(&e0));
   MDC_HIP(c, hipEventCreate(&e1));
   float best = 1e30f;
-  int bw = 0, bh = 0, bf = 0, tried = 0;
+  int bw = 0, bh = 0, bf = 0, bo = -1, tried = 0, timed = 0;
   int rc = MDC_OK;
   const int caller_fpb = c->opt_fpb;
-  for (const TileShape& sh : shapes) {
+  const int caller_order = c->opt_order;
+  const bool caller_order_set = c->opt_order_set;
+  c->opt_order_set = true;
+  for (int trial = 0; trial < 5 && rc == MDC_OK; trial++) {
+    const TileShape& sh = shapes[trial < 3 ? trial : (trial == 3 ? 2 : 0)];
+    if (trial >= 3 && caller_order_set) break;
+    c->opt_order = trial >= 3 ? MDC_ORDER_ROWS : (caller_order_set ? caller_order : MDC_ORDER_BANDS);
     c->opt_tile_w = sh.w;
     c->opt_tile_h = sh.h;
     if (hipDeviceSynchronize() != hipSuccess) {
@@ -990,6 +1029,7 @@
     }
     if ((rc = plan_tiles(c)) != MDC_OK) break;
     if (!c->plan[0].tiled) continue;
+    if (trial >= 3 && c->plan[0].n_tiles / c->plan[0].tiles_x < kXcds) continue;
     for (int fpb : fpbs) {
       c->opt_fpb = fpb;
       float ms[5];
@@ -1002,12 +1042,14 @@
       }
       if (!ok) continue;
       std::sort(ms, ms + 5);
-      tried++;
+      timed++;
+      if (trial < 3) tried++;
       if (ms[2] < best) {
         best = ms[2];
         bw = sh.w;
         bh = sh.h;
         bf = fpb;
+        bo = c->opt_order;
       }
     }
   }
@@ -1017,6 +1059,9 @@
   c->opt_tile_w = bw;
   c->opt_tile_h = bh;
   c->opt_fpb = caller_fpb;
+  c->opt_order = caller_order;
+  c->opt_order_set = caller_order_set;
+  c->tuned_order = caller_order_set ? -1 : bo;
   c->tuned_fpb = bf;
   c->tuned_min_frames = bf ? std::max<int64_t>(nframes / 4, (int64_t)bf * 8) : 0;
   const int rc2 = plan_tiles(c);
@@ -1027,6 +1072,8 @@
     result->frames_per_block = bf;
     result->ms = tried ? best : 0.f;
     result->candidates = tried;
+    result->order = bo >= 0 ? bo : caller_order;
+    result->timed = timed;
   }
   return rc;
 } MDC_CATCH(c)
diff --git a/mono_dataset_code_amd/csrc/mdc_ctx.h b/mono_dataset_code_amd/csrc/mdc_ctx.h
--- a/mono_dataset_code_amd/csrc/mdc_ctx.h
+++ b/mono_dataset_code_amd/csrc/mdc_ctx.h
@@ -17,6 +17,7 @@
 #include <new>
 #include <shared_mutex>
 #include <string>
+#include <tuple>
 #include <vector>
 
 struct mdc_ctx {
@@ -59,9 +60,20 @@
     int* d_order = nullptr;
     int chunk_cap = 0, win_bytes = 0, nbuf = 2;
     int tile_w = 0, tile_h = 0, n_tiles = 0, tiles_x = 0, n_blocks = 0;
+    int order = MDC_ORDER_BANDS;
+    long long share[mdc::kXcds] = {0};
     bool tiled = false;
     int64_t staged_bytes = 0;
   } plan[2];
+  struct DealKey {
+    int which, fpb, mode;
+    int64_t nframes;
+    bool operator<(const DealKey& o) const {
+      return std::tie(which, fpb, mode, nframes) < std::tie(o.which, o.fpb, o.mode, o.nframes);
+    }
+  };
+  std::mutex deal_mu;
+  std::map<DealKey, mdc::DealSchedule> deal_cache;
   struct Strip {
     uint32_t* d_chunks = nullptr;
     int* d_nch = nullptr;
@@ -81,6 +93,8 @@
   int opt_tile_h = 0;
   int opt_tile_w = 0;
   int opt_order = MDC_ORDER_BANDS;
+  bool opt_order_set = false;
+  int tuned_order = -1;
   int opt_xcd_rotate = 1;
   int opt_nbuf = 0;
   int opt_interleave = 0;
diff --git a/mono_dataset_code_amd/csrc/mdc_internal.h b/mono_dataset_code_amd/csrc/mdc_internal.h
--- a/mono_dataset_code_amd/csrc/mdc_internal.h
+++ b/mono_dataset_code_amd/csrc/mdc_internal.h
@@ -3,6 +3,7 @@
 #include <stdint.h>
 
 #include "fov_point_model.h"
+#include "frame_groups.h"
 #include "mdc_build_config.h"
 #include "xcd_placement.h"
 
@@ -49,6 +50,7 @@
   bool taper = true;
   bool rotate = false;
 };
+FrameGroups tiled_frame_groups(const TilePlan& p, int64_t nframes, int fpb, bool pyr, bool f32);
 
 constexpr int kStripTileW = 128, kStripTileH = 8;
 constexpr int kStripChunkCap = 128;
@@ -82,9 +84,9 @@
                                    hipStream_t s);
 hipError_t launch_remap_tiled_u8(const uint8_t* d_in, float* d_out, const RemapArgs& a, const TilePlan& p,
                                  int64_t nframes, int fpb, hipStream_t s, float* d_l1 = nullptr, float* d_l2 = nullptr,
-                                 float* d_l3 = nullptr);
+                                 float* d_l3 = nullptr, const DealSchedule* deal = nullptr);
 hipError_t launch_remap_tiled_f32(const float* d_in, float* d_out, const RemapArgs& a, const TilePlan& p,
-                                  int64_t nframes, int fpb, hipStream_t s);
+                                  int64_t nframes, int fpb, hipStream_t s, const DealSchedule* deal = nullptr);
 size_t tiled_lds_bytes(int win_bytes, int nbuf, bool lut = true);
 size_t tiled_pyramid_lds_bytes(int tile_w, int tile_h);
 constexpr size_t kLdsPerCU = 160 * 1024;
diff --git a/mono_dataset_code_amd/csrc/mdc_kernels.hip b/mono_dataset_code_amd/csrc/mdc_kernels.hip
--- a/mono_dataset_code_amd/csrc/mdc_kernels.hip
+++ b/mono_dataset_code_amd/csrc/mdc_kernels.hip
@@ -526,24 +526,17 @@
 template <bool VIG, bool BLACK, bool PYR, bool F32, int TW, int NT, int NBUF>
 __global__ __launch_bounds__(NT, (NT >= 960 ? 8 : NT == 640 ? 5 : NT == 512 ? (kLutRep < 32 ? 8 : 6) : 4)) void remap_tiled_kernel(
     const uint8_t* __restrict__ in, float* __restrict__ out, RemapArgs a, TilePlan p, PyramidOut py, int nframes, int fpb,
-    int interleave, int taper_full, int taper_r) {
+    int interleave, int taper_full, int taper_r, DealSchedule deal) {
   constexpr int RPT = tile_rpt(TW, 0);
   extern __shared__ __attribute__((aligned(1024))) unsigned char smem[];
   float* s_lut = reinterpret_cast<float*>(smem);
   lds_u8_ptr s_win = (lds_u8_ptr)smem + (F32 ? 0 : kLutBytes);
 
-  const int tile = p.d_order[xcd_table_entry((int)blockIdx.x, (int)blockIdx.y, p.rotate)];
+  const int tile = p.d_order[xcd_table_entry((int)blockIdx.x, (int)blockIdx.y, p.rotate, deal_shift(deal, (int)blockIdx.y))];
   if (tile < 0) return;
   const int fstep = interleave ? (int)gridDim.y : 1;
-  int f0 = interleave ? (int)blockIdx.y : (int)blockIdx.y * fpb;
-  int nf = interleave ? (nframes - f0 + fstep - 1) / fstep : min(nframes, f0 + fpb) - f0;
-  if (!interleave && taper_r > 0 && (int)blockIdx.y >= taper_full) {
-    const int k = (int)blockIdx.y - taper_full;
-    const int lvl = min(k / taper_r, 2);
-    const int size = fpb >> (lvl + 1);
-    f0 = taper_full * fpb + taper_r * (fpb - (fpb >> lvl)) + (k - lvl * taper_r) * size;
-    nf = min(nframes, f0 + size) - f0;
-  }
+  int f0, nf;
+  frame_group_range((int)blockIdx.y, (int)gridDim.y, nframes, fpb, interleave != 0, taper_full, taper_r, &f0, &nf);
   if (nf <= 0) return;
 
   const int tid = threadIdx.x;
@@ -1087,32 +1080,31 @@
   int64_t nframes;
   int fpb;
   hipStream_t s;
+  DealSchedule deal;
 };
 
-static int taper_groups(int64_t nframes, int fpb, int taper_r, int* full) {
-  *full = 0;
-  if (taper_r <= 0) return (int)ceil_div(nframes, fpb);
-  const int64_t tail = (int64_t)taper_r * (fpb / 2 + fpb / 4);
-  *full = (int)((nframes - tail) / fpb);
-  const int64_t rest = nframes - (int64_t)*full * fpb - tail;
-  return *full + 2 * taper_r + (int)ceil_div(rest, fpb / 8);
+FrameGroups tiled_frame_groups(const TilePlan& p, int64_t nframes, int fpb, bool pyr, bool f32) {
+  const int nt = tile_threads(p.tile_w, p.tile_h);
+  const size_t lds = tiled_lds_bytes(p.win_bytes, p.nbuf, !f32) + (pyr ? tiled_pyramid_lds_bytes(p.tile_w, p.tile_h) : 0);
+  const int resident = 256 * (int)std::max<size_t>(1, std::min<size_t>(2048 / nt, kLdsPerCU / std::max<size_t>(lds, 1)));
+  int taper_r = std::max(2, (resident + p.n_blocks / 2) / std::max(1, p.n_blocks));
+  if (!p.taper || p.interleave || fpb % 8 != 0 || fpb < 16 || nframes < (int64_t)fpb * (4 * taper_r)) taper_r = 0;
+  return frame_groups(nframes, fpb, taper_r);
 }
 
 template <bool VIG, bool BLACK, bool PYR, bool F32, int TW, int NT, int NBUF>
 static hipError_t launch_tiled_variant(const TiledLaunch& l) {
   const size_t lds = tiled_lds_bytes(l.p.win_bytes, NBUF, !F32) + (PYR ? tiled_pyramid_lds_bytes(l.p.tile_w, l.p.tile_h) : 0);
-  const int resident = 256 * (int)std::max<size_t>(1, std::min<size_t>(2048 / NT, kLdsPerCU / std::max<size_t>(lds, 1)));
-  int taper_r = std::max(2, (resident + l.p.n_blocks / 2) / std::max(1, l.p.n_blocks));
-  if (!l.p.taper || l.p.interleave || l.fpb % 8 != 0 || l.fpb < 16 || l.nframes < (int64_t)l.fpb * (4 * taper_r)) taper_r = 0;
-  int taper_full = 0;
-  dim3 grid(l.p.n_blocks, taper_groups(l.nframes, l.fpb, taper_r, &taper_full));
+  if (NBUF != l.p.nbuf || NT != tile_threads(l.p.tile_w, l.p.tile_h)) return hipErrorInvalidValue;
+  const FrameGroups fg = tiled_frame_groups(l.p, l.nframes, l.fpb, PYR, F32);
+  dim3 grid(l.p.n_blocks, fg.groups);
   if (lds > 64 * 1024) {
     hipError_t e = hipFuncSetAttribute(reinterpret_cast<const void*>(&remap_tiled_kernel<VIG, BLACK, PYR, F32, TW, NT, NBUF>),
                                        hipFuncAttributeMaxDynamicSharedMemorySize, (int)lds);
     if (e != hipSuccess) return e;
   }
   remap_tiled_kernel<VIG, BLACK, PYR, F32, TW, NT, NBUF><<<grid, NT, lds, l.s>>>(l.d_in, l.d_out, l.a, l.p, l.py, (int)l.nframes, l.fpb,
-                                                                                 l.p.interleave ? 1 : 0, taper_full, taper_r);
+                                                                                 l.p.interleave ? 1 : 0, fg.full, fg.r, l.deal);
   return hipGetLastError();
 }
 
@@ -1214,23 +1206,23 @@
 }
 
 hipError_t launch_remap_tiled_u8(const uint8_t* d_in, float* d_out, const RemapArgs& a, const TilePlan& p,
-                                 int64_t nframes, int fpb, hipStream_t s, float* d_l1, float* d_l2, float* d_l3) {
+                                 int64_t nframes, int fpb, hipStream_t s, float* d_l1, float* d_l2, float* d_l3, const DealSchedule* deal) {
   if (nframes <= 0) return hipSuccess;
   if ((int64_t)a.in_w * a.in_h >= (int64_t)kOutside || (int64_t)a.out_w * a.out_h * 4 >= (int64_t)kOutside)
     return hipErrorInvalidValue;
   PyramidOut tiled_py{};
   tiled_py.l1 = d_l1, tiled_py.l2 = d_l2, tiled_py.l3 = d_l3;
-  const TiledLaunch l{d_in, d_out, a, p, tiled_py, nframes, fpb, s};
+  const TiledLaunch l{d_in, d_out, a, p, tiled_py, nframes, fpb, s, deal ? *deal : DealSchedule{}};
   if (a.vinv) return p.has_black ? launch_tiled_nt<true, true>(l) : launch_tiled_nt<true, false>(l);
   return p.has_black ? launch_tiled_nt<false, true>(l) : launch_tiled_nt<false, false>(l);
 }
 
 hipError_t launch_remap_tiled_f32(const float* d_in, float* d_out, const RemapArgs& a, const TilePlan& p,
-                                  int64_t nframes, int fpb, hipStream_t s) {
+                                  int64_t nframes, int fpb, hipStream_t s, const DealSchedule* deal) {
   if (nframes <= 0) return hipSuccess;
   if ((int64_t)a.in_w * a.in_h * 4 >= (int64_t)kOutside || (int64_t)a.out_w * a.out_h * 4 >= (int64_t)kOutside)
     return hipErrorInvalidValue;
-  const TiledLaunch l{reinterpret_cast<const uint8_t*>(d_in), d_out, a, p, PyramidOut{}, nframes, fpb, s};
+  const TiledLaunch l{reinterpret_cast<const uint8_t*>(d_in), d_out, a, p, PyramidOut{}, nframes, fpb, s, deal ? *deal : DealSchedule{}};
   return p.has_black ? launch_tiled_shape<false, true, false, true>(l) : launch_tiled_shape<false, false, false, true>(l);
 }
 
diff --git a/mono_dataset_code_amd/csrc/mdc_plan.hip b/mono_dataset_code_amd/csrc/mdc_plan.hip
--- a/mono_dataset_code_amd/csrc/mdc_plan.hip
+++ b/mono_dataset_code_amd/csrc/mdc_plan.hip
@@ -29,6 +29,8 @@
     free_src_plan(pl);
   }
   free_strip_plan(c->strip);
+  std::lock_guard<std::mutex> g(c->deal_mu);
+  c->deal_cache.clear();
 }
 
 template <typename T>
@@ -126,8 +128,10 @@
   if ((rc = upload(c, &pl.d_chunks, flat)) != MDC_OK || (rc = upload(c, &pl.d_nch, nch)) != MDC_OK ||
       (rc = upload(c, &pl.d_taps, taps)) != MDC_OK)
     return rc;
-  const std::vector<int> order = tile_order(tx, ty, c->opt_order, c->opt_xcd_rotate != 0);
+  pl.order = (es == 1 && !c->opt_order_set && c->tuned_order >= 0) ? c->tuned_order : c->opt_order;
+  const std::vector<int> order = tile_order(tx, ty, pl.order, c->opt_xcd_rotate != 0);
   if ((rc = upload(c, &pl.d_order, order)) != MDC_OK) return rc;
+  xcd_shares(order, pl.share);
   pl.n_blocks = (int)order.size();
   pl.n_tiles = n_tiles;
   pl.tiles_x = tx;
diff --git a/mono_dataset_code_amd/csrc/xcd_placement.h b/mono_dataset_code_amd/csrc/xcd_placement.h
--- a/mono_dataset_code_amd/csrc/xcd_placement.h
+++ b/mono_dataset_code_amd/csrc/xcd_placement.h
@@ -15,7 +15,24 @@
 
 constexpr int kXcds = 8;
 
-MDC_XCD_HD int xcd_table_entry(int x, int y, bool rotate) { return rotate ? ((x & ~(kXcds - 1)) | ((x + y) & (kXcds - 1))) : x; }
+MDC_XCD_HD int xcd_table_entry(int x, int y, bool rotate, int shift = -1) {
+  return rotate ? ((x & ~(kXcds - 1)) | ((x + (shift < 0 ? y : shift)) & (kXcds - 1))) : x;
+}
+
+constexpr int kDealSlots = 63;
+constexpr int kDealPerWord = 21;
+struct DealSchedule {
+  unsigned long long bits[3] = {0, 0, 0};
+  int first = 0x7fffffff;
+};
+
+MDC_XCD_HD int deal_shift(const DealSchedule& d, int y) {
+  const int i = y - d.first;
+  if (i < 0 || i >= kDealSlots) return -1;
+  const unsigned long long w = i < kDealPerWord ? d.bits[0] : i < 2 * kDealPerWord ? d.bits[1] : d.bits[2];
+  const int j = i < kDealPerWord ? i : i < 2 * kDealPerWord ? i - kDealPerWord : i - 2 * kDealPerWord;
+  return (int)(w >> (3 * j)) & (kXcds - 1);
+}
 
 inline void xcd_bisect(int x0, int y0, int x1, int y1, int parts, int tx, std::vector<std::vector<int>>& out) {
   if (parts == 1) {
@@ -67,4 +84,50 @@
   return order;
 }
 
+inline void xcd_shares(const std::vector<int>& order, long long share[kXcds]) {
+  for (int k = 0; k < kXcds; k++) share[k] = 0;
+  for (size_t b = 0; b < order.size(); b++)
+    if (order[b] >= 0) share[b % kXcds]++;
 }
+
+inline long long deal_spread(const long long share[kXcds], const std::vector<int>& group_frames, const DealSchedule& d) {
+  long long acc[kXcds] = {0};
+  for (size_t y = 0; y < group_frames.size(); y++) {
+    const int s = deal_shift(d, (int)y);
+    for (int k = 0; k < kXcds; k++) acc[k] += share[(k + (s < 0 ? (int)y : s)) & (kXcds - 1)] * group_frames[y];
+  }
+  return *std::max_element(acc, acc + kXcds) - *std::min_element(acc, acc + kXcds);
+}
+
+inline DealSchedule deal_schedule(const long long share[kXcds], const std::vector<int>& group_frames) {
+  const int G = (int)group_frames.size();
+  DealSchedule none, d;
+  if (G == 0) return none;
+  d.first = std::max(0, G - kDealSlots);
+  long long acc[kXcds] = {0};
+  for (int y = 0; y < d.first; y++)
+    for (int k = 0; k < kXcds; k++) acc[k] += share[(k + y) & (kXcds - 1)] * group_frames[y];
+  for (int y = d.first; y < G; y++) {
+    int best = -1;
+    long long best_spread = 0;
+    for (int t = 0; t < kXcds; t++) {
+      const int s = (y + t) & (kXcds - 1);
+      long long mx = 0, mn = 0;
+      for (int k = 0; k < kXcds; k++) {
+        const long long v = acc[k] + share[(k + s) & (kXcds - 1)] * group_frames[y];
+        mx = k ? std::max(mx, v) : v;
+        mn = k ? std::min(mn, v) : v;
+      }
+      if (best < 0 || mx - mn < best_spread) {
+        best = s;
+        best_spread = mx - mn;
+      }
+    }
+    for (int k = 0; k < kXcds; k++) acc[k] += share[(k + best) & (kXcds - 1)] * group_frames[y];
+    const int i = y - d.first;
+    d.bits[i / kDealPerWord] |= (unsigned long long)best << (3 * (i % kDealPerWord));
+  }
+  return deal_spread(share, group_frames, d) < deal_spread(share, group_frames, none) ? d : none;
+}
+
+}
```

Result: faster. 3.925 million, median of 5 (+1.6%).
